# adelacvg/detail_tts

Hardware: AMD Instinct MI355X
Metric: generated audio seconds/sec (24 kHz), 10 s prompt, batch 8 per GPU (higher is better)
Workload: dtype f32; 1 GPU; configs[2]: 1xMI355X batch-8, 10 s prompts (T_ref=936), 234 codes -> 9.984 s audio per utterance; GPT KV-cache decode + 50-step CFG diffusion + flow-VAE/HiFiGAN vocoder, seed-0 random-init weights; batch_per_gpu=8, codes=234, diffusion_steps=50, parallelism=replica x1

## Files before the change

detail_tts_amd/csrc/conv_gemm.h:

```cpp
#pragma once
#include "common.h"

namespace dtts {

struct ConvParams {
    const float* x = nullptr;
    long long x_bs = 0;
    int x_cs = 0;
    const int* len_in = nullptr;
    const int* x_bidx = nullptr;
    int Tin = 0;
    const float* pro_ab = nullptr;
    int pro_act = ACT_NONE;
    float pro_slope = 0.f;
    const float* w = nullptr;
    const float* bias = nullptr;
    int Cin = 0, CinP = 0, Cout = 0, CoutP = 0, KW = 1, stride = 1, dil = 1, pad = 0;
    const float* badd = nullptr;
    int badd_bs = 0;
    int gate = GATE_NONE;
    int epi_act = ACT_NONE;
    float epi_slope = 0.f;
    float out_scale = 1.f;
    const float* res = nullptr;
    long long res_bs = 0;
    int res_cs = 0;
    float res_scale = 1.f;
    int res_bmod = 0;
    int mask_out = 0;
    float* y = nullptr;
    long long y_bs = 0;
    int y_cs = 0;
    const int* len_out = nullptr;
    int Nout = 0;
    int phases = 1;
    int B = 0;
    const void* w3 = nullptr;
    const void* x3 = nullptr;
    int x3_tp = 0;
    int x3_halo = 1;
    void* qkv_planes = nullptr;
    int qkv_heads = 0, qkv_nt64 = 0, qkv_tq = 0;
    float qkv_qscale = 1.f;
    void* gn_out3 = nullptr;
    const float *gn_gamma = nullptr, *gn_beta = nullptr;
    const float* gn_ada = nullptr;
    int gn_ada_stride = 0;
    const int* gn_ada_idx = nullptr;
    int gn_act = ACT_NONE, gn_groups = 32;
    float gn_eps = 1e-5f;
    void* gn_xch = nullptr;
    unsigned gn_tag = 0;
    int* gn_err = nullptr;
    const int* cols = nullptr;
    int ncols = 0, cols_b0 = 0;
    void* next3 = nullptr;
    int next_c8 = 0, next_tp = 0, next_halo = 0, next_act = ACT_NONE;
    float next_slope = 0.f;
    int* next_sat = nullptr;
    int ksplit = 1;
    int ksplit_max = 0;
    int p1 = 0;
    int epi_vec = 0;
    float* kpart = nullptr;
    int* kcount = nullptr;
    int ablate = 0;
};

void launch_conv_gemm(const ConvParams& p, hipStream_t stream);

}
```

detail_tts_amd/csrc/conv_gemm.hip:

```cpp
#include <cstdlib>
#include "conv_gemm_kernel.h"

namespace dtts {

static int env_int(const char* name) {
    const char* v = getenv(name);
    return v ? atoi(v) : 0;
}

void launch_conv_gemm(const ConvParams& p_in, hipStream_t stream) {
    static const int ablate = env_int("DTTS_CONV_ABLATE");
    ConvParams p = p_in;
    p.ablate = ablate;
    DTTS_REQUIRE(p.B > 0 && p.Nout > 0 && p.Cout > 0 && p.Cin > 0, "empty conv");
    DTTS_REQUIRE(p.x && p.w && p.y, "null pointer");
    DTTS_REQUIRE(p.gate == GATE_NONE || p.phases == 1, "gate+phases unsupported");
    static const int force_bn = env_int("DTTS_CONV_BN"), force_bk = env_int("DTTS_CONV_BK");
    const int halo = (p.KW - 1) * p.dil;
    auto fits = [&](int bn) { return (bn - 1) * p.stride + halo + 1 <= XW_MAX; };
    const bool bk32 = (p.CinP % 32 == 0) && force_bk == 32 && p.KW * p.dil <= 3;
    static const int small_tiles = []() { const char* v = getenv("DTTS_CONV_SMALL_TILES"); return v ? atoi(v) : 384; }();
    if (small_tiles > 0 && p.CoutP % 64 == 0 && fits(64) && (long long)cdiv(p.CoutP, 128) * cdiv(p.Nout, 128) * p.B <= small_tiles) {
        static const int small_bk = []() { const char* v = getenv("DTTS_CONV_SMALL_BK"); return v ? atoi(v) : 32; }();
        if (small_bk == 32 && p.CinP % 32 == 0 && p.KW * p.dil <= 3) launch_conv_tile<64, 64, 2, 2, 32>(p, stream, "conv_gemm_kernel<64,64,k32>");
        else launch_conv_tile<64, 64, 2, 2, 16>(p, stream, "conv_gemm_kernel<64,64,k16>");
        return;
    }
    if (p.CoutP % 128 == 0) {
        const int pad128 = round_up(p.Nout, 128), pad64 = round_up(p.Nout, 64);
        bool wide = fits(128) && (pad128 - pad64) * 10 <= p.Nout;
        if (force_bn == 128 && fits(128)) wide = true;
        if (force_bn == 64) wide = false;
        if (wide) {
            if (bk32) launch_conv_tile<128, 128, 2, 2, 32>(p, stream, "conv_gemm_kernel<128,128,k32>");
            else launch_conv_tile<128, 128, 2, 2, 16>(p, stream, "conv_gemm_kernel<128,128,k16>");
        } else {
            DTTS_REQUIRE(fits(64), "conv halo too large");
            if (bk32) launch_conv_tile<128, 64, 2, 2, 32>(p, stream, "conv_gemm_kernel<128,64,k32>");
            else launch_conv_tile<128, 64, 2, 2, 16>(p, stream, "conv_gemm_kernel<128,64,k16>");
        }
    } else if (p.CoutP % 64 == 0) {
        if (fits(128) && p.Nout > 64) launch_conv_tile<64, 128, 2, 2, 16>(p, stream, "conv_gemm_kernel<64,128,k16>");
        else { DTTS_REQUIRE(fits(64), "conv halo too large"); launch_conv_tile<64, 64, 2, 2, 16>(p, stream, "conv_gemm_kernel<64,64,k16>"); }
    } else {
        DTTS_REQUIRE(p.CoutP % 32 == 0, "CoutP must be a multiple of 32");
        DTTS_REQUIRE(fits(128), "conv halo too large");
        launch_conv_tile<32, 128, 1, 4, 16>(p, stream, "conv_gemm_kernel<32,128,k16>");
    }
}

}
```

detail_tts_amd/csrc/conv_x3.h:

```cpp
#pragma once
#include "conv_gemm.h"

namespace dtts {

constexpr int X3_HALO = 1;
constexpr int X3_BN = 192;
static inline int x3_tp(int T) { return round_up(T, X3_BN) + 2 * X3_HALO; }
static inline size_t x3_bytes(int B, int C, int T) { return (size_t)B * (C / 8) * 2 * x3_tp(T) * 16; }

void launch_split_weights(const float* wp, int KW, int CinP, int CoutP, void* out, hipStream_t s);
void launch_split_planes(const float* x, long long x_bs, int x_cs, const float* ab, int act, const int* lens, int T, int B, int C,
                         void* out, hipStream_t s);
void launch_split_planes_taps(const float* x, long long x_bs, int x_cs, const int* lens, int T, int B, int C, int KW, int pad, void* out,
                              hipStream_t s, int* sat = nullptr);
void launch_gn_split_planes(const float* x, long long x_bs, int x_cs, const int* lens, int T, int B, int C, int groups,
                            const float* gamma, const float* beta, float eps, const float* ada, int ada_stride, int ada_bs, int act,
                            void* out, hipStream_t s, const int* ada_idx = nullptr);
void launch_conv_x3(const ConvParams& p, hipStream_t s);

constexpr size_t X3_SLAB_FLOATS = 96 * 256, X3_MAX_SLABS = 1024, X3_SPLIT_COUNTERS = 4096;
void x3_split_workspace(hipStream_t s, size_t nslabs, float** part, int** count);

constexpr int GN_FUSE_MAX_NT = 6;
size_t conv_x3_gn_xch_bytes(int B, int Cout, int T);
bool conv_x3_gn_fusable(int Cout, int CoutP, int Cin, int KW, int groups, int B, int T);

constexpr int X3D_HALO = 32;
static inline int x3d_tp(int T) { return round_up(T, X3_BN) + 64 + X3D_HALO; }
static inline size_t x3d_bytes(int B, int CP, int T) { return (size_t)B * (CP / 8) * 2 * x3d_tp(T) * 16; }
void launch_split_planes_ex(const float* x, long long x_bs, int x_cs, int act, float slope, const int* lens, int T, int B, int C, int CP,
                            int halo, int Tp, void* out, hipStream_t s, int* sat = nullptr);
void launch_conv_x3d(const ConvParams& p, hipStream_t s);
void launch_zero_plane_margins(const int* lens, int T, int B, int CP, int halo, int Tp, void* out, hipStream_t s);

}
```

detail_tts_amd/csrc/conv_x3.hip:

```cpp
#include <algorithm>
#include <cstdio>
#include <mutex>
#include <type_traits>
#include <utility>
#include <vector>

#include "conv_x3.h"
#include <cstdlib>
#include "prof.h"
#include "split3.h"

namespace dtts {

typedef float f32x16 __attribute__((ext_vector_type(16)));

namespace {
constexpr int NPL = XS_PLANES, NK = 2 * NPL;
constexpr int BM = 128, BN = X3_BN;
constexpr int WTILE = NK * BM * 16;
constexpr int XMAIN = NK * BN * 16;
constexpr int XBUF = XMAIN + NK * 2 * 16;
typedef unsigned gn_u4 __attribute__((ext_vector_type(4)));
constexpr int GN_AUX_SC1 = 16;
constexpr int GN_MAXW = 8;
constexpr int GN_SPIN_LIMIT = 1 << 22;
static_assert(7 * 32 <= 256 && 3 * GN_FUSE_MAX_NT <= 32 && (4 * 16 * 104 + 4 * GN_MAXW + 16 + 2 * BM) * 4 <= 2 * (WTILE + XBUF), "fused GroupNorm epilogue: LDS / lanes");

__global__ __launch_bounds__(256) void split_weights_kernel(const float* __restrict__ wp, int C8, int CoutP, uint4* __restrict__ out) {
    const int m = blockIdx.x * 256 + threadIdx.x, c8 = blockIdx.y, tap = blockIdx.z;
    if (m >= CoutP) return;
    float v[8];
#pragma unroll
    for (int e = 0; e < 8; ++e) v[e] = wp[((long long)tap * C8 * 8 + c8 * 8 + e) * CoutP + m] * XS_SCALE_W;
    uint4 q0, q1;
    split8(v, q0, q1);
    uint4* o = out + ((long long)(tap * C8 + c8) * NPL) * CoutP + m;
    o[0] = q0;
    o[CoutP] = q1;
}

template <int ACT, bool AB>
__global__ __launch_bounds__(256) void split_planes_kernel(const float* __restrict__ x, long long x_bs, int x_cs,
                                                          const float* __restrict__ ab, const int* __restrict__ lens, int T, int C8,
                                                          int Tp, uint4* __restrict__ out) {
    const int tp = blockIdx.x * 256 + threadIdx.x, c8 = blockIdx.y, b = blockIdx.z;
    if (tp >= Tp) return;
    const int t = tp - X3_HALO, len = lens ? lens[b] : T;
    uint4 q0 = make_uint4(0, 0, 0, 0), q1 = q0;
    if (t >= 0 && t < len) {
        const float* xr = x + (long long)b * x_bs + (long long)(c8 * 8) * x_cs + t;
        float v[8];
#pragma unroll
        for (int e = 0; e < 8; ++e) v[e] = xr[(long long)e * x_cs];
        if (AB) {
            const float* abr = ab + ((long long)b * C8 + c8) * 16;
#pragma unroll
            for (int e = 0; e < 8; ++e) v[e] = abr[2 * e] * v[e] + abr[2 * e + 1];
        }
        if (ACT == ACT_SILU) {
#pragma unroll
            for (int e = 0; e < 8; ++e) v[e] = v[e] * __frcp_rn(1.f + __expf(-v[e]));
        }
#pragma unroll
        for (int e = 0; e < 8; ++e) v[e] *= XS_SCALE_X;
        split8(v, q0, q1);
    }
    uint4* o = out + ((long long)(b * C8 + c8) * NPL) * Tp + tp;
    o[0] = q0;
    o[Tp] = q1;
}

template <int ACT>
__global__ __launch_bounds__(1024) void gn_split_planes_kernel(const float* __restrict__ x, long long x_bs, int x_cs,
                                                              const int* __restrict__ lens, int T, int C, int groups,
                                                              const float* __restrict__ gamma, const float* __restrict__ beta, float eps,
                                                              const float* __restrict__ ada, int ada_stride, int ada_bs, int Tp,
                                                              uint4* __restrict__ out, const int* __restrict__ ada_idx) {
    __shared__ float red[2][16];
    __shared__ float sa[64], sd[64];
    const int g = blockIdx.x, b = blockIdx.y, tid = threadIdx.x, lane = tid & 63, wave = tid >> 6, nthr = blockDim.x;
    const int len = lens ? lens[b] : T;
    const int cpg = C / groups;
    const float* xg = x + (long long)b * x_bs + (long long)(g * cpg) * x_cs;
    const float k = xg[0];
    float s1 = 0.f, s2 = 0.f;
    const bool vec = ((x_cs & 3) == 0) && ((reinterpret_cast<unsigned long long>(xg) & 15ull) == 0);
    if (vec) {
        const int len4 = len >> 2, n4 = cpg * len4;
        for (int i0 = tid; i0 < n4; i0 += 4 * nthr) {
            float4 v[4];
#pragma unroll
            for (int u = 0; u < 4; ++u) {
                const int i = i0 + u * nthr, ic = i < n4 ? i : 0;
                const int row = ic / len4, t4 = ic - row * len4;
                v[u] = reinterpret_cast<const float4*>(xg + (long long)row * x_cs)[t4];
            }
#pragma unroll
            for (int u = 0; u < 4; ++u) {
                if (i0 + u * nthr >= n4) continue;
                const float d0 = v[u].x - k, d1 = v[u].y - k, d2 = v[u].z - k, d3 = v[u].w - k;
                s1 += (d0 + d1) + (d2 + d3);
                s2 += (d0 * d0 + d1 * d1) + (d2 * d2 + d3 * d3);
            }
        }
        const int rem = len - (len4 << 2);
        for (int i = tid; i < cpg * rem; i += nthr) {
            const int row = i / rem, t = (len4 << 2) + (i - row * rem);
            const float d = xg[(long long)row * x_cs + t] - k;
            s1 += d;
            s2 += d * d;
        }
    } else {
        for (int i = tid; i < cpg * len; i += nthr) {
            const int row = i / len, t = i - row * len;
            const float d = xg[(long long)row * x_cs + t] - k;
            s1 += d;
            s2 += d * d;
        }
    }
#pragma unroll
    for (int o = 32; o > 0; o >>= 1) {
        s1 += __shfl_xor(s1, o);
        s2 += __shfl_xor(s2, o);
    }
    if (lane == 0) { red[0][wave] = s1; red[1][wave] = s2; }
    __syncthreads();
    float S1 = 0.f, S2 = 0.f;
    for (int i = 0; i < (nthr >> 6); ++i) { S1 += red[0][i]; S2 += red[1][i]; }
    const float n = (float)(cpg * len);
    S1 /= n;
    S2 /= n;
    const float mean = k + S1, var = fmaxf(S2 - S1 * S1, 0.f), rstd = rsqrtf(var + eps);
    if (tid < cpg) {
        const int c = g * cpg + tid;
        float a = rstd * gamma[c];
        float d = beta[c] - mean * a;
        if (ada) {
            const float* ad = ada + (ada_idx ? (long long)ada_idx[b] : (long long)b * ada_bs);
            const float sc = 1.f + ad[(long long)c * ada_stride], sh = ad[(long long)(C + c) * ada_stride];
            a *= sc;
            d = d * sc + sh;
        }
        sa[tid] = a;
        sd[tid] = d;
    }
    __syncthreads();
    const int c8n = cpg >> 3, C8 = C >> 3;
    for (int item = blockIdx.z * nthr + tid; item < c8n * Tp; item += nthr * gridDim.z) {
        const int c8l = item / Tp, tp = item - c8l * Tp, t = tp - X3_HALO;
        uint4 q0 = make_uint4(0, 0, 0, 0), q1 = q0;
        if (t >= 0 && t < len) {
            const float* xr = xg + (long long)(c8l * 8) * x_cs + t;
            float v[8];
#pragma unroll
            for (int e = 0; e < 8; ++e) v[e] = xr[(long long)e * x_cs];
#pragma unroll
            for (int e = 0; e < 8; ++e) {
                v[e] = sa[c8l * 8 + e] * v[e] + sd[c8l * 8 + e];
                if (ACT == ACT_SILU) v[e] = v[e] * __frcp_rn(1.f + __expf(-v[e]));
                v[e] *= XS_SCALE_X;
            }
            split8(v, q0, q1);
        }
        uint4* o = out + ((long long)(b * C8 + g * c8n + c8l) * NPL) * Tp + tp;
        o[0] = q0;
        o[Tp] = q1;
    }
}

template <int ACT, int NI>
__global__ __launch_bounds__(1024) void gn_split_planes_reg_kernel(const float* __restrict__ x, long long x_bs, int x_cs,
                                                                  const int* __restrict__ lens, int T, int C, int groups,
                                                                  const float* __restrict__ gamma, const float* __restrict__ beta, float eps,
                                                                  const float* __restrict__ ada, int ada_stride, int ada_bs, int Tp,
                                                                  uint4* __restrict__ out, const int* __restrict__ ada_idx) {
    __shared__ float red[2][16];
    __shared__ float sa[64], sd[64];
    const int g = blockIdx.x, b = blockIdx.y, tid = threadIdx.x, lane = tid & 63, wave = tid >> 6;
    const int len = lens ? lens[b] : T;
    const int cpg = C / groups, c8n = cpg >> 3, C8 = C >> 3, nitems = c8n * Tp;
    const float* xg = x + (long long)b * x_bs + (long long)(g * cpg) * x_cs;
    const float k = xg[0];
    float v[NI][8];
    float s1 = 0.f, s2 = 0.f;
#pragma unroll
    for (int q = 0; q < NI; ++q) {
        const int item = tid + q * 1024, c8l = item / Tp, t = item - c8l * Tp - X3_HALO;
        const bool ok = item < nitems && t >= 0 && t < len;
        const float* xr = xg + (long long)(ok ? c8l * 8 : 0) * x_cs + (ok ? t : 0);
#pragma unroll
        for (int e = 0; e < 8; ++e) v[q][e] = xr[(long long)e * x_cs];
        if (ok) {
            float d[8];
#pragma unroll
            for (int e = 0; e < 8; ++e) d[e] = v[q][e] - k;
            s1 += ((d[0] + d[1]) + (d[2] + d[3])) + ((d[4] + d[5]) + (d[6] + d[7]));
            s2 += ((d[0] * d[0] + d[1] * d[1]) + (d[2] * d[2] + d[3] * d[3])) + ((d[4] * d[4] + d[5] * d[5]) + (d[6] * d[6] + d[7] * d[7]));
        }
    }
#pragma unroll
    for (int o = 32; o > 0; o >>= 1) {
        s1 += __shfl_xor(s1, o);
        s2 += __shfl_xor(s2, o);
    }
    if (lane == 0) { red[0][wave] = s1; red[1][wave] = s2; }
    __syncthreads();
    float S1 = 0.f, S2 = 0.f;
#pragma unroll
    for (int i = 0; i < 16; ++i) { S1 += red[0][i]; S2 += red[1][i]; }
    const float n = (float)(cpg * len);
    S1 /= n;
    S2 /= n;
    const float mean = k + S1, var = fmaxf(S2 - S1 * S1, 0.f), rstd = rsqrtf(var + eps);
    if (tid < cpg) {
        const int c = g * cpg + tid;
        float a = rstd * gamma[c];
        float d = beta[c] - mean * a;
        if (ada) {
            const float* ad = ada + (ada_idx ? (long long)ada_idx[b] : (long long)b * ada_bs);
            const float sc = 1.f + ad[(long long)c * ada_stride], sh = ad[(long long)(C + c) * ada_stride];
            a *= sc;
            d = d * sc + sh;
        }
        sa[tid] = a;
        sd[tid] = d;
    }
    __syncthreads();
#pragma unroll
    for (int q = 0; q < NI; ++q) {
        const int item = tid + q * 1024;
        if (item >= nitems) continue;
        const int c8l = item / Tp, tp = item - c8l * Tp, t = tp - X3_HALO;
        uint4 q0 = make_uint4(0, 0, 0, 0), q1 = q0;
        if (t >= 0 && t < len) {
            float w[8];
#pragma unroll
            for (int e = 0; e < 8; ++e) {
                w[e] = sa[c8l * 8 + e] * v[q][e] + sd[c8l * 8 + e];
                if (ACT == ACT_SILU) w[e] = w[e] * __frcp_rn(1.f + __expf(-w[e]));
                w[e] *= XS_SCALE_X;
            }
            split8(w, q0, q1);
        }
        uint4* o = out + ((long long)(b * C8 + g * c8n + c8l) * NPL) * Tp + tp;
        o[0] = q0;
        o[Tp] = q1;
    }
}

template <int EPI, bool KW3, int NSTG, bool P1 = false>
__global__ __launch_bounds__(256, (NSTG == 2 && EPI != 3) ? 3 : 2) void conv_x3_kernel(ConvParams p) {
    constexpr int KW = KW3 ? 3 : 1, D = NSTG - 1;
    constexpr int CB = P1 ? 4 : 2;
    constexpr int NT = P1 ? 2 : 3;
    auto chunk_of = [](int kind) { return P1 ? kind * NPL : (kind & 1) * NPL + (kind >> 1); };
    constexpr int XOFF = NSTG * WTILE;
    extern __shared__ __attribute__((aligned(16))) unsigned char smem[];
    const int tid = threadIdx.x, lane = tid & 63, wave = __builtin_amdgcn_readfirstlane(tid >> 6), l31 = lane & 31, lhi = lane >> 5;
    const int mtiles = p.CoutP / BM, ntiles = (p.Nout + BN - 1) / BN;
    const int Ls = xcd_remap(blockIdx.x, gridDim.x);
    const int S = p.ksplit, L = Ls / S, z = Ls - L * S;
    const bool mt_major = EPI == 3 && !(p.ablate & 16);
    int mt = mt_major ? (L / ntiles) % mtiles : L % mtiles;
    int b = mt_major ? L / (ntiles * mtiles) : (L / mtiles) / ntiles;
    int nti = mt_major ? L % ntiles : (L / mtiles) - b * ntiles;
    int bn = L / mtiles;
    if (EPI == 2 && mtiles > 6 && mtiles % 6 == 0 && !(p.ablate & 1024)) {
        const int nbn = p.cols ? p.ncols : ntiles * p.B, per_blk = 5 * mtiles, blk = L / per_blk, r = L - blk * per_blk;
        const int bn0 = blk * 5, nb = min(5, nbn - bn0), per_grp = nb * 6, mg = r / per_grp, r2 = r - mg * per_grp, bnl = r2 / 6;
        mt = mg * 6 + (r2 - bnl * 6);
        bn = bn0 + bnl;
        b = bn / ntiles;
        nti = bn - b * ntiles;
    }
    if (p.cols) {
        const int pk = __builtin_amdgcn_readfirstlane(p.cols[bn]);
        b = (pk >> 8) - p.cols_b0;
        nti = pk & 255;
    }
    const int m0 = mt * BM, n0 = nti * BN;
    const int nvalid = p.len_out ? p.len_out[b] : p.Nout;
    if (n0 >= nvalid) return;
    const int C8 = p.Cin >> 3, call = p.Cin >> (P1 ? 5 : 4), Tp = p.x3_tp;
    const int cbeg = (int)((long long)call * z / S), c16n = (int)((long long)call * (z + 1) / S) - cbeg, nks = KW * c16n;
    const int bin = p.x_bidx ? p.x_bidx[b] : b;
    const unsigned lane16 = (unsigned)lane * 16u;
    const unsigned char* wb8 = static_cast<const unsigned char*>(p.w3) + ((long long)m0 + (long long)(CB * cbeg) * NPL * p.CoutP) * 16;
    const unsigned char* xb8 = static_cast<const unsigned char*>(p.x3) +
                               ((long long)bin * C8 * NPL * Tp + n0 + (X3_HALO - p.pad) + (long long)(CB * cbeg) * NPL * Tp) * 16;
    const long long wtapB = (long long)C8 * NPL * p.CoutP * 16;
    const long long wblkB = (long long)CB * NPL * p.CoutP * 16;
    const long long xblkB = (long long)CB * NPL * Tp * 16;
    auto dma = [&](const unsigned char* g, int lds_off) {
        __builtin_amdgcn_global_load_lds((const __attribute__((address_space(1))) void*)(g + lane16),
                                         (__attribute__((address_space(3))) void*)(smem + lds_off), 16, 0, 0);
    };
    const int wkind = wave;
    const unsigned char* wq = wb8 + (long long)chunk_of(wkind) * p.CoutP * 16;
    const int wlds = wkind * (BM * 16);
    const unsigned char* xq = xb8 + (long long)chunk_of(wkind) * Tp * 16;
    const int xlds = XOFF + wkind * (BN * 16);
    long long x3o[3];
    int x3l[3];
#pragma unroll
    for (int t = 0; t < 3; ++t) {
        const int j = t * 4 + wave, kind = j / 3, cb = j - kind * 3;
        x3o[t] = ((long long)chunk_of(kind) * Tp + cb * 64) * 16;
        x3l[t] = XOFF + kind * (BN * 16) + cb * 1024;
    }
    const long long halo_lane = (lane < 2 * NK) ? (((long long)chunk_of(lane >> 1) * Tp + BN + (lane & 1)) * 16 - (long long)lane16) : 0;
    const unsigned char* xblk = xb8;
    auto issue_w = [&](int i, int stage) { dma(wq + i * 1024, stage * WTILE + wlds + i * 1024); };
    auto issue_x1 = [&](int i, int stage) { dma(xq + i * 1024, stage * XBUF + xlds + i * 1024); };
    auto issue_x3 = [&](int t, int stage) { dma(xblk + x3o[t], stage * XBUF + x3l[t]); };
    auto issue_halo = [&](int stage) {
        if (lane < 2 * NK)
            __builtin_amdgcn_global_load_lds((const __attribute__((address_space(1))) void*)(xblk + halo_lane + lane16),
                                             (__attribute__((address_space(3))) void*)(smem + XOFF + stage * XBUF + XMAIN), 16, 0, 0);
    };
    int itap = 0;
    auto next_w = [&]() {
        if (!KW3) wq += wblkB;
        else if (itap < 2) { wq += wtapB; ++itap; }
        else { wq += wblkB - 2 * wtapB; itap = 0; }
    };

    const int wm0 = (wave >> 1) * 64, wn0 = (wave & 1) * 96;
    f32x16 acc[2][3];
#pragma unroll
    for (int i = 0; i < 2; ++i)
#pragma unroll
        for (int j = 0; j < 3; ++j)
#pragma unroll
            for (int r = 0; r < 16; ++r) acc[i][j][r] = 0.f;

#pragma unroll
    for (int q = 0; q < D; ++q) {
        if (q < nks) {
            issue_w(0, q);
            issue_w(1, q);
        }
        next_w();
        if (!KW3) {
            if (q < nks) {
#pragma unroll
                for (int i = 0; i < 3; ++i) issue_x1(i, q);
            }
            xq += xblkB;
        } else {
            if (q < c16n) {
#pragma unroll
                for (int t = 0; t < 3; ++t) issue_x3(t, q);
                issue_halo(q);
            }
            xblk += xblkB;
        }
    }
    float* bias_s = reinterpret_cast<float*>(smem + XOFF + NSTG * XBUF);
    if (tid < BM) bias_s[tid] = (p.bias && m0 + tid < p.Cout) ? p.bias[m0 + tid] : 0.f;
    float* ga_s = bias_s + BM + 4;
    float* gb_s = ga_s + BM;
    if (EPI == 3 && tid < BM) {
        const int c = m0 + tid;
        float ga = p.gn_gamma[c], gb = p.gn_beta[c];
        if (p.gn_ada) {
            const float* ad = p.gn_ada + (p.gn_ada_idx ? (long long)p.gn_ada_idx[b] : 0);
            const float sc = 1.f + ad[(long long)c * p.gn_ada_stride], sh = ad[(long long)(p.Cout + c) * p.gn_ada_stride];
            ga *= sc;
            gb = gb * sc + sh;
        }
        ga_s[tid] = ga;
        gb_s[tid] = gb;
    }

    int c16 = 0, tap = 0;
    int sw = 0, sx = 0;
    auto read_frags = [&](hf8 (&fa)[2][NPL], hf8 (&fb)[3][NPL], int stw, int stx, int tp) {
        const unsigned char* As = smem + stw * WTILE + lhi * (BM * 16);
        const unsigned char* Xb = smem + XOFF + stx * XBUF;
#pragma unroll
        for (int j = 0; j < 3; ++j) {
            const int nn = wn0 + j * 32 + l31 + tp;
            const unsigned char* xr = nn < BN ? Xb + lhi * (BN * 16) + nn * 16 : Xb + XMAIN + lhi * 32 + (nn - BN) * 16;
            const int xps = nn < BN ? 2 * BN * 16 : 64;
#pragma unroll
            for (int pl = 0; pl < NPL; ++pl) fb[j][pl] = *reinterpret_cast<const hf8*>(xr + pl * xps);
        }
#pragma unroll
        for (int i = 0; i < 2; ++i)
#pragma unroll
            for (int pl = 0; pl < NPL; ++pl) fa[i][pl] = *reinterpret_cast<const hf8*>(As + pl * (2 * BM * 16) + (wm0 + i * 32 + l31) * 16);
    };
    auto issue_slot = [&](int slot, int swi, int sxi, bool wlive, bool xlive) {
        __builtin_amdgcn_sched_barrier(0);
        if (slot < 2) { if (wlive) issue_w(slot, swi); }
        else if (!KW3) { if (xlive) issue_x1(slot - 2, sxi); }
        else if (slot == 2) { if (xlive) issue_x3(tap, sxi); }
        else if (slot == 3 && tap == 2) { if (xlive) issue_halo(sxi); }
        __builtin_amdgcn_sched_barrier(0);
    };
    auto advance = [&]() {
        next_w();
        if (!KW3) xq += xblkB;
        sw = sw + 1 == NSTG ? 0 : sw + 1;
        if (++tap == KW) {
            tap = 0;
            ++c16;
            sx = sx + 1 == NSTG ? 0 : sx + 1;
            if (KW3) xblk += xblkB;
        }
    };
    constexpr int TA[3] = {P1 ? 0 : 1, P1 ? 1 : 0, 0}, TB[3] = {0, 1, 0};
    {
    hf8 a[2][NPL], bb[3][NPL];
    int ks = 0;
    constexpr int PERIOD = KW * NSTG;
    auto ustep = [&](auto kc) {
        constexpr int k = decltype(kc)::value;
        constexpr int TAPc = k % KW, SWc = k % NSTG, SXc = (k / KW) % NSTG;
        constexpr int SWI = (SWc + D) % NSTG, SXI = (SXc + D) % NSTG;
        if (NSTG == 2) asm volatile("s_waitcnt vmcnt(0)" ::: "memory");
        else asm volatile("s_waitcnt vmcnt(%0)" ::"n"((NSTG - 2) * (KW3 ? 3 : 5)) : "memory");
        __builtin_amdgcn_s_barrier();
        constexpr bool ASM_READS = NSTG >= 3;
        if (!ASM_READS) read_frags(a, bb, SWc, SXc, TAPc);
        else {
            const unsigned as_addr = (unsigned)(SWc * WTILE) + lhi * (BM * 16) + (wm0 + l31) * 16;
            const unsigned xb_addr = (unsigned)(XOFF + SXc * XBUF);
            auto rd = [&](hf8& dst, unsigned addr) { asm volatile("ds_read_b128 %0, %1" : "=v"(dst) : "v"(addr)); };
            auto a_addr = [&](int i, int pl) { return as_addr + pl * (2 * BM * 16) + i * 32 * 16; };
            auto x_addr = [&](int j, int pl) {
                const int nn = wn0 + j * 32 + l31 + TAPc;
                return nn < BN ? xb_addr + lhi * (BN * 16) + nn * 16 + pl * (2 * BN * 16) : xb_addr + XMAIN + lhi * 32 + (nn - BN) * 16 + pl * 64;
            };
            constexpr int PA0 = TA[0], PA1 = TA[1];
            rd(a[0][PA0], a_addr(0, PA0)); rd(bb[0][0], x_addr(0, 0)); rd(bb[1][0], x_addr(1, 0)); rd(bb[2][0], x_addr(2, 0));
            rd(a[1][PA0], a_addr(1, PA0));
            rd(a[0][PA1], a_addr(0, PA1)); rd(bb[0][1], x_addr(0, 1)); rd(bb[1][1], x_addr(1, 1)); rd(bb[2][1], x_addr(2, 1));
            rd(a[1][PA1], a_addr(1, PA1));
        }
        auto uslot = [&](int slot) {
            __builtin_amdgcn_sched_barrier(0);
            if (slot < 2) issue_w(slot, SWI);
            else if (!KW3) issue_x1(slot - 2, SXI);
            else if (slot == 2) issue_x3(TAPc, SXI);
            else if (slot == 3 && TAPc == 2) issue_halo(SXI);
            __builtin_amdgcn_sched_barrier(0);
        };
        int slot = 0;
#pragma unroll
        for (int t = 0; t < NT; ++t)
#pragma unroll
            for (int i = 0; i < 2; ++i) {
                if (ASM_READS && t == 0 && i == 0) asm volatile("s_waitcnt lgkmcnt(6)" : "+v"(a[0][TA[0]]), "+v"(bb[0][0]), "+v"(bb[1][0]), "+v"(bb[2][0]));
                if (ASM_READS && t == 0 && i == 1) asm volatile("s_waitcnt lgkmcnt(5)" : "+v"(a[1][TA[0]]));
                if (ASM_READS && t == 1 && i == 0) asm volatile("s_waitcnt lgkmcnt(1)" : "+v"(a[0][TA[1]]), "+v"(bb[0][1]), "+v"(bb[1][1]), "+v"(bb[2][1]));
                if (ASM_READS && t == 1 && i == 1) asm volatile("s_waitcnt lgkmcnt(0)" : "+v"(a[1][TA[1]]));
#pragma unroll
                for (int j = 0; j < 3; ++j) acc[i][j] = __builtin_amdgcn_mfma_f32_32x32x16_f16(a[i][TA[t]], bb[j][TB[t]], acc[i][j], 0, 0, 0);
                if (slot < 5) uslot(slot);
                ++slot;
            }
#pragma unroll
        for (; slot < 5; ++slot) uslot(slot);
        if (!KW3) {
            wq += wblkB;
            xq += xblkB;
        } else {
            if ((TAPc + D) % KW < 2) wq += wtapB;
            else wq += wblkB - 2 * wtapB;
            if (TAPc == KW - 1) xblk += xblkB;
        }
    };
    auto uperiod = [&](auto... kc) { (ustep(kc), ...); };
    constexpr bool UNROLL = KW3 || EPI == 2;
    if (UNROLL && !(p.ablate & 512)) {
        const int nper = KW3 ? (c16n - D) / NSTG : (nks - D) / PERIOD;
        for (int q = 0; q < nper; ++q) {
            if constexpr (PERIOD == 2) uperiod(std::integral_constant<int, 0>{}, std::integral_constant<int, 1>{});
            else if constexpr (PERIOD == 3) uperiod(std::integral_constant<int, 0>{}, std::integral_constant<int, 1>{}, std::integral_constant<int, 2>{});
            else if constexpr (PERIOD == 4) uperiod(std::integral_constant<int, 0>{}, std::integral_constant<int, 1>{}, std::integral_constant<int, 2>{}, std::integral_constant<int, 3>{});
            else if constexpr (PERIOD == 6) uperiod(std::integral_constant<int, 0>{}, std::integral_constant<int, 1>{}, std::integral_constant<int, 2>{}, std::integral_constant<int, 3>{}, std::integral_constant<int, 4>{}, std::integral_constant<int, 5>{});
            else if constexpr (PERIOD == 9) uperiod(std::integral_constant<int, 0>{}, std::integral_constant<int, 1>{}, std::integral_constant<int, 2>{}, std::integral_constant<int, 3>{}, std::integral_constant<int, 4>{}, std::integral_constant<int, 5>{}, std::integral_constant<int, 6>{}, std::integral_constant<int, 7>{}, std::integral_constant<int, 8>{});
            else uperiod(std::integral_constant<int, 0>{}, std::integral_constant<int, 1>{}, std::integral_constant<int, 2>{}, std::integral_constant<int, 3>{}, std::integral_constant<int, 4>{}, std::integral_constant<int, 5>{}, std::integral_constant<int, 6>{}, std::integral_constant<int, 7>{}, std::integral_constant<int, 8>{}, std::integral_constant<int, 9>{}, std::integral_constant<int, 10>{}, std::integral_constant<int, 11>{});
        }
        ks = nper * PERIOD;
        c16 = ks / KW;
        itap = D % KW;
    }
    for (; ks < nks; ++ks) {
        if (NSTG == 2 || ks + D > nks || (KW3 && c16 + D >= c16n)) asm volatile("s_waitcnt vmcnt(0)" ::: "memory");
        else asm volatile("s_waitcnt vmcnt(%0)" ::"n"((NSTG - 2) * (KW3 ? 3 : 5)) : "memory");
        __builtin_amdgcn_s_barrier();
        read_frags(a, bb, sw, sx, tap);
        const int swi = sw + D >= NSTG ? sw + D - NSTG : sw + D, sxi = sx + D >= NSTG ? sx + D - NSTG : sx + D;
        const bool wlive = ks + D < nks, xlive = KW3 ? c16 + D < c16n : ks + D < nks;
        int slot = 0;
#pragma unroll
        for (int t = 0; t < NT; ++t)
#pragma unroll
            for (int i = 0; i < 2; ++i) {
#pragma unroll
                for (int j = 0; j < 3; ++j) acc[i][j] = __builtin_amdgcn_mfma_f32_32x32x16_f16(a[i][TA[t]], bb[j][TB[t]], acc[i][j], 0, 0, 0);
                if (slot < 5) issue_slot(slot, swi, sxi, wlive, xlive);
                ++slot;
            }
#pragma unroll
        for (; slot < 5; ++slot) issue_slot(slot, swi, sxi, wlive, xlive);
        advance();
    }
    }
    asm volatile("s_waitcnt vmcnt(0)" ::: "memory");

    if (S > 1) {
        float* slab = p.kpart + ((size_t)L * S) * (96 * 256);
        float* mine = slab + (size_t)z * (96 * 256) + tid;
#pragma unroll
        for (int i = 0; i < 2; ++i)
#pragma unroll
            for (int j = 0; j < 3; ++j)
#pragma unroll
                for (int r = 0; r < 16; ++r) __hip_atomic_store(mine + ((i * 3 + j) * 16 + r) * 256, acc[i][j][r], __ATOMIC_RELAXED, __HIP_MEMORY_SCOPE_AGENT);
        asm volatile("s_waitcnt vmcnt(0)" ::: "memory");
        __syncthreads();
        int* s_last = reinterpret_cast<int*>(bias_s + BM);
        if (tid == 0) *s_last = __hip_atomic_fetch_add(p.kcount + L, 1, __ATOMIC_RELAXED, __HIP_MEMORY_SCOPE_AGENT) == S - 1 ? 1 : 0;
        __syncthreads();
        if (!*s_last) return;
        if (tid == 0) __hip_atomic_store(p.kcount + L, 0, __ATOMIC_RELAXED, __HIP_MEMORY_SCOPE_AGENT);
#pragma unroll
        for (int i = 0; i < 2; ++i)
#pragma unroll
            for (int j = 0; j < 3; ++j)
#pragma unroll
                for (int r = 0; r < 16; ++r) acc[i][j][r] = 0.f;
        for (int zz = 0; zz < S; ++zz) {
            const float* src = slab + (size_t)zz * (96 * 256) + tid;
#pragma unroll
            for (int i = 0; i < 2; ++i)
#pragma unroll
                for (int j = 0; j < 3; ++j)
#pragma unroll
                    for (int r = 0; r < 16; ++r)
                        acc[i][j][r] += __hip_atomic_load(src + ((i * 3 + j) * 16 + r) * 256, __ATOMIC_RELAXED, __HIP_MEMORY_SCOPE_AGENT);
        }
    }

    if (EPI == 3) {
        constexpr int EP_LD = 104;
        if (p.ablate & 64) return;
        __syncthreads();
        float* st = reinterpret_cast<float*>(smem) + wave * (16 * EP_LD);
        float* prt = reinterpret_cast<float*>(smem) + 4 * 16 * EP_LD;
        float* gst = prt + 4 * GN_MAXW;
        float* sa = gst + 16;
        float* sd = sa + BM;
        const int ncol0 = n0 + wn0;
        const float* rb = p.res ? p.res + (long long)(p.res_bmod ? b % p.res_bmod : b) * p.res_bs : nullptr;
        float4 rv[4][6];
        if (rb) {
#pragma unroll
            for (int q = 0; q < 4; ++q)
#pragma unroll
                for (int k = 0; k < 6; ++k) {
                    const int idx = lane + 64 * k, rl = idx / 24, c4 = idx - rl * 24, row = m0 + wm0 + (q >> 1) * 32 + (q & 1) * 16 + rl, n = ncol0 + c4 * 4;
                    const float* src = rb + (long long)row * p.res_cs + n;
                    rv[q][k] = make_float4(0.f, 0.f, 0.f, 0.f);
                    if (n + 3 < nvalid) rv[q][k] = *reinterpret_cast<const float4*>(src);
                    else if (n < nvalid) {
                        rv[q][k].x = src[0];
                        if (n + 1 < nvalid) rv[q][k].y = src[1];
                        if (n + 2 < nvalid) rv[q][k].z = src[2];
                    }
                }
        }
#pragma unroll
        for (int q = 0; q < 4; ++q) {
            const int i = q >> 1, rowt0 = wm0 + i * 32 + (q & 1) * 16;
            if (rb) {
#pragma unroll
                for (int k = 0; k < 6; ++k) {
                    const int idx = lane + 64 * k, rl = idx / 24, c4 = idx - rl * 24;
                    *reinterpret_cast<float4*>(st + rl * EP_LD + c4 * 4) = rv[q][k];
                }
                asm volatile("s_waitcnt lgkmcnt(0)" ::: "memory");
                __builtin_amdgcn_wave_barrier();
            }
#pragma unroll
            for (int j = 0; j < 3; ++j)
#pragma unroll
                for (int rr = 0; rr < 8; ++rr) {
                    const int r = (q & 1) * 8 + rr, rl = (rr & 3) + 8 * (rr >> 2) + 4 * lhi;
                    float v = acc[i][j][r] * XS_ACC_SCALE + bias_s[rowt0 + rl];
                    if (rb) v += p.res_scale * st[rl * EP_LD + j * 32 + l31];
                    acc[i][j][r] = v;
                }
            if (rb) {
                asm volatile("s_waitcnt lgkmcnt(0)" ::: "memory");
                __builtin_amdgcn_wave_barrier();
            }
        }
        bool okj[3];
#pragma unroll
        for (int j = 0; j < 3; ++j) okj[j] = ncol0 + j * 32 + l31 < nvalid;
        const int nvh = min(max(nvalid - ncol0, 0), 96);
        const float cnt = 8.f * (float)nvh, rcnt = nvh > 0 ? 1.f / cnt : 0.f;
        float s8[8];
#pragma unroll
        for (int ck = 0; ck < 8; ++ck) {
            float a = 0.f;
#pragma unroll
            for (int j = 0; j < 3; ++j)
#pragma unroll
                for (int e = 0; e < 4; ++e) a += okj[j] ? acc[ck >> 2][j][4 * (ck & 3) + e] : 0.f;
            s8[ck] = a;
        }
        const float tot = wave_sum8(s8, lane);
#pragma unroll
        for (int ck = 0; ck < 8; ++ck) {
            const float mu = __builtin_bit_cast(float, __builtin_amdgcn_readlane(__builtin_bit_cast(int, tot), 8 * ck)) * rcnt;
            float a = 0.f;
#pragma unroll
            for (int j = 0; j < 3; ++j)
#pragma unroll
                for (int e = 0; e < 4; ++e) {
                    const float dv = acc[ck >> 2][j][4 * (ck & 3) + e] - mu;
                    a += okj[j] ? dv * dv : 0.f;
                }
            s8[ck] = a;
        }
        const float m2 = wave_sum8(s8, lane);
        const int C8o = p.Cout >> 3, NTs = ntiles;
        const __amdgpu_buffer_rsrc_t xrs = __builtin_amdgcn_make_buffer_rsrc(p.gn_xch, (short)0, (int)((size_t)p.B * C8o * NTs * 2 * 16), 0x00020000);
        if ((lane & 7) == 0) {
            const int chunk = ((m0 + wm0) >> 3) + (lane >> 3);
            const gn_u4 wv = {__float_as_uint(tot * rcnt), __float_as_uint(m2), __float_as_uint(cnt), p.gn_tag};
            __builtin_amdgcn_raw_buffer_store_b128(wv, xrs, (((b * C8o + chunk) * NTs + nti) * 2 + (wave & 1)) * 16, 0, GN_AUX_SC1);
        }
        if (p.y) {
            float* yb = p.y + (long long)b * p.y_bs;
#pragma unroll
            for (int q = 0; q < 4; ++q) {
                const int i = q >> 1, rowt0 = wm0 + i * 32 + (q & 1) * 16;
#pragma unroll
                for (int j = 0; j < 3; ++j)
#pragma unroll
                    for (int rr = 0; rr < 8; ++rr) {
                        const int r = (q & 1) * 8 + rr, rl = (rr & 3) + 8 * (rr >> 2) + 4 * lhi;
                        st[rl * EP_LD + j * 32 + l31] = acc[i][j][r];
                    }
                asm volatile("s_waitcnt lgkmcnt(0)" ::: "memory");
                __builtin_amdgcn_wave_barrier();
#pragma unroll
                for (int k = 0; k < 6; ++k) {
                    const int idx = lane + 64 * k, rl = idx / 24, c4 = idx - rl * 24, row = m0 + rowt0 + rl, n = ncol0 + c4 * 4;
                    const float4 a4 = *reinterpret_cast<const float4*>(st + rl * EP_LD + c4 * 4);
                    if (n < nvalid) {
                        float* dst = yb + (long long)row * p.y_cs + n;
                        if (n + 3 < nvalid) *reinterpret_cast<float4*>(dst) = a4;
                        else {
                            dst[0] = a4.x;
                            if (n + 1 < nvalid) dst[1] = a4.y;
                            if (n + 2 < nvalid) dst[2] = a4.z;
                        }
                    }
                }
                asm volatile("s_waitcnt lgkmcnt(0)" ::: "memory");
                __builtin_amdgcn_wave_barrier();
            }
        }
        if (p.ablate & 128) return;
        const int cpg8 = (p.Cout / p.gn_groups) >> 3;
        const int ct0 = m0 >> 3, g_lo = ct0 / cpg8, g_hi = (ct0 + BM / 8 - 1) / cpg8;
        const int nvt = (nvalid + BN - 1) / BN, ppg = cpg8 * nvt;
        const int SL = ppg <= 16 ? 16 : 32;
        {
            const int gs = tid / SL, k = tid - gs * SL;
            const bool active = gs <= g_hi - g_lo && k < ppg;
            float pn = 0.f, pm = 0.f, pq = 0.f;
            if (active) {
                const int ch = k / nvt, nt = k - ch * nvt;
                const int off = (((b * C8o + (g_lo + gs) * cpg8 + ch) * NTs + nt) * 2) * 16;
                gn_u4 v0, v1;
                int spins = 0;
                for (;;) {
                    v0 = __builtin_amdgcn_raw_buffer_load_b128(xrs, off, 0, GN_AUX_SC1);
                    v1 = __builtin_amdgcn_raw_buffer_load_b128(xrs, off + 16, 0, GN_AUX_SC1);
                    if ((v0.w == p.gn_tag && v1.w == p.gn_tag) || (p.ablate & 8)) break;
                    if (++spins > GN_SPIN_LIMIT) {
                        __hip_atomic_store(p.gn_err, 1, __ATOMIC_RELAXED, __HIP_MEMORY_SCOPE_SYSTEM);
                        break;
                    }
                    __builtin_amdgcn_s_sleep(1);
                }
                const float m0v = __uint_as_float(v0.x), q0v = __uint_as_float(v0.y), n0v = __uint_as_float(v0.z);
                const float m1v = __uint_as_float(v1.x), q1v = __uint_as_float(v1.y), n1v = __uint_as_float(v1.z);
                pn = n0v + n1v;
                const float rn = pn > 0.f ? 1.f / pn : 0.f, dm = m0v - m1v;
                pm = (n0v * m0v + n1v * m1v) * rn;
                pq = q0v + q1v + n0v * n1v * rn * dm * dm;
            }
            float N = pn, S = pn * pm;
            for (int o = 1; o < SL; o <<= 1) {
                N += __shfl_xor(N, o);
                S += __shfl_xor(S, o);
            }
            const float mu = N > 0.f ? S / N : 0.f, dmu = pm - mu;
            float M2 = pq + pn * dmu * dmu;
            for (int o = 1; o < SL; o <<= 1) M2 += __shfl_xor(M2, o);
            if (active && k == 0) {
                gst[2 * gs] = mu;
                gst[2 * gs + 1] = rsqrtf((N > 0.f ? M2 / N : 0.f) + p.gn_eps);
            }
        }
        __syncthreads();
        if (tid < BM) {
            const int g = (m0 + tid) / (p.Cout / p.gn_groups) - g_lo;
            const float a = gst[2 * g + 1] * ga_s[tid];
            sa[tid] = a;
            sd[tid] = gb_s[tid] - gst[2 * g] * a;
        }
        __syncthreads();
        if (p.ablate & 256) return;
        const int Tp = p.x3_tp;
        unsigned char* ob = static_cast<unsigned char*>(p.gn_out3) + (size_t)b * C8o * NPL * Tp * 16;
        const bool silu = p.gn_act == ACT_SILU;
#pragma unroll
        for (int i = 0; i < 2; ++i)
#pragma unroll
            for (int j = 0; j < 3; ++j) {
                const int n = ncol0 + j * 32 + l31;
                const bool ok = n < nvalid;
#pragma unroll
                for (int k2 = 0; k2 < 2; ++k2) {
                    const int r16 = wm0 + i * 32 + 16 * k2;
                    float ve[4], vo[4];
#pragma unroll
                    for (int e = 0; e < 4; ++e) {
                        const int ra = r16 + e + 4 * lhi, rb2 = ra + 8;
                        float x0 = acc[i][j][8 * k2 + e] * sa[ra] + sd[ra], x1 = acc[i][j][8 * k2 + 4 + e] * sa[rb2] + sd[rb2];
                        if (silu) {
                            x0 = x0 * __frcp_rn(1.f + __expf(-x0));
                            x1 = x1 * __frcp_rn(1.f + __expf(-x1));
                        }
                        ve[e] = ok ? x0 * XS_SCALE_X : 0.f;
                        vo[e] = ok ? x1 * XS_SCALE_X : 0.f;
                    }
                    unsigned we0[2], we1[2], wo0[2], wo1[2];
                    split_pair(ve[0], ve[1], we0[0], we1[0]);
                    split_pair(ve[2], ve[3], we0[1], we1[1]);
                    split_pair(vo[0], vo[1], wo0[0], wo1[0]);
                    split_pair(vo[2], vo[3], wo0[1], wo1[1]);
                    const auto s00 = __builtin_amdgcn_permlane32_swap(we0[0], wo0[0], false, false);
                    const auto s01 = __builtin_amdgcn_permlane32_swap(we0[1], wo0[1], false, false);
                    const auto s10 = __builtin_amdgcn_permlane32_swap(we1[0], wo1[0], false, false);
                    const auto s11 = __builtin_amdgcn_permlane32_swap(we1[1], wo1[1], false, false);
                    const int c8 = ((m0 + r16) >> 3) + lhi;
                    unsigned char* o = ob + ((size_t)c8 * NPL * Tp + n + X3_HALO) * 16;
                    if (p.ablate & 32) continue;
                    *reinterpret_cast<uint4*>(o) = make_uint4(s00[0], s01[0], s00[1], s01[1]);
                    *reinterpret_cast<uint4*>(o + (size_t)Tp * 16) = make_uint4(s10[0], s11[0], s10[1], s11[1]);
                }
            }
        if (tid < 64) {
            const int side = tid >> 5, c8 = (m0 >> 3) + ((tid & 31) >> 1), pl = tid & 1;
            const int tp = side == 0 ? 0 : n0 + BN + X3_HALO;
            if (side == 0 ? n0 == 0 : (n0 + BN >= nvalid && tp < Tp))
                *reinterpret_cast<uint4*>(ob + ((size_t)(c8 * NPL + pl) * Tp + tp) * 16) = make_uint4(0, 0, 0, 0);
        }
        return;
    }

    if (EPI != 2 && p.epi_vec) {
        constexpr int EP_LD = 104;
        float* yb = p.y + (long long)b * p.y_bs;
        const float* rb = p.res ? p.res + (long long)(p.res_bmod ? b % p.res_bmod : b) * p.res_bs : nullptr;
        const int ncol0 = n0 + wn0;
        constexpr bool RES_AHEAD = NSTG >= 3;
        float4 rva[RES_AHEAD ? 4 : 1][6];
        auto load_res = [&](int q, float4 (&dst)[6]) {
#pragma unroll
            for (int k = 0; k < 6; ++k) {
                const int idx = lane + 64 * k, rl = idx / 24, c4 = idx - rl * 24, row = m0 + wm0 + (q >> 1) * 32 + (q & 1) * 16 + rl, n = ncol0 + c4 * 4;
                dst[k] = (row < p.Cout && n < nvalid) ? *reinterpret_cast<const float4*>(rb + (long long)row * p.res_cs + n)
                                                      : make_float4(0.f, 0.f, 0.f, 0.f);
            }
        };
        if (RES_AHEAD && rb) {
#pragma unroll
            for (int q = 0; q < 4; ++q) load_res(q, rva[q]);
        }
        __syncthreads();
        float* st = reinterpret_cast<float*>(smem) + wave * (16 * EP_LD);
#pragma unroll
        for (int q = 0; q < 4; ++q) {
            const int i = q >> 1, rowt0 = wm0 + i * 32 + (q & 1) * 16;
            float4 (&rv)[6] = rva[RES_AHEAD ? q : 0];
            if (!RES_AHEAD && rb) load_res(q, rv);
#pragma unroll
            for (int j = 0; j < 3; ++j)
#pragma unroll
                for (int rr = 0; rr < 8; ++rr) {
                    const int r = (q & 1) * 8 + rr, rl = (rr & 3) + 8 * (rr >> 2) + 4 * lhi;
                    st[rl * EP_LD + j * 32 + l31] = acc[i][j][r];
                }
            asm volatile("s_waitcnt lgkmcnt(0)" ::: "memory");
            __builtin_amdgcn_wave_barrier();
            if (EPI == 4) {
                const float* bad = p.badd ? p.badd + (long long)b * p.badd_bs : nullptr;
#pragma unroll
                for (int k = 0; k < 3; ++k) {
                    const int idx = lane + 64 * k, pr = idx / 24, c4 = idx - pr * 24, rt = rowt0 + 2 * pr, row = m0 + rt, n = ncol0 + c4 * 4;
                    const float4 a4 = *reinterpret_cast<const float4*>(st + (2 * pr) * EP_LD + c4 * 4);
                    const float4 b4 = *reinterpret_cast<const float4*>(st + (2 * pr + 1) * EP_LD + c4 * 4);
                    if (row + 1 < p.Cout && n < nvalid) {
                        float ba = bias_s[rt], bb = bias_s[rt + 1];
                        if (bad) { ba += bad[row]; bb += bad[row + 1]; }
                        const float av[4] = {a4.x, a4.y, a4.z, a4.w}, gv[4] = {b4.x, b4.y, b4.z, b4.w};
                        float o[4];
#pragma unroll
                        for (int e = 0; e < 4; ++e) {
                            const float ta = av[e] * XS_ACC_SCALE + ba, tb = gv[e] * XS_ACC_SCALE + bb;
                            o[e] = tanhf(ta) * sigmoidf_(tb);
                        }
                        float* dst = yb + (long long)(row >> 1) * p.y_cs + n;
                        if (n + 3 < nvalid) *reinterpret_cast<float4*>(dst) = make_float4(o[0], o[1], o[2], o[3]);
                        else
                            for (int e = 0; e < 4 && n + e < nvalid; ++e) dst[e] = o[e];
                    }
                }
                asm volatile("s_waitcnt lgkmcnt(0)" ::: "memory");
                __builtin_amdgcn_wave_barrier();
                continue;
            }
#pragma unroll
            for (int k = 0; k < 6; ++k) {
                const int idx = lane + 64 * k, rl = idx / 24, c4 = idx - rl * 24, row = m0 + rowt0 + rl, n = ncol0 + c4 * 4;
                const float4 a4 = *reinterpret_cast<const float4*>(st + rl * EP_LD + c4 * 4);
                const float bz = bias_s[rowt0 + rl];
                float o[4] = {a4.x * XS_ACC_SCALE + bz, a4.y * XS_ACC_SCALE + bz, a4.z * XS_ACC_SCALE + bz, a4.w * XS_ACC_SCALE + bz};
                if (EPI == 1) {
#pragma unroll
                    for (int e = 0; e < 4; ++e) o[e] = act_apply(o[e], p.epi_act, p.epi_slope) * p.out_scale;
                }
                if (rb) {
                    o[0] += p.res_scale * rv[k].x; o[1] += p.res_scale * rv[k].y; o[2] += p.res_scale * rv[k].z; o[3] += p.res_scale * rv[k].w;
                }
                if (row < p.Cout && n < nvalid) {
                    float* dst = yb + (long long)row * p.y_cs + n;
                    if (n + 3 < nvalid) *reinterpret_cast<float4*>(dst) = make_float4(o[0], o[1], o[2], o[3]);
                    else
                        for (int e = 0; e < 4 && n + e < nvalid; ++e) dst[e] = o[e];
                }
            }
            asm volatile("s_waitcnt lgkmcnt(0)" ::: "memory");
            __builtin_amdgcn_wave_barrier();
        }
        return;
    }
    if (EPI == 4) return;
    float bv[2][16];
#pragma unroll
    for (int i = 0; i < 2; ++i)
#pragma unroll
        for (int r = 0; r < 16; ++r) bv[i][r] = bias_s[wm0 + i * 32 + (r & 3) + 8 * (r >> 2) + 4 * lhi];
    if (EPI == 2) {
        constexpr int D = 48, KT = 64;
        const int H = p.qkv_heads, Tq = p.qkv_tq;
        const size_t qb = (size_t)2 * 6 * Tq * 16, hb = qb + (size_t)p.qkv_nt64 * (2 * (6 * KT + 384) * 16);
        unsigned char* pb = static_cast<unsigned char*>(p.qkv_planes) + (size_t)b * H * hb;
        const int q4 = lane & 3;
#pragma unroll
        for (int i = 0; i < 2; ++i)
#pragma unroll
            for (int j = 0; j < 3; ++j) {
                const int n = n0 + wn0 + j * 32 + l31;
                if (((n0 + wn0 + j * 32) & ~63) >= nvalid) continue;
                const bool ok = n < nvalid;
#pragma unroll
                for (int k2 = 0; k2 < 2; ++k2) {
                    const int r16 = m0 + wm0 + i * 32 + 16 * k2;
                    if (r16 >= p.Cout) continue;
                    const int h = r16 / (3 * D), rem = r16 - h * 3 * D, sec = rem / D, c16 = rem - sec * D;
                    if (sec == 2) continue;
                    unsigned char* hp = pb + (size_t)h * hb;
                    const float sc = sec == 0 ? p.qkv_qscale * 16.f : 16.f;
                    unsigned we0[2], we1[2], wo0[2], wo1[2];
                    {
                        float ve[4], vo[4];
#pragma unroll
                        for (int e = 0; e < 4; ++e) {
                            ve[e] = (acc[i][j][8 * k2 + e] * XS_ACC_SCALE + bv[i][8 * k2 + e]) * sc;
                            vo[e] = (acc[i][j][8 * k2 + 4 + e] * XS_ACC_SCALE + bv[i][8 * k2 + 4 + e]) * sc;
                            if (sec == 1 && !ok) ve[e] = vo[e] = 0.f;
                        }
                        split_pair(ve[0], ve[1], we0[0], we1[0]);
                        split_pair(ve[2], ve[3], we0[1], we1[1]);
                        split_pair(vo[0], vo[1], wo0[0], wo1[0]);
                        split_pair(vo[2], vo[3], wo0[1], wo1[1]);
                    }
                    uint4 q0, q1;
                    {
                        const auto s00 = __builtin_amdgcn_permlane32_swap(we0[0], wo0[0], false, false);
                        const auto s01 = __builtin_amdgcn_permlane32_swap(we0[1], wo0[1], false, false);
                        const auto s10 = __builtin_amdgcn_permlane32_swap(we1[0], wo1[0], false, false);
                        const auto s11 = __builtin_amdgcn_permlane32_swap(we1[1], wo1[1], false, false);
                        q0 = make_uint4(s00[0], s01[0], s00[1], s01[1]);
                        q1 = make_uint4(s10[0], s11[0], s10[1], s11[1]);
                    }
                    const int c8 = (c16 >> 3) + lhi;
                    if (sec == 0) {
                        if (ok) {
                            unsigned char* o = hp + ((size_t)c8 * Tq + n) * 16;
                            *reinterpret_cast<uint4*>(o) = q0;
                            *reinterpret_cast<uint4*>(o + (size_t)6 * Tq * 16) = q1;
                        }
                    } else {
                        unsigned char* o = hp + qb + (size_t)(n >> 6) * (2 * (6 * KT + 384) * 16) + ((size_t)c8 * KT + (n & 63)) * 16;
                        *reinterpret_cast<uint4*>(o) = q0;
                        *reinterpret_cast<uint4*>(o + 6 * KT * 16) = q1;
                    }
                }
#pragma unroll
                for (int rg = 0; rg < 4; ++rg) {
                    const int row0 = m0 + wm0 + i * 32 + 8 * rg + 4 * lhi;
                    if (row0 >= p.Cout) continue;
                    const int h = row0 / (3 * D), rem = row0 - h * 3 * D, sec = rem / D, c = rem - sec * D;
                    if (sec != 2) continue;
                    float v[4];
#pragma unroll
                    for (int e = 0; e < 4; ++e) v[e] = acc[i][j][4 * rg + e] * XS_ACC_SCALE + bv[i][4 * rg + e];
                    unsigned char* hp = pb + (size_t)h * hb;
                    {
                        float t[4];
#pragma unroll
                        for (int e = 0; e < 4; ++e) t[e] = ok ? v[e] * 16.f : 0.f;
                        {
                            const bool odd = q4 & 1;
                            const float a = odd ? t[0] : t[1], bq = odd ? t[2] : t[3];
                            const float ra = __builtin_bit_cast(float, __builtin_amdgcn_mov_dpp(__builtin_bit_cast(int, a), 0xB1, 0xF, 0xF, true));
                            const float rb = __builtin_bit_cast(float, __builtin_amdgcn_mov_dpp(__builtin_bit_cast(int, bq), 0xB1, 0xF, 0xF, true));
                            if (odd) { t[0] = ra; t[2] = rb; } else { t[1] = ra; t[3] = rb; }
                        }
                        {
                            const bool hi2 = q4 & 2;
                            const float a = hi2 ? t[0] : t[2], bq = hi2 ? t[1] : t[3];
                            const float ra = __builtin_bit_cast(float, __builtin_amdgcn_mov_dpp(__builtin_bit_cast(int, a), 0x4E, 0xF, 0xF, true));
                            const float rb = __builtin_bit_cast(float, __builtin_amdgcn_mov_dpp(__builtin_bit_cast(int, bq), 0x4E, 0xF, 0xF, true));
                            if (hi2) { t[0] = ra; t[1] = rb; } else { t[2] = ra; t[3] = rb; }
                        }
                        unsigned w0[2], w1[2];
                        split_pair(t[0], t[1], w0[0], w1[0]);
                        split_pair(t[2], t[3], w0[1], w1[1]);
                        const int ch = c + q4, kb = n - q4, k64 = kb & 63, u = k64 >> 5, j16 = (k64 >> 4) & 1, grp = (k64 & 15) >> 2;
                        const int chunk = ((u * 2 + j16) * 2 + (grp & 1)) * D + ch;
                        unsigned char* o = hp + qb + (size_t)(kb >> 6) * (2 * (6 * KT + 384) * 16) + (size_t)2 * 6 * KT * 16 + (size_t)chunk * 16 + (grp >> 1) * 8;
                        *reinterpret_cast<uint2*>(o) = make_uint2(w0[0], w0[1]);
                        *reinterpret_cast<uint2*>(o + 384 * 16) = make_uint2(w1[0], w1[1]);
                    }
                }
            }
        return;
    }
    float* yb = p.y + (long long)b * p.y_bs;
    const float* rb = p.res ? p.res + (long long)(p.res_bmod ? b % p.res_bmod : b) * p.res_bs : nullptr;
#pragma unroll
    for (int i = 0; i < 2; ++i)
#pragma unroll
        for (int j = 0; j < 3; ++j) {
            const int n = n0 + wn0 + j * 32 + l31;
            if (n >= nvalid) continue;
            float rv[16];
#pragma unroll
            for (int r = 0; r < 16; ++r) {
                const int row = m0 + wm0 + i * 32 + (r & 3) + 8 * (r >> 2) + 4 * lhi;
                rv[r] = rb ? rb[(long long)(row < p.Cout ? row : p.Cout - 1) * p.res_cs + n] : 0.f;
            }
#pragma unroll
            for (int r = 0; r < 16; ++r) {
                const int row = m0 + wm0 + i * 32 + (r & 3) + 8 * (r >> 2) + 4 * lhi;
                if (row >= p.Cout) continue;
                float v = acc[i][j][r] * XS_ACC_SCALE + bv[i][r];
                if (EPI == 1) v = act_apply(v, p.epi_act, p.epi_slope) * p.out_scale;
                v += p.res_scale * rv[r];
                yb[(long long)row * p.y_cs + n] = v;
            }
        }
}
}

void launch_split_weights(const float* wp, int KW, int CinP, int CoutP, void* out, hipStream_t s) {
    DTTS_REQUIRE(CinP % 16 == 0 && CoutP % 64 == 0, "split_weights: padding");
    hipLaunchKernelGGL(split_weights_kernel, dim3(cdiv(CoutP, 256), CinP / 8, KW), dim3(256), 0, s, wp, CinP / 8, CoutP,
                       static_cast<uint4*>(out));
    DTTS_CHECK_HIP(hipGetLastError());
}

template <int KW>
__global__ __launch_bounds__(256) void split_planes_taps_kernel(const float* __restrict__ x, long long x_bs, int x_cs, const int* __restrict__ lens,
                                                               int T, int C8, int pad, int Tp, uint4* __restrict__ out, int* __restrict__ sat) {
    const int tp = blockIdx.x * 256 + threadIdx.x, c8 = blockIdx.y, b = blockIdx.z;
    if (tp >= Tp) return;
    const int t = tp - X3_HALO, len = lens ? lens[b] : T;
    const bool live = t >= 0 && t < len;
    const float* xr = x + (long long)b * x_bs + (long long)(c8 * 8) * x_cs;
    bool over = false;
#pragma unroll
    for (int tap = 0; tap < KW; ++tap) {
        uint4 q0 = make_uint4(0, 0, 0, 0), q1 = q0;
        const int ts = t + tap - pad;
        if (live && ts >= 0 && ts < len) {
            float v[8];
#pragma unroll
            for (int e = 0; e < 8; ++e) {
                v[e] = xr[(long long)e * x_cs + ts] * XS_SCALE_X;
                over |= !(fabsf(v[e]) <= 65504.f);
            }
            split8(v, q0, q1);
        }
        uint4* o = out + ((long long)((b * KW + tap) * C8 + c8) * NPL) * Tp + tp;
        o[0] = q0;
        o[Tp] = q1;
    }
    if (sat && over) *sat = 1;
}

void launch_split_planes_taps(const float* x, long long x_bs, int x_cs, const int* lens, int T, int B, int C, int KW, int pad, void* out,
                              hipStream_t s, int* sat) {
    DTTS_REQUIRE(C % 16 == 0 && KW == 5 && pad >= 0 && pad < KW, "split_planes_taps: 5 taps, channels a multiple of 16");
    const int Tp = x3_tp(T);
    ProfScope ps("split_planes_taps_kernel", 0.0, (double)B * C * T * 4.0 * (1 + KW), s);
    hipLaunchKernelGGL((split_planes_taps_kernel<5>), dim3(cdiv(Tp, 256), C / 8, B), dim3(256), 0, s, x, x_bs, x_cs, lens, T, C / 8, pad, Tp,
                       static_cast<uint4*>(out), sat);
    DTTS_CHECK_HIP(hipGetLastError());
}

void launch_split_planes(const float* x, long long x_bs, int x_cs, const float* ab, int act, const int* lens, int T, int B, int C,
                         void* out, hipStream_t s) {
    DTTS_REQUIRE(C % 16 == 0, "split_planes: channels must be a multiple of 16");
    DTTS_REQUIRE(act == ACT_NONE || act == ACT_SILU, "split_planes: activation");
    const int Tp = x3_tp(T);
    const dim3 grid(cdiv(Tp, 256), C / 8, B);
    uint4* o = static_cast<uint4*>(out);
    const double n = (double)B * C * T;
    ProfScope ps("split_planes_kernel", 0.0, n * 8.0, s);
    if (ab) {
        if (act == ACT_SILU) hipLaunchKernelGGL((split_planes_kernel<ACT_SILU, true>), grid, dim3(256), 0, s, x, x_bs, x_cs, ab, lens, T, C / 8, Tp, o);
        else hipLaunchKernelGGL((split_planes_kernel<ACT_NONE, true>), grid, dim3(256), 0, s, x, x_bs, x_cs, ab, lens, T, C / 8, Tp, o);
    } else {
        if (act == ACT_SILU) hipLaunchKernelGGL((split_planes_kernel<ACT_SILU, false>), grid, dim3(256), 0, s, x, x_bs, x_cs, ab, lens, T, C / 8, Tp, o);
        else hipLaunchKernelGGL((split_planes_kernel<ACT_NONE, false>), grid, dim3(256), 0, s, x, x_bs, x_cs, ab, lens, T, C / 8, Tp, o);
    }
    DTTS_CHECK_HIP(hipGetLastError());
}

void launch_gn_split_planes(const float* x, long long x_bs, int x_cs, const int* lens, int T, int B, int C, int groups,
                            const float* gamma, const float* beta, float eps, const float* ada, int ada_stride, int ada_bs, int act,
                            void* out, hipStream_t s, const int* ada_idx) {
    DTTS_REQUIRE(C % groups == 0 && (C / groups) % 8 == 0 && C / groups <= 64, "gn_split_planes: group size");
    DTTS_REQUIRE(act == ACT_NONE || act == ACT_SILU, "gn_split_planes: activation");
    const int Tp = x3_tp(T);
    uint4* o = static_cast<uint4*>(out);
    ProfScope ps("gn_split_planes_kernel", 0.0, (double)B * C * T * 8.0, s);
    static const int ns = []() { const char* v = getenv("DTTS_GN_SPLIT_NS"); return v ? atoi(v) : 1; }();
    static const int nt = []() { const char* v = getenv("DTTS_GN_SPLIT_NT"); return v ? atoi(v) : 1024; }();
    static const bool reg_ok = []() { const char* v = getenv("DTTS_GN_SPLIT_REG"); return !(v && v[0] == '0'); }();
    constexpr int NI = 3;
    if (reg_ok && ns == 1 && (C / groups / 8) * Tp <= NI * 1024) {
        if (act == ACT_SILU)
            hipLaunchKernelGGL((gn_split_planes_reg_kernel<ACT_SILU, NI>), dim3(groups, B), dim3(1024), 0, s, x, x_bs, x_cs, lens, T, C, groups,
                               gamma, beta, eps, ada, ada_stride, ada_bs, Tp, o, ada_idx);
        else
            hipLaunchKernelGGL((gn_split_planes_reg_kernel<ACT_NONE, NI>), dim3(groups, B), dim3(1024), 0, s, x, x_bs, x_cs, lens, T, C, groups,
                               gamma, beta, eps, ada, ada_stride, ada_bs, Tp, o, ada_idx);
        DTTS_CHECK_HIP(hipGetLastError());
        return;
    }
    if (act == ACT_SILU)
        hipLaunchKernelGGL(gn_split_planes_kernel<ACT_SILU>, dim3(groups, B, ns), dim3(nt), 0, s, x, x_bs, x_cs, lens, T, C, groups, gamma,
                           beta, eps, ada, ada_stride, ada_bs, Tp, o, ada_idx);
    else
        hipLaunchKernelGGL(gn_split_planes_kernel<ACT_NONE>, dim3(groups, B, ns), dim3(nt), 0, s, x, x_bs, x_cs, lens, T, C, groups, gamma,
                           beta, eps, ada, ada_stride, ada_bs, Tp, o, ada_idx);
    DTTS_CHECK_HIP(hipGetLastError());
}

namespace {
struct KSplitWs {
    float* part;
    int* count;
};
KSplitWs ksplit_workspace(hipStream_t s, size_t nslabs) {
    constexpr int SLOTS = 8;
    constexpr size_t MAX_SLABS = X3_MAX_SLABS, MAX_TILES = X3_SPLIT_COUNTERS;
    static std::mutex mu;
    static hipStream_t owner[SLOTS];
    static int owner_dev[SLOTS];
    static float* part[SLOTS];
    static int* count[SLOTS];
    static int used = 0, victim = 0;
    DTTS_REQUIRE(nslabs <= MAX_SLABS, "conv_x3 split-K: launch too large");
    int dev = 0;
    DTTS_CHECK_HIP(hipGetDevice(&dev));
    std::lock_guard<std::mutex> lk(mu);
    int k = 0;
    while (k < used && !(owner[k] == s && owner_dev[k] == dev)) ++k;
    if (k == used) {
        if (used == SLOTS) {
            DTTS_CHECK_HIP(hipDeviceSynchronize());
            for (int t = 0; t < SLOTS; ++t, victim = (victim + 1) % SLOTS)
                if (owner_dev[victim] == dev) break;
            DTTS_REQUIRE(owner_dev[victim] == dev, "conv_x3 split-K: no scratch slot on this device");
            k = victim;
            victim = (victim + 1) % SLOTS;
            owner[k] = s;
            return {part[k], count[k]};
        }
        DTTS_CHECK_HIP(hipMalloc(reinterpret_cast<void**>(&part[k]), MAX_SLABS * 96 * 256 * sizeof(float)));
        DTTS_CHECK_HIP(hipMalloc(reinterpret_cast<void**>(&count[k]), MAX_TILES * sizeof(int)));
        DTTS_CHECK_HIP(hipMemsetAsync(count[k], 0, MAX_TILES * sizeof(int), s));
        owner[k] = s;
        owner_dev[k] = dev;
        ++used;
    }
    return {part[k], count[k]};
}
}

void x3_split_workspace(hipStream_t s, size_t nslabs, float** part, int** count) {
    const KSplitWs w = ksplit_workspace(s, nslabs);
    *part = w.part;
    *count = w.count;
}

size_t conv_x3_gn_xch_bytes(int B, int Cout, int T) { return (size_t)B * (Cout / 8) * cdiv(T, BN) * 2 * 16; }

static long long split_tiles_max() {
    static const long long v = []() { const char* e = getenv("DTTS_CONV_KSPLIT_MAXTILE"); return e ? atoll(e) : 128LL; }();
    return v;
}

bool conv_x3_gn_fusable(int Cout, int CoutP, int Cin, int KW, int groups, int B, int T) {
    if (Cout != CoutP || Cout % BM || groups <= 0 || Cout % groups || Cout / groups != 24 || Cin % 16 || (KW != 1 && KW != 3)) return false;
    const int nt = cdiv(T, BN);
    (void)B;
    return nt <= GN_FUSE_MAX_NT;
}

void launch_conv_x3(const ConvParams& p_in, hipStream_t s) {
    ConvParams p = p_in;
    DTTS_REQUIRE(p.w3 && p.x3 && (p.y || p.qkv_planes || p.gn_out3) && p.x3_tp > 0, "conv_x3: operands");
    const bool gn = p.gn_out3 != nullptr;
    static const int env_ablate = []() { const char* v = getenv("DTTS_CONV_ABLATE"); return v ? atoi(v) : 0; }();
    if (env_ablate) p.ablate = env_ablate;
    if (gn) {
        DTTS_REQUIRE(conv_x3_gn_fusable(p.Cout, p.CoutP, p.Cin, p.KW, p.gn_groups, p.B, p.Nout), "conv_x3: this launch cannot carry a fused GroupNorm");
        DTTS_REQUIRE(p.gn_gamma && p.gn_beta && p.gn_xch && p.gn_tag && p.gn_err && !p.qkv_planes && p.epi_act == ACT_NONE && p.out_scale == 1.f &&
                         (p.gn_act == ACT_NONE || p.gn_act == ACT_SILU), "conv_x3 fused GroupNorm: parameters");
        auto a16 = [](const void* q, long long bs, int cs) { return (reinterpret_cast<unsigned long long>(q) & 15ull) == 0 && (bs & 3) == 0 && (cs & 3) == 0; };
        DTTS_REQUIRE((!p.y || a16(p.y, p.y_bs, p.y_cs)) && (!p.res || a16(p.res, p.res_bs, p.res_cs)), "conv_x3 fused GroupNorm: 16-byte aligned rows");
    }
    DTTS_REQUIRE(p.B > 0 && p.Nout > 0 && p.Cout > 0, "empty conv");
    DTTS_REQUIRE(p.Cin % 16 == 0 && p.CoutP % BM == 0, "conv_x3: channel padding");
    const bool p1 = p.p1 != 0;
    DTTS_REQUIRE(!p1 || (p.Cin % 32 == 0 && p.gate == GATE_NONE), "conv_x3 one-product mode: input channels a multiple of 32, no gate");
    const bool gated = p.gate == GATE_TANH_SIGMOID;
    DTTS_REQUIRE(p.stride == 1 && p.dil == 1 && p.phases == 1 && (p.gate == GATE_NONE ? !p.badd : gated), "conv_x3: unsupported conv form");
    DTTS_REQUIRE(!gated || (p.KW == 1 && !gn && !p.qkv_planes && !p.res && p.epi_act == ACT_NONE && p.out_scale == 1.f && p.Cout % 2 == 0),
                 "conv_x3 gated epilogue: 1x1 conv, no residual / activation");
    DTTS_REQUIRE((p.KW == 1 && p.pad == 0) || (p.KW == 3 && p.pad == 1), "conv_x3: k = 1 or k = 3 (same padding) only");
    DTTS_REQUIRE(round_up(p.Nout, BN) + 2 * X3_HALO <= p.x3_tp, "conv_x3: time padding");
    static const int force_stg = []() { const char* v = getenv("DTTS_CONV_STAGES"); const int n = v ? atoi(v) : 0; return n >= 2 && n <= 4 ? n : 0; }();
    static const long long max3 = []() { const char* v = getenv("DTTS_CONV_STAGES3_MAXWG"); return v ? atoll(v) : 600LL; }();
    static const long long max4 = []() { const char* v = getenv("DTTS_CONV_STAGES4_MAXWG"); return v ? atoll(v) : 128LL; }();
    if (gn) p.cols = nullptr;
    DTTS_REQUIRE(!p.cols || (p.ncols > 0 && p.ncols <= cdiv(p.Nout, BN) * p.B && cdiv(p.Nout, BN) < 256), "conv_x3: column table");
    const long long ntile = (long long)(p.CoutP / BM) * (p.cols ? p.ncols : cdiv(p.Nout, BN) * p.B);
    static const int max_split = []() { const char* v = getenv("DTTS_CONV_KSPLIT"); const int n = v ? atoi(v) : 4; return n < 1 ? 1 : (n > 8 ? 8 : n); }();
    int S = 1;
    const long long split_tiles = split_tiles_max();
    static const long long split_wgs = []() { const char* v = getenv("DTTS_CONV_KSPLIT_WGS"); return v ? atoll(v) : 256LL; }();
    const long long ntile_pad = (long long)(p.CoutP / BM) * cdiv(p.Nout, BN) * p.B;
    static const int max_split_k1 = []() { const char* v = getenv("DTTS_CONV_KSPLIT_K1"); return v ? atoi(v) : 2; }();
    if (ntile_pad <= split_tiles) S = (int)std::min<long long>(std::min<long long>(p.KW == 3 ? max_split : std::min(max_split, max_split_k1), split_wgs / ntile_pad), (p.Cin >> 4) / 8);
    if (p.ksplit_max > 0) S = std::min(S, p.ksplit_max);
    if (S < 1) S = 1;
    p.ksplit = S;
    static const bool epi_vec_on = []() { const char* v = getenv("DTTS_X3_EPI_VEC"); return !(v && v[0] == '0'); }();
    auto al16 = [](const void* q, long long bs, int cs) { return (reinterpret_cast<unsigned long long>(q) & 15ull) == 0 && (bs & 3) == 0 && (cs & 3) == 0; };
    p.epi_vec = (epi_vec_on && p.y && al16(p.y, p.y_bs, p.y_cs) && (!p.res || al16(p.res, p.res_bs, p.res_cs))) ? 1 : 0;
    if (S > 1) {
        const KSplitWs w = ksplit_workspace(s, (size_t)ntile * S);
        p.kpart = w.part;
        p.kcount = w.count;
    }
    const long long nwg = ntile * S;
    static const long long max4k3 = []() { const char* v = getenv("DTTS_CONV_STAGES4_MAXWG_K3"); return v ? atoll(v) : 128LL; }();
    const int nstg = force_stg ? force_stg : (nwg <= (p.KW == 3 ? max4k3 : max4) ? 4 : (nwg <= max3 ? 3 : 2));
    const size_t lds = (size_t)nstg * (WTILE + XBUF) + BM * sizeof(float) + 16 + (gn ? 2 * BM * sizeof(float) : 0);
    const int l4 = 4 * (WTILE + XBUF) + 3 * BM * (int)sizeof(float) + 16;
    const dim3 grid((unsigned)nwg);
    const double cols = (double)p.B * p.Nout;
    const double flops = 2.0 * p.Cout * p.Cin * p.KW * cols;
    const double bytes = 4.0 * cols * p.Cin + 4.0 * cols * p.Cout * (p.res ? 2.0 : 1.0) + 4.0 * (double)p.Cout * p.Cin * p.KW;
    {
        static const bool by_shape = []() { const char* v = getenv("DTTS_PROF_SHAPES"); return v && v[0] == '1'; }();
        const char* tag = p1 ? "conv_x3_kernel<128,192,fp16>" : "conv_x3_kernel<128,192>";
        if (by_shape && p1) tag = p.KW == 3 ? "conv_x3 fp16 k3" : (p.Cout > 1024 ? "conv_x3 fp16 k1 M=2304" : (p.res ? "conv_x3 fp16 k1 +res" : "conv_x3 fp16 k1"));
        else if (by_shape) tag = p.KW == 3 ? "conv_x3 k3" : (p.Cout > 1024 ? "conv_x3 k1 M=2304" : (p.res ? "conv_x3 k1 +res" : "conv_x3 k1"));
        ProfScope ps(tag, flops, bytes, s);
        const bool epi = p.epi_act != ACT_NONE || p.out_scale != 1.f;
#define DTTS_LAUNCH_X3P1(E, K3)                                                                                        \
    do {                                                                                                               \
        if (nstg == 4) { lds_optin(reinterpret_cast<const void*>(conv_x3_kernel<E, K3, 4, true>), l4); hipLaunchKernelGGL((conv_x3_kernel<E, K3, 4, true>), grid, dim3(256), lds, s, p); } \
        else if (nstg == 3) { lds_optin(reinterpret_cast<const void*>(conv_x3_kernel<E, K3, 3, true>), l4); hipLaunchKernelGGL((conv_x3_kernel<E, K3, 3, true>), grid, dim3(256), lds, s, p); } \
        else { lds_optin(reinterpret_cast<const void*>(conv_x3_kernel<E, K3, 2, true>), l4); hipLaunchKernelGGL((conv_x3_kernel<E, K3, 2, true>), grid, dim3(256), lds, s, p); } \
    } while (0)
#define DTTS_LAUNCH_X3(E, K3)                                                                                          \
    do {                                                                                                               \
        if (p1) DTTS_LAUNCH_X3P1(E, K3);                                                                               \
        else DTTS_LAUNCH_X3N(E, K3);                                                                                   \
    } while (0)
#define DTTS_LAUNCH_X3N(E, K3)                                                                                         \
    do {                                                                                                               \
        if (nstg == 4) { lds_optin(reinterpret_cast<const void*>(conv_x3_kernel<E, K3, 4>), l4); hipLaunchKernelGGL((conv_x3_kernel<E, K3, 4>), grid, dim3(256), lds, s, p); } \
        else if (nstg == 3) { lds_optin(reinterpret_cast<const void*>(conv_x3_kernel<E, K3, 3>), l4); hipLaunchKernelGGL((conv_x3_kernel<E, K3, 3>), grid, dim3(256), lds, s, p); } \
        else { lds_optin(reinterpret_cast<const void*>(conv_x3_kernel<E, K3, 2>), l4); hipLaunchKernelGGL((conv_x3_kernel<E, K3, 2>), grid, dim3(256), lds, s, p); } \
    } while (0)
        if (gn) {
            if (p.KW == 3) DTTS_LAUNCH_X3(3, true);
            else DTTS_LAUNCH_X3(3, false);
        } else if (gated) {
            DTTS_REQUIRE(p.epi_vec, "conv_x3 gated epilogue: rows of y must be 16-byte aligned");
            DTTS_LAUNCH_X3N(4, false);
        } else if (p.qkv_planes) {
            DTTS_REQUIRE(p.KW == 1 && !epi && !p.res && p.Cout % 144 == 0 && p.qkv_heads * 144 == p.Cout, "qkv planes epilogue: 48-channel heads, 1x1 conv");
            DTTS_LAUNCH_X3(2, false);
        } else if (p.KW == 3) {
            if (epi) DTTS_LAUNCH_X3(1, true);
            else DTTS_LAUNCH_X3(0, true);
        } else {
            if (epi) DTTS_LAUNCH_X3(1, false);
            else DTTS_LAUNCH_X3(0, false);
        }
#undef DTTS_LAUNCH_X3
#undef DTTS_LAUNCH_X3N
#undef DTTS_LAUNCH_X3P1
    }
    DTTS_CHECK_HIP(hipGetLastError());
}

}
```

detail_tts_amd/csrc/model.h:

```cpp
#pragma once
#include <map>
#include <memory>
#include <atomic>
#include <thread>
#include <cstring>
#include <memory>
#include <mutex>
#include <string>
#include <unordered_map>
#include <vector>

#include "attention.h"
#include "common.h"
#include "conv_gemm.h"
#include "gpt_kernels.h"
#include "ops.h"
#include "../../include/detail_hip.h"

namespace dtts {

struct PackedConv {
    const float* w = nullptr;
    const float* b = nullptr;
    int Cin = 0, CinP = 0, Cout = 0, CoutP = 0, KW = 1;
    const void* w3 = nullptr;
};

static inline int packed_cout(int cout) { return cout > 64 ? round_up(cout, 128) : (cout > 32 ? 64 : 32); }

struct AttnBlockW {
    const float *gn_g = nullptr, *gn_b = nullptr, *bias_tab = nullptr;
    PackedConv qkv, proj;
    int C = 0, H = 0;
};

struct ResBlockW {
    const float *gn1_g = nullptr, *gn1_b = nullptr, *gn2_g = nullptr, *gn2_b = nullptr;
    PackedConv c1, c2, emb;
    int index = 0;
};

struct DiffLayerW {
    ResBlockW rb;
    AttnBlockW at;
};

struct MelStyleW {
    PackedConv sp0, sp1, t0, t1, qkv, afc, fc;
    int n_mel = 0, hidden = 0, out = 0;
};

struct EncLayerW {
    PackedConv qkv, o, f1, f2;
    const float *ek = nullptr, *ev = nullptr, *g1 = nullptr, *b1 = nullptr, *g2 = nullptr, *b2 = nullptr;
};

struct CouplingW {
    PackedConv pre, post, cond;
    PackedConv in[4], res[3], skip[4];
};

struct GptLayerW {
    const float *ln1_g = nullptr, *ln1_b = nullptr, *ln2_g = nullptr, *ln2_b = nullptr;
    PackedConv attn, proj, fc, fc2;
    const float *attn_c = nullptr, *attn_d = nullptr, *fc_c = nullptr, *fc_d = nullptr;
};

struct GptSession {
    int B = 0, cap = 0, G = 0, steps = 0;
    bool active = false;
    long long kv_bs = 0, kv_layer = 0;
    float *kv = nullptr, *x = nullptr, *y = nullptr, *ab = nullptr, *lat = nullptr, *xa = nullptr, *part = nullptr, *part2 = nullptr,
          *st1 = nullptr, *st2 = nullptr;
    unsigned char* seen = nullptr;
    int *finished = nullptr, *codes = nullptr, *forced = nullptr;
    GptCtl* ctl = nullptr;
    unsigned long long* xch = nullptr;
    float* logits = nullptr;
    int* tok_err = nullptr;
    unsigned* tok_epoch = nullptr;
    int tok_wgs = 128;
};

struct ResBlock1W {
    PackedConv c1[3], c2[3];
    int k = 3;
};

struct GenStageW {
    PackedConv up;
    int rate = 1, up_pad = 0, cout = 0;
    ResBlock1W rb[3];
};

class Arena {
public:
    ~Arena();
    void ensure(size_t bytes);
    void reset() { off_ = 0; }
    size_t mark() const { return off_; }
    void rewind(size_t m) { off_ = m; }
    float* f32(size_t n) { return static_cast<float*>(raw(n * sizeof(float))); }
    int* i32(size_t n) { return static_cast<int*>(raw(n * sizeof(int))); }
    void* raw(size_t bytes);
    size_t capacity() const { return cap_; }
    void swap(Arena& o) { std::swap(base_, o.base_); std::swap(cap_, o.cap_); std::swap(off_, o.off_); }

private:
    char* base_ = nullptr;
    size_t cap_ = 0, off_ = 0;
};

class ArenaUse {
public:
    explicit ArenaUse(Arena& a);
    ~ArenaUse();
    ArenaUse(const ArenaUse&) = delete;
    ArenaUse& operator=(const ArenaUse&) = delete;

private:
    Arena* prev_;
};
Arena* arena_override();

struct Schedule {
    int id = 0;
    int kind = 0;
    std::vector<int> tmap;
    std::vector<float> ftimes;
    std::vector<DiffStepCoefs> p;
    std::vector<float> ac, ac_prev;
    std::vector<DpmStepCoefs> dpm;
    float cfk_k = 0.f;
    const float* ss_table = nullptr;
    int n = 0;
    void* mem = nullptr;
    hipEvent_t used = nullptr;
    ~Schedule();
    DdimStepCoefs ddim(int i, float eta) const;
    bool same_key(const Schedule& o) const { return kind == o.kind && tmap == o.tmap && ftimes == o.ftimes; }
};

void dpm_schedule_table(int n, float cfk, std::vector<float>& times, std::vector<float>& model_times, std::vector<DpmStepCoefs>& steps,
                        std::vector<float>* lambda_s = nullptr);

class Model {
public:
    Model(const dtts_config& cfg, int device);
    ~Model();

    void bind_weights(const void* blob, size_t nbytes, const char* const* names, const unsigned long long* offsets,
                      const unsigned long long* numels, int n, hipStream_t stream);

    void diff_conditioning(const float* refer, const int* lens_host, int B, int Tmax, float* cond_out, hipStream_t s);
    void diff_timestep_independent(const float* latent_cm, const int* lens_n_host, int B, int nmax, const float* cond,
                                   float* code_emb, hipStream_t s);
    void diff_forward(const float* x, const float* code_emb, const int* lens_host, int B, int T, int step, int cond_free,
                      float* out, hipStream_t s);
    void diff_sample(const float* code_emb, const int* lens_host, int B, int T, unsigned long long seed, const int* sample_ids_host,
                     int n_steps, const float* x_init, const float* step_noise, float* mel_out, int denorm, hipStream_t s);
    void diff_sample_ex(int sched_id, int sampler, float eta, const float* code_emb, const int* lens_host, int B, int T,
                        unsigned long long seed, const int* sample_ids_host, int n_steps, const float* x_init, const float* step_noise,
                        float* mel_out, int denorm, hipStream_t s);
    void diff_step(int sched_id, int sampler, float eta, float* x, const float* code_emb, const int* lens_host, int B, int T, int step,
                   unsigned long long seed, const int* sample_ids_host, const float* noise, float* x0_out, hipStream_t s);
    void diff_forward_t(const float* x, const float* code_emb, const int* lens_host, int B, int T, int timestep, int cond_free,
                        float* out, hipStream_t s);
    int diff_schedule(const int* timesteps, int n, hipStream_t s);
    int diff_schedule_info(int sched_id, int* tmap, float* coefs, int cap);
    int diff_schedule_dpm(int n, hipStream_t s);
    void diff_step_dpm(int sched_id, float* x, float* x0_hist, const float* code_emb, const int* lens_host, int B, int T, int step,
                       float* x0_out, hipStream_t s);
    void diff_forward_tf(const float* x, const float* code_emb, const int* lens_host, int B, int T, float timestep, int cond_free,
                         float* out, hipStream_t s);
    void diff_p_sample(float* x, const float* code_emb, const int* lens_host, int B, int T, int step, unsigned long long seed,
                       const int* sample_ids_host, const float* noise, float* x0_out, hipStream_t s);
    void gpt_generate(const float* refer, const int* refer_lens_host, int Tr, const int* text_host, const int* text_lens_host,
                      int Lt_max, int B, const dtts_gpt_options& o, int* codes_host, int* ncodes_host, float* latents_cm,
                      int lat_stride, hipStream_t s);
    void gpt_prefill(const float* refer, const int* refer_lens_host, int Tr, const int* text_host, const int* text_lens_host, int Lt_max,
                     int B, const dtts_gpt_options& o, float* latents_cm, int lat_stride, hipStream_t s);
    void gpt_decode_step(hipStream_t s);
    int gpt_decode(int n_steps, hipStream_t s);
    int gpt_all_finished(hipStream_t s);
    void gpt_finish(int* codes_host, int* ncodes_host, hipStream_t s);
    int gpt_steps() const { return gs_.active ? gs_.steps : 0; }
    void op_sample_logits(const float* logits, int R, int V, const int* history_host, int hist_len, const float* uniforms, int top_k,
                          float top_p, float temperature, float repetition_penalty, float typical_mass, int suppress_eos, int* tokens_host,
                          hipStream_t s);
    void gpt_latents(const float* refer, const int* refer_lens_host, int Tr, const int* text_host, const int* text_lens_host,
                     int Lt_max, const int* codes_host, const int* ncodes_host, int n_max, int B, float* latents_cm, int lat_stride,
                     hipStream_t s);
    void mel_style(const MelStyleW& w, const float* mel, const int* lens_dev, const int* lens_host, int B, int T, float* g_out,
                   hipStream_t s);
    void op_mel_style(const char* which, const float* mel, const int* lens_host, int B, int T, float* g_out, hipStream_t s);
    void vocoder(const float* mel, const int* lens_host, int B, int T, unsigned long long seed, const int* sample_ids_host,
                 float noise_scale, const float* noise_override, float* wav, float* trace_z, hipStream_t s, int gen_chunk = 0);
    void generator(const float* z, const float* g, const int* lens_host, int B, int T, float* wav, hipStream_t s, long long z_bs = 0,
                   int z_cs = 0);
    void op_generator(const float* z, const float* g, const int* lens_host, int B, int T, float* wav, hipStream_t s);
    bool rb_fused_ok(const GenStageW& st, int ch) const;
    void rb_fused(const GenStageW& st, const float* x, float* y, int ch, const int* lens, int B, int T, int branch_mask, float scale, hipStream_t s);
    void op_resblock1(int stage, int branch, const float* x, const int* lens_host, int B, int T, float* y, hipStream_t s);
    void op_wn(int flow, const float* h, const float* g, const int* lens_host, int B, int T, float* out, hipStream_t s);
    void op_enc_p(const float* mel, const int* lens_host, int B, int T, float* m_p, float* logs_p, hipStream_t s);
    void enc_p_fwd(const float* mel, const int* dl, int B, int T, float* x, float* y, float* qkv, float* att, float* ffn, float* relk, float* ml,
                   float* stats, hipStream_t s);
    void vq_decode(const int* codes_host, const int* ncodes_host, int nmax, const float* refer, const int* refer_lens_host, int Tr,
                   int B, float* mel_out, hipStream_t s);
    void resample(const float* x, int B, int L, const float* kernel, int orig, int neu, int width, float* y, int Lout, hipStream_t s);
    void mel_spectrogram(const float* wav, const int* lens_host, int B, int L, int n_fft, int hop, float* mel_out, int Tmax, hipStream_t s,
                         float* spec_out = nullptr);
    void vq_encode(const float* mel, const int* lens_host, int B, int T, int* codes_out, float* xvq_out, hipStream_t s);
    void op_attention_block(const char* prefix, const float* x, const int* lens_host, int B, int C, int T, float* y, hipStream_t s);
    void op_resblock(const char* prefix, const float* x, const int* lens_host, int B, int T, int step, float* y, hipStream_t s);
    void op_conv1d(const char* name, const float* x, const int* lens_in_host, int B, int Cin, int Tin, int Cout, int KW, int stride,
                   int dil, int pad, int pro_act, int epi_act, int gate, int phases, const float* res, float* y, int Tout_alloc,
                   hipStream_t s);
    void op_philox_normal(float* out, int n, int B, unsigned long long seed, const int* sample_ids_host, int stage, int step,
                          hipStream_t s);

    void set_option(const std::string& key, int value) {
        if (key == "two_streams") opt_two_streams_ = value != 0;
        else if (key == "conv_x3") {
            DTTS_REQUIRE(value != 0 || !opt_trunk_fp16_, "conv_x3 = 0 (exact fp32 kernels) has no trunk_fp16 mode: set trunk_fp16 = 0 first");
            opt_conv_x3_ = value != 0;
        }
        else if (key == "trunk_fp16") {
            DTTS_REQUIRE(value == 0 || value == 1, "trunk_fp16: 0 or 1");
            DTTS_REQUIRE(value == 0 || use_x3(), "trunk_fp16 = 1 needs the split-precision kernels (conv_x3 = 1): the exact fp32 kernels have no one-product mode");
            opt_trunk_fp16_ = value != 0;
        }
        else if (key == "gpt_graph") opt_gpt_graph_ = value != 0;
        else if (key == "x3_range_check") opt_range_check_ = value != 0;
        else if (key == "gpt_token_kernel") { opt_gpt_token_ = value != 0; if (value != 0) tok_failed_ = false; gpt_drop_graphs(); }
        else if (key == "gpt_token_exclusive_cu") { opt_tok_exclusive_ = value != 0; gpt_drop_graphs(); }
        else if (key == "gpt_token_min_rows") { DTTS_REQUIRE(value == 1 || value == 4 || value == 8, "gpt_token_min_rows: 1, 4 or 8"); opt_tok_min_rows_ = value; gpt_drop_graphs(); }
        else if (key == "gpt_token_wgs") { DTTS_REQUIRE(value == 128 || value == 64 || value == 32, "gpt_token_wgs: 128, 64 or 32"); opt_tok_wgs_ = value; gpt_drop_graphs(); }
        else if (key == "gpt_token_fault") opt_tok_fault_ = value;
        else if (key == "gpt_token_fault_eos") opt_tok_fault_eos_ = value;
        else if (key == "cfg_streams") opt_cfg_streams_ = value < 0 ? 0 : value;
        else if (key == "gn_fuse") opt_gn_fuse_ = value != 0;
        else if (key == "conv_cols") opt_conv_cols_ = value != 0;
        else if (key == "voc_chain_planes") opt_voc_chain_ = value != 0;
        else if (key == "voc_x3") opt_voc_x3_ = value != 0;
        else if (key == "x3_fault") opt_x3_fault_ = value;
        else if (key == "attn_ksplit_cus") set_attn_ksplit_cus(value);
        else if (key == "attn_ksplit") set_attn_ksplit(value);
        else if (key == "ln_reg") set_ln_channels_reg(value != 0);
        else if (key == "integ_pipeline") opt_integ_pipeline_ = value;
        else throw Error(-1, "unknown option '" + key + "'");
    }
    int get_option(const std::string& key) const {
        if (key == "conv_x3") return use_x3() ? 1 : 0;
        if (key == "trunk_fp16") return opt_trunk_fp16_ ? 1 : 0;
        throw Error(-1, "option '" + key + "' cannot be read back");
    }
    std::string last_error;
    dtts_config cfg;
    int device;

private:
    friend struct Stage;
    const float* W(const std::string& name, size_t numel) const;
    const float* Wopt(const std::string& name, size_t numel) const;
    PackedConv conv(const std::string& name, int Cin, int Cout, int KW, bool bias = true, int cout_p = 0) const;
    AttnBlockW attn_block(const std::string& prefix, int C, int H) const;
    ResBlockW res_block(const std::string& prefix, int C, int index) const;
    void resblock1_fwd(const ResBlock1W& rb, const float* x, float* tmp, float* out, int ch, const int* lens, int B, int T, hipStream_t s,
                       void* xs = nullptr);
    bool vocoder_x3() const;
    void wn_fwd(const CouplingW& c, float* h, const float* g, int gin, float* Gc, float* acts, float* h2, float* skip, const int* dl, int B,
                int T, hipStream_t s);
    void build_diffusion(hipStream_t s);
    void build_vocoder(hipStream_t s);
    void build_gpt(hipStream_t s);
    void gpt_head_and_sample(hipStream_t s);
    void gpt_step_launches(hipStream_t s);
    hipGraphExec_t gpt_capture(int n);
    void gpt_drop_graphs();
    void build_vq();
    void build_frontend();
    void gpt_prefill_layers(float* x, const int* lens, int B, int L, float* kv_cache, long long kv_layer_stride, long long kv_bs,
                            int kv_cs, hipStream_t s);
    MelStyleW mel_style_w(const std::string& prefix, int n_mel, int hidden, int out) const;
    ConvParams cp(const float* x, int cin, float* y, int cout, int B, int T, int Ta, const int* lens) const;

    const int* upload_ints(const int* host, int n, hipStream_t s);
    void register_cols(const int* lens_dev, const int* lens_host, int nb, int T, hipStream_t s);

    void run_conv(const PackedConv& pc, ConvParams p, hipStream_t s) const;
    struct GnNext {
        const float *gamma = nullptr, *beta = nullptr;
        int act = ACT_NONE;
    };
    struct GnFuse {
        void* xs_alt = nullptr;
        int slot = 0;
        bool in_ready = false;
    };
    void attention_block(const AttnBlockW& w, const float* x, float* y, float* qkv, float* att, float* ab, const int* lens, int B,
                         int T, int Ta, hipStream_t s, void* xs = nullptr, GnFuse* f = nullptr, const GnNext* next = nullptr);
    void res_block_fwd(const Schedule& sc, const ResBlockW& w, const float* x, float* h1, float* y, float* ab, const int* lens, int B, int T, int Ta,
                       int step, hipStream_t s, void* xs = nullptr, const int* step_idx = nullptr, GnFuse* f = nullptr,
                       const GnNext* next = nullptr);
    struct GnXch {
        void* buf = nullptr;
        size_t bytes = 0;
        unsigned tag = 0;
    };
    static constexpr int GN_SLOTS = 8;
    GnXch gn_xch_[GN_SLOTS];
    int* gn_err_host_ = nullptr;
    int* gn_err_dev_ = nullptr;
    bool opt_gn_fuse_ = false;
    void gn_fill(ConvParams& p, int slot, size_t bytes, const GnNext& n, void* out3, int groups, hipStream_t s);
    void gn_check();
    bool use_x3() const;
    void diff_forward_pair(const Schedule& sc, const float* x, const float* cbuf0, const int* lens2, const int* lens_i, const int* umap, int B, int Nu,
                           int T, int step, float* out2, hipStream_t s, const float* integ = nullptr);
    void precompute_integrator(const Schedule& sc, const float* cbuf0, const int* lens_i_host, int B, int Nu, int T, const std::vector<int>& steps,
                               float* integ_all, hipStream_t s, std::vector<std::pair<int, hipEvent_t>>* ready = nullptr);
    struct PairPlan { const int *lens2, *lens_i, *umap; int Nu; std::vector<int> ulen; };
    PairPlan plan_pair(const int* lens_host, int B, int T, hipStream_t s);

    std::unordered_map<std::string, std::pair<const float*, size_t>> weights_;
    bool bound_ = false;

    std::vector<DiffLayerW> integ_, layers_;
    std::vector<ResBlockW> tail_;
    std::vector<AttnBlockW> latcond_, ctx_;
    PackedConv inp_block_, integ1_, integ2_, out_conv_, latcond0_, ctx0_, ctx1_, te0_, te2_;
    const float *out_gn_g_ = nullptr, *out_gn_b_ = nullptr, *code_gn_g_ = nullptr, *code_gn_b_ = nullptr, *uncond_ = nullptr;
    int n_resblocks_ = 0;
    Schedule sched0_;
    static constexpr size_t MAX_SCHEDULES = 8;
    std::vector<std::unique_ptr<Schedule>> sched_cache_;
    int sched_next_id_ = 1;
    std::mutex sched_mu_;
    Schedule& schedule(int id);
    void diff_forward_s(Schedule& sc, const float* x, const float* code_emb, const int* lens_host, int B, int T, int step, int cond_free,
                        float* out, hipStream_t s);
    void build_ss_table(const Schedule& sc, float* ss_table, float* scratch, void* ts_dev, hipStream_t s);
    int cache_schedule(std::unique_ptr<Schedule> key, hipStream_t s);

    MelStyleW ref_enc_, gpt_cond_;
    bool has_vocoder_ = false, has_gpt_ = false;
    PackedConv in_proj_, enc_out_, enc_proj_, dec_pre_, dec_cond_, dec_post_;
    std::vector<EncLayerW> enc_layers_;
    std::vector<CouplingW> flows_;
    std::vector<GenStageW> gen_;

    std::vector<GptLayerW> gpt_layers_;
    PackedConv mel_head_;
    const float *lnf_g_ = nullptr, *lnf_b_ = nullptr, *fin_g_ = nullptr, *fin_b_ = nullptr;
    const float *text_emb_ = nullptr, *mel_emb_ = nullptr, *text_pos_ = nullptr, *mel_pos_ = nullptr;

    Arena gpt_persist_;
    Arena gpt_tokw_;
    std::vector<GptTokenLayer> tok_layers_;
    GptTokenParams tokp_;
    bool tok_ok_ = false;
    bool opt_gpt_token_ = true;
    bool opt_tok_exclusive_ = false;
    int opt_tok_min_rows_ = 1;
    int opt_tok_wgs_ = 128;
    bool tok_failed_ = false;
    int opt_tok_fault_ = 0;
    int opt_tok_fault_eos_ = 0;
    struct GptReplay {
        bool valid = false;
        int Tr = 0, Lt_max = 0, B = 0, lat_stride = 0;
        bool has_refer_lens = false, has_text_lens = false;
        std::vector<int> refer_lens, text, text_lens, sample_ids, forced_codes;
        std::vector<unsigned long long> row_seeds;
        dtts_gpt_options o;
        float* latents_cm = nullptr;
    } replay_;
    Arena gpt_replay_;
    bool replaying_ = false;
    bool gpt_use_token_kernel() const;
    Arena gpt_state_;
    GptSession gs_;
    GptCtl ctl_host_;
    hipGraphExec_t gpt_graph_[2] = {nullptr, nullptr};
    hipStream_t sg_ = nullptr;
    hipEvent_t ev_g0_ = nullptr, ev_g1_ = nullptr;
    bool opt_gpt_graph_ = false;

    bool opt_two_streams_ = true;
    int prof_rot_ = 0;
    bool opt_voc_x3_ = true;
    int opt_x3_fault_ = 0;
    bool opt_voc_chain_ = true;
    bool opt_conv_cols_ = true;
    bool opt_range_check_ = false;
    static constexpr int X3_SAT_SLOTS = 8;
    int* x3_sat_ = nullptr;
    int* x3_sat_ring_dev_ = nullptr;
    int* x3_sat_dev_ = nullptr;
    long long x3_ticket_ = 0;
    int* x3_sat_flag(hipStream_t s);
    void x3_sat_check(hipStream_t s);
public:
    long long vocoder_ticket() const { return x3_ticket_; }
    bool vocoder_check_active() const { return x3_sat_dev_ != nullptr && vocoder_x3(); }
    int x3_sat_depth_ = 0;
    struct SatScope {
        Model* m;
        hipStream_t s;
        SatScope(Model* m_, hipStream_t s_) : m(m_), s(s_) { if (m->x3_sat_depth_++ == 0) m->x3_sat_flag(s); }
        ~SatScope() { --m->x3_sat_depth_; }
        void check() { if (m->x3_sat_depth_ == 1) m->x3_sat_check(s); }
        SatScope(const SatScope&) = delete;
        SatScope& operator=(const SatScope&) = delete;
    };
    void vocoder_check(long long ticket);
private:
    int opt_cfg_streams_ = 0;
    bool opt_conv_x3_ = true;
    bool opt_trunk_fp16_ = false;
    Arena w3_;
    Arena w3_voc_;
    static constexpr int MAX_CFG_STREAMS = 4;
    hipStream_t sx_[MAX_CFG_STREAMS - 1] = {nullptr, nullptr, nullptr};
    hipEvent_t ev_fork_ = nullptr, ev_joinx_[MAX_CFG_STREAMS - 1] = {nullptr, nullptr, nullptr};
    int opt_integ_pipeline_ = 0;
    hipStream_t si_ = nullptr;
    std::vector<hipEvent_t> ev_integ_;

    bool has_frontend_ = false;
    PackedConv fe_dft_, fe_mel_;
    int fe_nfft_ = 0;

    bool has_vq_ = false;
    MelStyleW vq_ref_enc_;
    PackedConv vq_up1_, vq_up2_, vq_out_;
    const float *vq_table_ = nullptr, *vq_ln_g_ = nullptr, *vq_ln_b_ = nullptr;
    bool has_vq_enc_ = false;
    PackedConv vqe_c1_, vqe_c2_, vqe_c3_, vq_proj_in_;
    const float *vqe_ln_g_ = nullptr, *vqe_ln_b_ = nullptr, *vq_embed_ = nullptr, *vq_embed_sq_ = nullptr;

    Arena ws_main_;
    Arena& ws() { Arena* o = arena_override(); return o ? *o : ws_main_; }
    Arena ws_voc_;
    Arena ws_gpt_;
    Arena persist_;
    struct IntRing {
        static constexpr int SEGS = 16;
        int* dev = nullptr;
        int* pinned = nullptr;
        size_t off = 0;
        int seg = 0;
        std::vector<hipStream_t> users[SEGS];
        hipEvent_t ev = nullptr;
        unsigned long long last_use = 0;
        std::shared_ptr<std::atomic<int>> owner_alive;
    };
    static constexpr size_t MAX_INT_RINGS = 16;
    unsigned long long ring_clock_ = 0;
    std::map<std::thread::id, std::unique_ptr<IntRing>> int_rings_;
    std::mutex ints_mu_;
    IntRing& int_ring();
};

}
```

detail_tts_amd/csrc/model.hip:

```cpp
#include "model.h"
#include <algorithm>
#include <cstring>
#include "conv_x3.h"
#include "prof.h"

#include <cmath>
#include <cstdlib>

namespace dtts {
static void make_side_stream(hipStream_t* st) {
    static const int reserve = []() { const char* v = getenv("DTTS_B_CU_RESERVE"); return v ? atoi(v) : 0; }();
    if (reserve > 0 && reserve < 256) {
        uint32_t mask[8];
        for (int i = 0; i < 8; ++i) mask[i] = 0xffffffffu;
        for (int b = 256 - reserve; b < 256; ++b) mask[b >> 5] &= ~(1u << (b & 31));
        DTTS_CHECK_HIP(hipExtStreamCreateWithCUMask(st, 8, mask));
        return;
    }
    DTTS_CHECK_HIP(hipStreamCreateWithFlags(st, hipStreamNonBlocking));
}


static thread_local Arena* t_arena_override = nullptr;
Arena* arena_override() { return t_arena_override; }
// ... 472 lines not shown
        if (e->id == id) return *e;
    throw Error(-1, "diffusion schedule " + std::to_string(id) + " is not cached (evicted or never built): call dtts_diff_schedule again");
}

int Model::cache_schedule(std::unique_ptr<Schedule> sc, hipStream_t s) {
    std::lock_guard<std::mutex> lk(sched_mu_);
    for (size_t k = 0; k < sched_cache_.size(); ++k)
        if (sched_cache_[k]->same_key(*sc)) {
            std::rotate(sched_cache_.begin(), sched_cache_.begin() + k, sched_cache_.begin() + k + 1);
            return sched_cache_[0]->id;
        }
    while (sched_cache_.size() >= MAX_SCHEDULES) sched_cache_.pop_back();
    const int C = cfg.diff_channels, NS = sc->n;
    const size_t fl = (size_t)n_resblocks_ * 2 * C * NS;
    DTTS_CHECK_HIP(hipMalloc(&sc->mem, sizeof(float) * (fl + 3 * (size_t)C * NS) + sizeof(int) * NS));
    float* base = static_cast<float*>(sc->mem);
    sc->ss_table = base;
    build_ss_table(*sc, base, base + fl, base + fl + 3 * (size_t)C * NS, s);
    DTTS_CHECK_HIP(hipEventCreateWithFlags(&sc->used, hipEventDisableTiming));
    DTTS_CHECK_HIP(hipEventRecord(sc->used, s));
    sc->id = sched_next_id_++;
    sched_cache_.insert(sched_cache_.begin(), std::move(sc));
    return sched_cache_[0]->id;
}

int Model::diff_schedule(const int* timesteps, int n, hipStream_t s) {
    DTTS_REQUIRE(bound_ && sched0_.n > 0, "diffusion weights not bound");
    DTTS_REQUIRE(timesteps && n >= 1, "diff_schedule: empty timestep list");
    const int trained = cfg.diff_trained_steps;
    std::vector<int> tmap(timesteps, timesteps + n);
    for (int t : tmap) DTTS_REQUIRE(t >= 0 && t < trained, "diff_schedule: timestep out of [0, diff_trained_steps)");
    std::sort(tmap.begin(), tmap.end());
    tmap.erase(std::unique(tmap.begin(), tmap.end()), tmap.end());
    if (tmap == sched0_.tmap) return 0;
    auto sc = std::make_unique<Schedule>();
    make_schedule(trained, tmap, cfg.cond_free_k, *sc);
    return cache_schedule(std::move(sc), s);
}

int Model::diff_schedule_dpm(int n, hipStream_t s) {
    DTTS_REQUIRE(bound_ && sched0_.n > 0, "diffusion weights not bound");
    DTTS_REQUIRE(n >= 2 && n <= cfg.diff_trained_steps, "diff_schedule_dpm: n out of [2, diff_trained_steps]");
    auto sc = std::make_unique<Schedule>();
    std::vector<float> times, mt;
    std::vector<DpmStepCoefs> steps;
    dpm_schedule_table(n, cfg.cond_free_k, times, mt, steps);
    sc->kind = 1;
    sc->n = n;
    sc->cfk_k = cfg.cond_free_k;
    sc->ftimes.resize(n);
    sc->dpm.resize(n);
    for (int i = 0; i < n; ++i) {
        sc->ftimes[i] = mt[n - 1 - i];
        sc->dpm[i] = steps[n - 1 - i];
    }
    return cache_schedule(std::move(sc), s);
}

int Model::diff_schedule_info(int sched_id, int* tmap, float* coefs, int cap) {
    const Schedule& sc = schedule(sched_id);
    DTTS_REQUIRE(sc.kind == 0, "diff_schedule_coefs: not an integer-timestep schedule (DPM tables: dtts_dpm_schedule_table)");
    for (int i = 0; i < sc.n && i < cap; ++i) {
        if (tmap) tmap[i] = sc.tmap[i];
        if (coefs) {
            const DiffStepCoefs& k = sc.p[i];
            const float v[9] = {k.sqrt_recip_ac, k.sqrt_recipm1_ac, k.coef1, k.coef2, k.min_log, k.max_log, k.cfk, sc.ac[i], sc.ac_prev[i]};
            std::memcpy(coefs + (size_t)9 * i, v, sizeof(v));
        }
    }
    return sc.n;
}

void Model::build_diffusion(hipStream_t s) {
    const int C = cfg.diff_channels, H = cfg.diff_heads, NL = cfg.diff_layers;
    {
        std::lock_guard<std::mutex> lk(sched_mu_);
        sched_cache_.clear();
    }
    const std::string d = "diffusion.";
    integ_.clear();
    layers_.clear();
    tail_.clear();
    latcond_.clear();
    ctx_.clear();
    int rbi = 0;
    for (int i = 0; i < 3; ++i) {
        const std::string p = d + "conditioning_timestep_integrator." + std::to_string(i);
        integ_.push_back({res_block(p + ".resblk", C, rbi++), attn_block(p + ".attn", C, H)});
    }
    for (int i = 0; i < NL; ++i) {
        const std::string p = d + "layers." + std::to_string(i);
        layers_.push_back({res_block(p + ".resblk", C, rbi++), attn_block(p + ".attn", C, H)});
    }
    for (int i = NL; i < NL + 3; ++i) tail_.push_back(res_block(d + "layers." + std::to_string(i), C, rbi++));
    inp_block_ = conv(d + "inp_block", cfg.mel_channels, C, 3);
    integ1_ = conv(d + "integrating_conv.a", C, C, 1);
    integ2_ = conv(d + "integrating_conv.b", C, C, 1, false);
    out_gn_g_ = W(d + "out.0.weight", C);
    out_gn_b_ = W(d + "out.0.bias", C);
    out_conv_ = conv(d + "out.2", C, cfg.diff_out_channels, 3);
    code_gn_g_ = W(d + "code_norm.weight", C);
    code_gn_b_ = W(d + "code_norm.bias", C);
    uncond_ = W(d + "unconditioned_embedding", C);
    latcond0_ = conv(d + "latent_conditioner.0", C, C, 3);
    for (int i = 1; i < 5; ++i) latcond_.push_back(attn_block(d + "latent_conditioner." + std::to_string(i), C, H));
    ctx0_ = conv(d + "contextual_embedder.0", cfg.mel_channels, C, 3);
    ctx1_ = conv(d + "contextual_embedder.1", C, 2 * C, 3);
    for (int i = 2; i < 7; ++i) ctx_.push_back(attn_block(d + "contextual_embedder." + std::to_string(i), 2 * C, H));
    te0_ = conv(d + "time_embed.0", C, C, 1);
    te2_ = conv(d + "time_embed.2", C, C, 1);

    make_schedule(cfg.diff_trained_steps, space_steps(cfg.diff_trained_steps, cfg.diff_steps), cfg.cond_free_k, sched0_);
    sched0_.id = 0;
    n_resblocks_ = rbi;

    const int NS = sched0_.n, NRB = rbi;
    persist_.ensure(sizeof(float) * ((size_t)NRB * 2 * C * NS + 3 * (size_t)C * NS) + sizeof(int) * NS + 4096);
    float* ss_table = persist_.f32((size_t)NRB * 2 * C * NS);
    float* scratch = persist_.f32(3 * (size_t)C * NS);
    int* ts_dev = persist_.i32(NS);
    sched0_.ss_table = ss_table;
    build_ss_table(sched0_, ss_table, scratch, ts_dev, s);

    std::vector<PackedConv*> hot = {&inp_block_, &integ1_, &integ2_, &out_conv_};
    auto add_layer = [&](DiffLayerW& l) {
        hot.push_back(&l.rb.c1);
        hot.push_back(&l.rb.c2);
        hot.push_back(&l.at.qkv);
        hot.push_back(&l.at.proj);
    };
    for (auto& l : integ_) add_layer(l);
    for (auto& l : layers_) add_layer(l);
    for (auto& r : tail_) { hot.push_back(&r.c1); hot.push_back(&r.c2); }
    for (auto& b : ctx_) { hot.push_back(&b.qkv); hot.push_back(&b.proj); }
    for (auto& b : latcond_) { hot.push_back(&b.qkv); hot.push_back(&b.proj); }
    size_t total = 0;
    for (PackedConv* pc : hot) {
        DTTS_REQUIRE(pc->Cin == pc->CinP && pc->CoutP % 128 == 0, "trunk conv not eligible for the split-precision path");
        total += (size_t)pc->KW * pc->CinP * pc->CoutP * 4 + 256;
    }
    w3_.ensure(total + 4096);
    for (PackedConv* pc : hot) {
        void* dst = w3_.raw((size_t)pc->KW * pc->CinP * pc->CoutP * 4);
        launch_split_weights(pc->w, pc->KW, pc->CinP, pc->CoutP, dst, s);
        pc->w3 = dst;
    }
}

static size_t qkv_floats(int B, int C, int T) {
    const size_t rows = (size_t)3 * B * C * T, planes = (AttnPlanes::bytes(B, C / AttnPlanes::D, T) + 3) / 4;
    return std::max(rows, planes) + 64;
}

static bool attn_x3_enabled() {
    static const bool on = []() { const char* v = getenv("DTTS_ATTN_X3"); return !(v && v[0] == '0'); }();
    return on;
}

bool Model::use_x3() const {
    static const bool env_on = []() { const char* v = getenv("DTTS_CONV_X3"); return !(v && v[0] == '0'); }();
    return env_on && opt_conv_x3_;
}

void Model::gn_fill(ConvParams& p, int slot, size_t bytes, const GnNext& n, void* out3, int groups, hipStream_t s) {
    DTTS_REQUIRE(slot >= 0 && slot < GN_SLOTS, "fused GroupNorm: exchange slot");
    GnXch& g = gn_xch_[slot];
    if (!gn_err_host_) {
        DTTS_CHECK_HIP(hipHostMalloc(reinterpret_cast<void**>(&gn_err_host_), sizeof(int), hipHostMallocMapped));
        *gn_err_host_ = 0;
        DTTS_CHECK_HIP(hipHostGetDevicePointer(reinterpret_cast<void**>(&gn_err_dev_), gn_err_host_, 0));
    }
    if (bytes > g.bytes) {
        DTTS_CHECK_HIP(hipDeviceSynchronize());
        if (g.buf) DTTS_CHECK_HIP(hipFree(g.buf));
        g.buf = nullptr;
        g.bytes = 0;
        const size_t want = bytes + bytes / 4 + 4096;
        DTTS_CHECK_HIP(hipMalloc(&g.buf, want));
        DTTS_CHECK_HIP(hipMemsetAsync(g.buf, 0, want, s));
        g.bytes = want;
        g.tag = 0;
    }
    if (++g.tag == 0) {
        DTTS_CHECK_HIP(hipMemsetAsync(g.buf, 0, g.bytes, s));
        g.tag = 1;
    }
    p.gn_out3 = out3;
    p.gn_gamma = n.gamma;
    p.gn_beta = n.beta;
    p.gn_act = n.act;
    p.gn_groups = groups;
    p.gn_eps = 1e-5f;
    p.gn_xch = g.buf;
    p.gn_tag = g.tag;
    p.gn_err = gn_err_dev_;
}

void Model::gn_check() {
    if (gn_err_host_ && *gn_err_host_) {
        *gn_err_host_ = 0;
        throw Error(-4, "fused GroupNorm: a statistics exchange timed out (the result of the previous diffusion call is invalid); "
                        "dtts_set_option(\"gn_fuse\", 0) selects the separate pass");
    }
}

void Model::attention_block(const AttnBlockW& w, const float* x, float* y, float* qkv, float* att, float* ab, const int* lens,
                            int B, int T, int Ta, hipStream_t s, void* xs, GnFuse* f, const GnNext* next) {
    const int C = w.C, D = C / w.H;
    const long long bs = (long long)C * Ta;
    int groups = 32;
    while (C % groups) groups /= 2;
    const bool x3 = xs && w.qkv.w3 && w.proj.w3;
    DTTS_REQUIRE(!f || x3, "fused GroupNorm needs the split-precision path");
    const bool in_ready = f && f->in_ready;
    if (f) f->in_ready = false;
    if (in_ready) {}
    else if (x3) launch_gn_split_planes(x, bs, Ta, lens, T, B, C, groups, w.gn_g, w.gn_b, 1e-5f, nullptr, 0, 0, ACT_NONE, xs, s);
    else launch_gn_coeffs(x, bs, Ta, lens, T, B, C, groups, w.gn_g, w.gn_b, 1e-5f, nullptr, 0, 0, ab, s);
    ConvParams p;
    p.B = B;
    p.Tin = T;
    p.Nout = T;
    p.len_in = lens;
    p.len_out = lens;
    p.x = x;
    p.x_bs = bs;
    p.x_cs = Ta;
    p.pro_ab = ab;
    p.y = qkv;
    p.y_bs = 3 * bs;
    p.y_cs = Ta;
    static const bool env_planes = []() { const char* v = getenv("DTTS_ATTN_PLANES"); return !(v && v[0] == '0'); }();
    const bool planes = x3 && attn_x3_enabled() && env_planes && D == AttnPlanes::D;
    DTTS_REQUIRE(!t_layer_p1 || planes, "trunk_fp16: the attention has its one-product mode only on the qkv conv's operand images (split-precision path, head dim 48)");
    if (x3) {
        p.x3 = xs;
        p.x3_tp = x3_tp(T);
    }
    if (planes) {
        p.qkv_planes = qkv;
        p.qkv_heads = w.H;
        p.qkv_nt64 = AttnPlanes::nt64(T);
        p.qkv_tq = AttnPlanes::tq(T);
        p.qkv_qscale = (1.f / std::sqrt((float)D)) * 1.4426950408889634f;
    }
    run_conv(w.qkv, p, s);
    AttnParams a;
    a.qkv = qkv;
    a.bs = 3 * bs;
    a.cs = Ta;
    a.q_off = 0;
    a.k_off = D;
    a.v_off = 2 * D;
    a.head_stride = 3 * D;
    a.out = att;
    a.o_bs = bs;
    a.o_cs = Ta;
    a.lens = lens;
    a.T = T;
    a.B = B;
    a.H = w.H;
    a.D = D;
    a.scale = 1.f / std::sqrt((float)D);
    a.bias_tab = w.bias_tab;
    a.x3 = x3 && attn_x3_enabled();
    if (planes) a.planes = qkv;
    a.p1 = t_layer_p1 ? 1 : 0;
    const bool att_planes = a.x3 && D == 48 && w.bias_tab && T + 1 < x3_tp(T);
    DTTS_REQUIRE(!f || att_planes, "fused GroupNorm: the attention must write the proj conv's planes");
    void* xs_att = f ? f->xs_alt : xs;
    if (att_planes) {
        a.out_x3 = xs_att;
        a.x3_tp = x3_tp(T);
    }
    launch_flash_attention(a, s);
    ConvParams q;
    q.B = B;
    q.Tin = T;
    q.Nout = T;
    q.len_in = lens;
    q.len_out = lens;
    q.x = att;
    q.x_bs = bs;
    q.x_cs = Ta;
    q.y = y;
    q.y_bs = bs;
    q.y_cs = Ta;
    q.res = x;
    q.res_bs = bs;
    q.res_cs = Ta;
    if (x3) {
        if (!att_planes) launch_split_planes(att, bs, Ta, nullptr, ACT_NONE, lens, T, B, C, xs, s);
        q.x3 = xs_att;
        q.x3_tp = x3_tp(T);
    }
    if (f && next) {
        gn_fill(q, f->slot, conv_x3_gn_xch_bytes(B, C, T), *next, xs, groups, s);
        f->in_ready = true;
    }
    run_conv(w.proj, q, s);
}

void Model::res_block_fwd(const Schedule& sc, const ResBlockW& w, const float* x, float* h1, float* y, float* ab, const int* lens, int B, int T,
                          int Ta, int step, hipStream_t s, void* xs, const int* step_idx, GnFuse* f, const GnNext* next) {
    const int C = cfg.diff_channels;
    const long long bs = (long long)C * Ta;
    int groups = 32;
    while (C % groups) groups /= 2;
    const bool x3 = xs && w.c1.w3 && w.c2.w3;
    DTTS_REQUIRE(!f || x3, "fused GroupNorm needs the split-precision path");
    const bool in_ready = f && f->in_ready;
    if (f) f->in_ready = false;
    if (in_ready) {}
    else if (x3) launch_gn_split_planes(x, bs, Ta, lens, T, B, C, groups, w.gn1_g, w.gn1_b, 1e-5f, nullptr, 0, 0, ACT_SILU, xs, s);
    else launch_gn_coeffs(x, bs, Ta, lens, T, B, C, groups, w.gn1_g, w.gn1_b, 1e-5f, nullptr, 0, 0, ab, s);
    ConvParams p;
    p.B = B;
    p.Tin = T;
    p.Nout = T;
    p.len_in = lens;
    p.len_out = lens;
    p.x = x;
    p.x_bs = bs;
    p.x_cs = Ta;
    p.pro_ab = ab;
    p.pro_act = ACT_SILU;
    p.y = h1;
    p.y_bs = bs;
    p.y_cs = Ta;
    if (x3) {
        p.x3 = xs;
        p.x3_tp = x3_tp(T);
    }
    const float* ada = sc.ss_table + (size_t)w.index * 2 * C * sc.n + (step_idx ? 0 : step);
    if (f) {
        GnNext n2;
        n2.gamma = w.gn2_g;
        n2.beta = w.gn2_b;
        n2.act = ACT_SILU;
        ConvParams p1 = p;
        p1.y = nullptr;
        gn_fill(p1, f->slot, conv_x3_gn_xch_bytes(B, C, T), n2, f->xs_alt, groups, s);
        p1.gn_ada = ada;
        p1.gn_ada_stride = sc.n;
        p1.gn_ada_idx = step_idx;
        run_conv(w.c1, p1, s);
    } else {
        run_conv(w.c1, p, s);
        if (x3) launch_gn_split_planes(h1, bs, Ta, lens, T, B, C, groups, w.gn2_g, w.gn2_b, 1e-5f, ada, sc.n, 0, ACT_SILU, xs, s, step_idx);
        else launch_gn_coeffs(h1, bs, Ta, lens, T, B, C, groups, w.gn2_g, w.gn2_b, 1e-5f, ada, sc.n, 0, ab, s, step_idx);
    }
    ConvParams q = p;
    q.x = h1;
    q.pad = 1;
    q.y = y;
    q.res = x;
    q.res_bs = bs;
    q.res_cs = Ta;
    if (f) {
        q.x3 = f->xs_alt;
        if (next) {
            gn_fill(q, f->slot, conv_x3_gn_xch_bytes(B, C, T), *next, xs, groups, s);
            f->in_ready = true;
        }
    }
    run_conv(w.c2, q, s);
}

Model::PairPlan Model::plan_pair(const int* lens_host, int B, int T, hipStream_t s) {
    std::vector<int> l2(2 * B), li, um(2 * B), ul;
    for (int b = 0; b < B; ++b) {
        const int len = lens_host ? lens_host[b] : T;
        l2[b] = l2[B + b] = len;
        li.push_back(len);
        um[b] = b;
        int gidx = -1;
        for (size_t k = 0; k < ul.size(); ++k)
            if (ul[k] == len) gidx = (int)k;
        if (gidx < 0) { gidx = (int)ul.size(); ul.push_back(len); }
        um[B + b] = B + gidx;
    }
    for (int v : ul) li.push_back(v);
    PairPlan pl;
    pl.Nu = (int)ul.size();
    pl.ulen = ul;
    pl.lens2 = upload_ints(l2.data(), 2 * B, s);
    pl.lens_i = upload_ints(li.data(), (int)li.size(), s);
    pl.umap = upload_ints(um.data(), 2 * B, s);
    register_cols(pl.lens2, l2.data(), 2 * B, T, s);
    register_cols(pl.lens_i, li.data(), (int)li.size(), T, s);
    return pl;
}

void Model::diff_forward_pair(const Schedule& sc, const float* x, const float* cbuf0, const int* lens2, const int* lens_i, const int* umap, int B, int Nu,
                              int T, int step, float* out2, hipStream_t s, const float* integ) {
    const int C = cfg.diff_channels, Ta = T, OC = cfg.diff_out_channels;
    const long long bs = (long long)C * Ta;
    static const bool env_two = []() { const char* v = getenv("DTTS_TWO_STREAMS"); return !(v && v[0] == '0'); }();
    const bool two_streams = env_two && opt_two_streams_;
    int groups = 32;
    while (C % groups) groups /= 2;
    const bool x3 = use_x3();
    DTTS_REQUIRE(!opt_trunk_fp16_ || x3, "trunk_fp16 = 1 needs the split-precision kernels (conv_x3 = 1)");

    float* xin = ws().f32((size_t)B * C * Ta);
    float* xpath = ws().f32((size_t)B * C * Ta);
    {
        ConvParams p = cp(x, cfg.mel_channels, xin, C, B, T, Ta, lens2);
        p.x_bs = (long long)cfg.mel_channels * T;
        p.x_cs = T;
        p.pad = 1;
        ConvParams q = cp(xin, C, xpath, C, B, T, Ta, lens2);
        if (x3) {
            void* xs0 = ws().raw(x3_bytes(B, C, T));
            launch_split_planes(x, p.x_bs, T, nullptr, ACT_NONE, lens2, T, B, cfg.mel_channels, xs0, s);
            p.x3 = xs0;
            p.x3_tp = x3_tp(T);
            run_conv(inp_block_, p, s);
            launch_split_planes(xin, bs, Ta, nullptr, ACT_NONE, lens2, T, B, C, xs0, s);
            q.x3 = xs0;
            q.x3_tp = x3_tp(T);
            run_conv(integ1_, q, s);
        } else {
            run_conv(inp_block_, p, s);
            run_conv(integ1_, q, s);
        }
    }
    static const int env_ns = []() { const char* v = getenv("DTTS_CFG_STREAMS"); return v ? atoi(v) : 0; }();
    int NS = env_ns > 0 ? env_ns : (opt_cfg_streams_ > 0 ? opt_cfg_streams_ : (B <= 4 ? 1 : 2));
    if (!two_streams) NS = 1;
    if (NS > MAX_CFG_STREAMS) NS = MAX_CFG_STREAMS;
    while (NS > 1 && ((2 * B) % NS != 0 || (B % ((2 * B) / NS) != 0 && ((2 * B) / NS) % B != 0))) --NS;
    const int n = 2 * B / NS, Bi = B + Nu;
    for (int k = 1; k < NS; ++k)
        if (!sx_[k - 1]) make_side_stream(&sx_[k - 1]);
    if (NS > 1 && !ev_fork_) {
        DTTS_CHECK_HIP(hipEventCreateWithFlags(&ev_fork_, hipEventDisableTiming));
        for (auto& e : ev_joinx_) DTTS_CHECK_HIP(hipEventCreateWithFlags(&e, hipEventDisableTiming));
    }
    const float* code_path = integ;
    if (!integ) {
        float* bufI = ws().f32((size_t)Bi * C * Ta);
        const size_t mark = ws().mark();
        const size_t act = (size_t)Bi * C * Ta;
        float* tA = ws().f32(act);
        float* tB = ws().f32(act);
        float* qkv = ws().f32(qkv_floats(Bi, C, T));
        float* ab = ws().f32((size_t)Bi * C * 2);
        void* xs = x3 ? ws().raw(x3_bytes(Bi, C, T)) : nullptr;
        const float* in = cbuf0;
        for (int l = 0; l < 3; ++l) {
            res_block_fwd(sc, integ_[l].rb, in, tA, tB, ab, lens_i, Bi, T, Ta, step, s, xs);
            attention_block(integ_[l].at, tB, bufI, qkv, tA, ab, lens_i, Bi, T, Ta, s, xs);
            in = bufI;
        }
        ws().rewind(mark);
        code_path = bufI;
    }
    void* xs_code = nullptr;
    if (x3) {
        xs_code = ws().raw(x3_bytes(Bi, C, T));
        launch_split_planes(code_path, bs, Ta, nullptr, ACT_NONE, lens_i, T, Bi, C, xs_code, s);
    }
    if (NS > 1) {
        DTTS_CHECK_HIP(hipEventRecord(ev_fork_, s));
        for (int k = 1; k < NS; ++k) DTTS_CHECK_HIP(hipStreamWaitEvent(sx_[k - 1], ev_fork_, 0));
    }
    for (int k = 0; k < NS; ++k) {
        hipStream_t st = k ? sx_[k - 1] : s;
        const int b0 = k * n;
        const int* lens = lens2 + b0;
        const size_t act = (size_t)n * C * Ta;
        float* bufA = ws().f32(act);
        float* bufB = ws().f32(act);
        float* bufC = ws().f32(act);
        float* qkv = ws().f32(qkv_floats(n, C, T));
        float* ab = ws().f32((size_t)n * C * 2);
        void* xs = x3 ? ws().raw(x3_bytes(n, C, T)) : nullptr;
        static const int env_fuse = []() { const char* v = getenv("DTTS_GN_FUSE"); return v ? (v[0] == '0' ? 0 : 1) : -1; }();
        const bool fuse = x3 && (env_fuse >= 0 ? env_fuse != 0 : opt_gn_fuse_) && conv_x3_gn_fusable(C, C, C, 3, groups, n, T) && T + 1 < x3_tp(T);
        GnFuse fz;
        GnFuse* f = nullptr;
        if (fuse) {
            fz.xs_alt = ws().raw(x3_bytes(n, C, T));
            fz.slot = k;
            f = &fz;
        }
        auto norm_of = [](const float* g, const float* be, int act) {
            GnNext nn;
            nn.gamma = g;
            nn.beta = be;
            nn.act = act;
            return nn;
        };
        ConvParams r = cp(code_path, C, bufB, C, n, T, Ta, lens);
        r.res = xpath + (size_t)(b0 % B) * C * Ta;
        r.res_bs = bs;
        r.res_cs = Ta;
        r.res_bmod = n > B ? B : 0;
        r.x_bidx = umap + b0;
        if (x3) {
            r.x3 = xs_code;
            r.x3_tp = x3_tp(T);
        }
        const GnNext out_norm = norm_of(out_gn_g_, out_gn_b_, ACT_SILU);
        auto first_norm = [&](size_t li, size_t ti) {
            if (li < layers_.size()) return norm_of(layers_[li].rb.gn1_g, layers_[li].rb.gn1_b, ACT_SILU);
            if (ti < tail_.size()) return norm_of(tail_[ti].gn1_g, tail_[ti].gn1_b, ACT_SILU);
            return out_norm;
        };
        if (f) {
            const GnNext n0 = first_norm(0, 0);
            gn_fill(r, f->slot, conv_x3_gn_xch_bytes(n, C, T), n0, xs, groups, st);
            f->in_ready = true;
        }
        run_conv(integ2_, r, st);
        float* cur = bufB;
        float* t1 = bufA;
        float* t2 = bufC;
        for (size_t li = 0; li < layers_.size(); ++li) {
            const auto& l = layers_[li];
            LayerP1 mode(opt_trunk_fp16_ && li >= 1);
            const GnNext na = norm_of(l.at.gn_g, l.at.gn_b, ACT_NONE), nn = first_norm(li + 1, 0);
            res_block_fwd(sc, l.rb, cur, t1, t2, ab, lens, n, T, Ta, step, st, xs, nullptr, f, &na);
            attention_block(l.at, t2, cur, qkv, t1, ab, lens, n, T, Ta, st, xs, f, &nn);
        }
        for (size_t ti = 0; ti < tail_.size(); ++ti) {
            const GnNext nn = first_norm(layers_.size(), ti + 1);
            LayerP1 mode(opt_trunk_fp16_);
            res_block_fwd(sc, tail_[ti], cur, t1, t2, ab, lens, n, T, Ta, step, st, xs, nullptr, f, &nn);
            std::swap(cur, t2);
        }
        if (f && f->in_ready) {}
        else if (x3) launch_gn_split_planes(cur, bs, Ta, lens, T, n, C, groups, out_gn_g_, out_gn_b_, 1e-5f, nullptr, 0, 0, ACT_SILU, xs, st);
        else launch_gn_coeffs(cur, bs, Ta, lens, T, n, C, groups, out_gn_g_, out_gn_b_, 1e-5f, nullptr, 0, 0, ab, st);
        ConvParams o = cp(cur, C, out2 + (size_t)b0 * OC * T, OC, n, T, Ta, lens);
        o.pro_ab = ab;
        o.pro_act = ACT_SILU;
        o.pad = 1;
        o.y_bs = (long long)OC * T;
        o.y_cs = T;
        if (x3) {
            o.x3 = xs;
            o.x3_tp = x3_tp(T);
        }
        run_conv(out_conv_, o, st);
    }
    for (int k = 1; k < NS; ++k) {
        DTTS_CHECK_HIP(hipEventRecord(ev_joinx_[k - 1], sx_[k - 1]));
        DTTS_CHECK_HIP(hipStreamWaitEvent(s, ev_joinx_[k - 1], 0));
    }
}

static size_t integ_ws_bytes(int Bv, int C, int T) {
    const size_t act = (size_t)Bv * C * T;
    return sizeof(float) * (act + 2 * (3 * act + qkv_floats(Bv, C, T) + (size_t)2 * Bv * C)) + 2 * x3_bytes(Bv, C, T) + 32 * 256;
}
static int integ_chunk(int Bi) {
    static const int target = []() { const char* v = getenv("DTTS_INTEG_SAMPLES"); return v ? atoi(v) : 36; }();
    return std::max(1, target / Bi);
}

void Model::precompute_integrator(const Schedule& sc, const float* cbuf0, const int* lens_i_host, int B, int Nu, int T, const std::vector<int>& steps,
                                  float* integ_all, hipStream_t s, std::vector<std::pair<int, hipEvent_t>>* ready) {
    const int C = cfg.diff_channels, Bi = B + Nu, J = integ_chunk(Bi), NS = (int)steps.size();
    const size_t ct = (size_t)C * T, mark = ws().mark();
    const int Bv = J * Bi;
    const bool x3 = use_x3();
    static const bool env_two = []() { const char* v = getenv("DTTS_TWO_STREAMS"); return !(v && v[0] == '0'); }();
    const bool piped = ready != nullptr && NS > J;
    const bool two = (env_two && opt_two_streams_) || piped;
    if (piped) {
        if (!si_) {
            static const int cus = []() { const char* v = getenv("DTTS_INTEG_CUS"); return v ? atoi(v) : 0; }();
            if (cus > 0 && cus < 256) {
                uint32_t mask[8] = {0, 0, 0, 0, 0, 0, 0, 0};
                for (int b = 0; b < cus; ++b) mask[b >> 5] |= 1u << (b & 31);
                DTTS_CHECK_HIP(hipExtStreamCreateWithCUMask(&si_, 8, mask));
            } else {
                static const bool low = []() { const char* v = getenv("DTTS_INTEG_PRIO"); return v && v[0] == 'l'; }();
                int least = 0, greatest = 0;
                DTTS_CHECK_HIP(hipDeviceGetStreamPriorityRange(&least, &greatest));
                DTTS_CHECK_HIP(hipStreamCreateWithPriority(&si_, hipStreamNonBlocking, low ? least : 0));
            }
        }
        while ((int)ev_integ_.size() < cdiv(NS, J)) {
            hipEvent_t e;
            DTTS_CHECK_HIP(hipEventCreateWithFlags(&e, hipEventDisableTiming));
            ev_integ_.push_back(e);
        }
    }
    hipStream_t side = piped ? si_ : sx_[0];
    if (two && !piped && !sx_[0]) { make_side_stream(&sx_[0]); side = sx_[0]; }
    if (two && !ev_fork_) {
        DTTS_CHECK_HIP(hipEventCreateWithFlags(&ev_fork_, hipEventDisableTiming));
        for (auto& e : ev_joinx_) DTTS_CHECK_HIP(hipEventCreateWithFlags(&e, hipEventDisableTiming));
    }
    float* vin = ws().f32((size_t)Bv * ct);
    for (int j = 0; j < J; ++j)
        DTTS_CHECK_HIP(hipMemcpyAsync(vin + (size_t)j * Bi * ct, cbuf0, sizeof(float) * (size_t)Bi * ct, hipMemcpyDeviceToDevice, s));
    struct Lane { hipStream_t st; float *bufA, *bufB, *bufC, *qkv, *ab; void* xs; };
    Lane lanes[2];
    for (int q = 0; q < (two ? 2 : 1); ++q) {
        lanes[q].st = q ? side : s;
        lanes[q].bufB = ws().f32((size_t)Bv * ct);
        lanes[q].bufC = ws().f32((size_t)Bv * ct);
        lanes[q].bufA = ws().f32((size_t)Bv * ct);
        lanes[q].qkv = ws().f32(qkv_floats(Bv, C, T));
        lanes[q].ab = ws().f32((size_t)2 * Bv * C);
        lanes[q].xs = x3 ? ws().raw(x3_bytes(Bv, C, T)) : nullptr;
    }
    if (two) {
        DTTS_CHECK_HIP(hipEventRecord(ev_fork_, s));
        DTTS_CHECK_HIP(hipStreamWaitEvent(side, ev_fork_, 0));
    }
    std::vector<int> lv(Bv), sv(Bv);
    int ci = 0;
    const int prof_rot = prof_rot_++;
    for (int k0 = 0; k0 < NS; k0 += J, ++ci) {
        const Lane& L = lanes[piped ? (ci ? 1 : 0) : (two ? (ci & 1) : 0)];
        Profiler::gate() = ((ci / 2 + prof_rot) % Profiler::get().step_every) == 0;
        const int jn = std::min(J, NS - k0), nb = jn * Bi;
        for (int j = 0; j < jn; ++j)
            for (int b = 0; b < Bi; ++b) {
                lv[j * Bi + b] = lens_i_host[b];
                sv[j * Bi + b] = steps[k0 + j];
            }
        const int* dl = upload_ints(lv.data(), nb, L.st);
        const int* ds = upload_ints(sv.data(), nb, L.st);
        register_cols(dl, lv.data(), nb, T, L.st);
        float* outp = integ_all + (size_t)k0 * Bi * ct;
        auto dlayer = [&](const DiffLayerW& l, const float* in, float* o) {
            res_block_fwd(sc, l.rb, in, L.bufB, L.bufC, L.ab, dl, nb, T, T, 0, L.st, L.xs, ds);
            attention_block(l.at, L.bufC, o, L.qkv, L.bufB, L.ab, dl, nb, T, T, L.st, L.xs);
        };
        dlayer(integ_[0], vin, L.bufA);
        dlayer(integ_[1], L.bufA, L.bufA);
        dlayer(integ_[2], L.bufA, outp);
        register_cols(dl, nullptr, 0, T, L.st);
        if (piped && ci) {
            DTTS_CHECK_HIP(hipEventRecord(ev_integ_[ci], si_));
            ready->emplace_back(k0, ev_integ_[ci]);
        }
    }
    Profiler::gate() = true;
    if (piped) return;
    if (two) {
        DTTS_CHECK_HIP(hipEventRecord(ev_joinx_[0], sx_[0]));
        DTTS_CHECK_HIP(hipStreamWaitEvent(s, ev_joinx_[0], 0));
    }
    ws().rewind(mark);
}

static size_t pair_ws_bytes(int B, int C, int T) {
    const size_t act = (size_t)B * C * T;
    return sizeof(float) * (2 * act + 2 * (3 * act + qkv_floats(B, C, T) + (size_t)2 * B * C) + 2 * act + 2 * (2 * act + qkv_floats(B, C, T) + (size_t)2 * B * C)) +
           9 * x3_bytes(B, C, T) + 64 * 256;
}

void Model::diff_forward(const float* x, const float* code_emb, const int* lens_host, int B, int T, int step, int cond_free,
                         float* out, hipStream_t s) {
    gn_check();
    DTTS_REQUIRE(bound_, "weights not bound");
    DTTS_REQUIRE(step >= 0 && step < sched0_.n, "step out of range");
    diff_forward_s(sched0_, x, code_emb, lens_host, B, T, step, cond_free, out, s);
}

void Model::diff_forward_s(Schedule& sc, const float* x, const float* code_emb, const int* lens_host, int B, int T, int step, int cond_free,
                           float* out, hipStream_t s) {
    const int C = cfg.diff_channels, OC = cfg.diff_out_channels;
    ws().ensure(pair_ws_bytes(B, C, T) + sizeof(float) * ((size_t)2 * B * C * T + (size_t)2 * B * OC * T) + 4096);
    const PairPlan pl = plan_pair(lens_host, B, T, s);
    float* cbuf0 = ws().f32((size_t)2 * B * C * T);
    float* out2 = ws().f32((size_t)2 * B * OC * T);
    const size_t half = (size_t)B * C * T;
    if (code_emb)
        DTTS_CHECK_HIP(hipMemcpyAsync(cbuf0, code_emb, sizeof(float) * half, hipMemcpyDeviceToDevice, s));
    else
        launch_broadcast_channels(uncond_, B, C, T, cbuf0, (long long)C * T, T, s);
    launch_broadcast_channels(uncond_, pl.Nu, C, T, cbuf0 + half, (long long)C * T, T, s);
    diff_forward_pair(sc, x, cbuf0, pl.lens2, pl.lens_i, pl.umap, B, pl.Nu, T, step, out2, s);
    const float* src = out2 + (cond_free ? (size_t)B * OC * T : 0);
    DTTS_CHECK_HIP(hipMemcpyAsync(out, src, sizeof(float) * (size_t)B * OC * T, hipMemcpyDeviceToDevice, s));
}

void Model::diff_forward_t(const float* x, const float* code_emb, const int* lens_host, int B, int T, int timestep, int cond_free,
                           float* out, hipStream_t s) {
    gn_check();
    DTTS_REQUIRE(bound_, "weights not bound");
    DTTS_REQUIRE(timestep >= 0 && timestep < cfg.diff_trained_steps, "timestep out of [0, diff_trained_steps)");
    const auto it = std::lower_bound(sched0_.tmap.begin(), sched0_.tmap.end(), timestep);
    if (it != sched0_.tmap.end() && *it == timestep) {
        diff_forward_s(sched0_, x, code_emb, lens_host, B, T, (int)(it - sched0_.tmap.begin()), cond_free, out, s);
        return;
    }
    Schedule& sc = schedule(diff_schedule(&timestep, 1, s));
    diff_forward_s(sc, x, code_emb, lens_host, B, T, 0, cond_free, out, s);
    DTTS_CHECK_HIP(hipEventRecord(sc.used, s));
}

void Model::diff_forward_tf(const float* x, const float* code_emb, const int* lens_host, int B, int T, float timestep, int cond_free,
                            float* out, hipStream_t s) {
    gn_check();
    DTTS_REQUIRE(bound_, "weights not bound");
    DTTS_REQUIRE(std::isfinite(timestep) && timestep >= 0.f && timestep < (float)cfg.diff_trained_steps,
                 "timestep out of [0, diff_trained_steps)");
    if (timestep == std::floor(timestep)) {
        diff_forward_t(x, code_emb, lens_host, B, T, (int)timestep, cond_free, out, s);
        return;
    }
    auto key = std::make_unique<Schedule>();
    key->kind = 2;
    key->n = 1;
    key->ftimes = {timestep};
    Schedule& sc = schedule(cache_schedule(std::move(key), s));
    diff_forward_s(sc, x, code_emb, lens_host, B, T, 0, cond_free, out, s);
    DTTS_CHECK_HIP(hipEventRecord(sc.used, s));
}

void Model::diff_sample(const float* code_emb, const int* lens_host, int B, int T, unsigned long long seed,
                        const int* sample_ids_host, int n_steps, const float* x_init, const float* step_noise, float* mel_out,
                        int denorm, hipStream_t s) {
    diff_sample_ex(0, 0, 0.f, code_emb, lens_host, B, T, seed, sample_ids_host, n_steps, x_init, step_noise, mel_out, denorm, s);
}

void Model::diff_sample_ex(int sched_id, int sampler, float eta, const float* code_emb, const int* lens_host, int B, int T,
                           unsigned long long seed, const int* sample_ids_host, int n_steps, const float* x_init, const float* step_noise,
                           float* mel_out, int denorm, hipStream_t s) {
    gn_check();
    DTTS_REQUIRE(bound_, "weights not bound");
    DTTS_REQUIRE(sampler == 0 || sampler == 1 || sampler == 2, "sampler: 0 (p), 1 (ddim) or 2 (dpmsolver++)");
    DTTS_REQUIRE(eta >= 0.f, "eta must be >= 0");
    Schedule& sc = schedule(sched_id);
    const bool dpm = sampler == 2;
    DTTS_REQUIRE(dpm == (sc.kind == 1), dpm ? "sampler 2 (dpmsolver++) runs on a DPM schedule (dtts_diff_schedule_dpm)"
                                            : "samplers 0 / 1 run on an integer-timestep schedule (dtts_diff_schedule)");
    DTTS_REQUIRE(!dpm || (eta == 0.f && !step_noise), "dpmsolver++ draws no noise: eta must be 0 and step_noise NULL");
    const int C = cfg.diff_channels, OC = cfg.diff_out_channels, MC = cfg.mel_channels;
    if (n_steps <= 0 || n_steps > sc.n) n_steps = sc.n;
    const size_t per_call = pair_ws_bytes(B, C, T);
    static const bool env_pre_on = []() { const char* v = getenv("DTTS_INTEG_PRECOMPUTE"); return !(v && v[0] == '0'); }();
    static const double max_gb = []() { const char* v = getenv("DTTS_INTEG_MAX_GB"); return v ? atof(v) : 24.0; }();
    const size_t integ_table = sizeof(float) * (size_t)n_steps * 2 * B * C * T;
    const bool env_pre = env_pre_on && (double)integ_table <= max_gb * 1073741824.0;
    const size_t integ_bytes = env_pre ? integ_table + integ_ws_bytes(integ_chunk(B + 1) * 2 * B, C, T) : 0;
    const size_t hist_floats = dpm ? (size_t)B * MC * T : 0;
    ws().ensure(per_call + integ_bytes + sizeof(float) * ((size_t)2 * B * C * T + (size_t)2 * B * OC * T + hist_floats) + 8192);
    const PairPlan pl = plan_pair(lens_host, B, T, s);
    const int* lens2 = pl.lens2;
    const int* sids = upload_ints(sample_ids_host, B, s);
    float* cbuf0 = ws().f32((size_t)2 * B * C * T);
    float* out2 = ws().f32((size_t)2 * B * OC * T);
    float* x0_hist = dpm ? ws().f32(hist_floats) : nullptr;
    const size_t half = (size_t)B * C * T;
    DTTS_CHECK_HIP(hipMemcpyAsync(cbuf0, code_emb, sizeof(float) * half, hipMemcpyDeviceToDevice, s));
    launch_broadcast_channels(uncond_, pl.Nu, C, T, cbuf0 + half, (long long)C * T, T, s);
    float* x = mel_out;
    const long long xbs = (long long)MC * T;
    if (x_init) {
        DTTS_CHECK_HIP(hipMemcpyAsync(x, x_init, sizeof(float) * (size_t)B * MC * T, hipMemcpyDeviceToDevice, s));
    } else {
        DTTS_CHECK_HIP(hipMemsetAsync(x, 0, sizeof(float) * (size_t)B * MC * T, s));
        for (int b = 0; b < B; ++b) {
            const int len = lens_host ? lens_host[b] : T;
            if (len == T) {
                launch_philox_normal(x + (size_t)b * xbs, xbs, MC * T, 1, seed, sids + b, STAGE_DIFF_INIT, 0, 1.f, s);
            } else {
                float* tmp = out2;
                launch_philox_normal(tmp, 0, MC * len, 1, seed, sids + b, STAGE_DIFF_INIT, 0, 1.f, s);
                DTTS_CHECK_HIP(hipMemcpy2DAsync(x + (size_t)b * xbs, sizeof(float) * T, tmp, sizeof(float) * len,
                                                sizeof(float) * len, MC, hipMemcpyDeviceToDevice, s));
            }
        }
    }
    float* integ_all = nullptr;
    const int Bi = B + pl.Nu;
    static const int env_pipe = []() { const char* v = getenv("DTTS_INTEG_PIPELINE"); return v ? atoi(v) : -1; }();
    const int pipe_opt = env_pipe >= 0 ? env_pipe : opt_integ_pipeline_;
    const bool pipe = pipe_opt < 0 ? B <= 4 : pipe_opt != 0;
    std::vector<std::pair<int, hipEvent_t>> ready;
    if (env_pre) {
        std::vector<int> steps(n_steps), li(Bi);
        for (int k = 0; k < n_steps; ++k) steps[k] = sc.n - 1 - k;
        for (int b = 0; b < B; ++b) li[b] = lens_host ? lens_host[b] : T;
        for (int u = 0; u < pl.Nu; ++u) li[B + u] = pl.ulen[u];
        integ_all = ws().f32((size_t)n_steps * Bi * C * T);
        precompute_integrator(sc, cbuf0, li.data(), B, pl.Nu, T, steps, integ_all, s, pipe ? &ready : nullptr);
    }
    const size_t mark = ws().mark();
    size_t next_ready = 0;
    for (int k = 0; k < n_steps; ++k) {
        const int i = sc.n - 1 - k;
        Profiler::gate() = (k % Profiler::get().step_every) == 0;
        ws().rewind(mark);
        if (next_ready < ready.size() && ready[next_ready].first == k)
            DTTS_CHECK_HIP(hipStreamWaitEvent(s, ready[next_ready++].second, 0));
        diff_forward_pair(sc, x, cbuf0, lens2, pl.lens_i, pl.umap, B, pl.Nu, T, i, out2, s,
                          integ_all ? integ_all + (size_t)k * Bi * C * T : nullptr);
        const bool last = (k == n_steps - 1);
        const float* nz = step_noise ? step_noise + (size_t)k * B * MC * T : nullptr;
        if (dpm)
            launch_dpm_update(x, xbs, T, out2, (long long)OC * T, T, lens2, T, B, MC, sc.dpm[i], x0_hist, (denorm && last) ? 1 : 0, s);
        else if (sampler == 1)
            launch_ddim_update(x, xbs, T, out2, (long long)OC * T, T, lens2, T, B, MC, sc.ddim(i, eta), seed, sids, i, nz,
                               (denorm && last) ? 1 : 0, s);
        else
            launch_diff_update(x, xbs, T, out2, (long long)OC * T, T, lens2, T, B, MC, sc.p[i], seed, sids, i, nz, (denorm && last) ? 1 : 0, s);
    }
    Profiler::gate() = true;
    if (sc.used) DTTS_CHECK_HIP(hipEventRecord(sc.used, s));
}

void Model::diff_p_sample(float* x, const float* code_emb, const int* lens_host, int B, int T, int step, unsigned long long seed,
                          const int* sample_ids_host, const float* noise, float* x0_out, hipStream_t s) {
    diff_step(0, 0, 0.f, x, code_emb, lens_host, B, T, step, seed, sample_ids_host, noise, x0_out, s);
}

void Model::diff_step(int sched_id, int sampler, float eta, float* x, const float* code_emb, const int* lens_host, int B, int T, int step,
                      unsigned long long seed, const int* sample_ids_host, const float* noise, float* x0_out, hipStream_t s) {
    gn_check();
    DTTS_REQUIRE(bound_, "weights not bound");
    DTTS_REQUIRE(sampler == 0 || sampler == 1, "sampler: 0 (p) or 1 (ddim)");
    DTTS_REQUIRE(eta >= 0.f, "eta must be >= 0");
    Schedule& sc = schedule(sched_id);
    DTTS_REQUIRE(sc.kind == 0, "diff_step runs on an integer-timestep schedule (DPM-Solver++: diff_step_dpm)");
    DTTS_REQUIRE(step >= 0 && step < sc.n, "step out of range");
    DTTS_REQUIRE(sample_ids_host, "sample_ids");
    const int C = cfg.diff_channels, OC = cfg.diff_out_channels, MC = cfg.mel_channels;
    ws().ensure(pair_ws_bytes(B, C, T) + sizeof(float) * ((size_t)2 * B * C * T + (size_t)2 * B * OC * T) + 8192);
    const PairPlan pl = plan_pair(lens_host, B, T, s);
    const int* sids = upload_ints(sample_ids_host, B, s);
    float* cbuf0 = ws().f32((size_t)2 * B * C * T);
    float* out2 = ws().f32((size_t)2 * B * OC * T);
    const size_t half = (size_t)B * C * T;
    DTTS_CHECK_HIP(hipMemcpyAsync(cbuf0, code_emb, sizeof(float) * half, hipMemcpyDeviceToDevice, s));
    launch_broadcast_channels(uncond_, pl.Nu, C, T, cbuf0 + half, (long long)C * T, T, s);
    diff_forward_pair(sc, x, cbuf0, pl.lens2, pl.lens_i, pl.umap, B, pl.Nu, T, step, out2, s);
    if (sampler == 1)
        launch_ddim_update(x, (long long)MC * T, T, out2, (long long)OC * T, T, pl.lens2, T, B, MC, sc.ddim(step, eta), seed, sids, step, noise,
                           0, s, x0_out);
    else
        launch_diff_update(x, (long long)MC * T, T, out2, (long long)OC * T, T, pl.lens2, T, B, MC, sc.p[step], seed, sids, step, noise, 0, s,
                           x0_out);
    if (sc.used) DTTS_CHECK_HIP(hipEventRecord(sc.used, s));
}

void Model::diff_step_dpm(int sched_id, float* x, float* x0_hist, const float* code_emb, const int* lens_host, int B, int T, int step,
                          float* x0_out, hipStream_t s) {
    gn_check();
    DTTS_REQUIRE(bound_, "weights not bound");
    Schedule& sc = schedule(sched_id);
    DTTS_REQUIRE(sc.kind == 1, "diff_step_dpm runs on a DPM schedule (dtts_diff_schedule_dpm)");
    DTTS_REQUIRE(step >= 0 && step < sc.n, "step out of range");
    DTTS_REQUIRE(x && x0_hist && code_emb, "x, x0_hist, code_emb");
    const int C = cfg.diff_channels, OC = cfg.diff_out_channels, MC = cfg.mel_channels;
    ws().ensure(pair_ws_bytes(B, C, T) + sizeof(float) * ((size_t)2 * B * C * T + (size_t)2 * B * OC * T) + 8192);
    const PairPlan pl = plan_pair(lens_host, B, T, s);
    float* cbuf0 = ws().f32((size_t)2 * B * C * T);
    float* out2 = ws().f32((size_t)2 * B * OC * T);
    const size_t half = (size_t)B * C * T;
    DTTS_CHECK_HIP(hipMemcpyAsync(cbuf0, code_emb, sizeof(float) * half, hipMemcpyDeviceToDevice, s));
    launch_broadcast_channels(uncond_, pl.Nu, C, T, cbuf0 + half, (long long)C * T, T, s);
    diff_forward_pair(sc, x, cbuf0, pl.lens2, pl.lens_i, pl.umap, B, pl.Nu, T, step, out2, s);
    launch_dpm_update(x, (long long)MC * T, T, out2, (long long)OC * T, T, pl.lens2, T, B, MC, sc.dpm[step], x0_hist, 0, s, x0_out);
    DTTS_CHECK_HIP(hipEventRecord(sc.used, s));
}

void Model::diff_conditioning(const float* refer, const int* lens_host, int B, int Tmax, float* cond_out, hipStream_t s) {
    DTTS_REQUIRE(bound_, "weights not bound");
    const int C = cfg.diff_channels, C2 = 2 * C;
    const int T1 = (Tmax - 1) / 2 + 1, T2 = (T1 - 1) / 2 + 1;
    std::vector<int> l0(B), l1(B), l2(B);
    for (int b = 0; b < B; ++b) {
        l0[b] = lens_host ? lens_host[b] : Tmax;
        l1[b] = (l0[b] - 1) / 2 + 1;
        l2[b] = (l1[b] - 1) / 2 + 1;
    }
    const size_t act = (size_t)B * C2 * T2;
    const bool x3c = use_x3() && !ctx_.empty() && ctx_[0].qkv.w3;
    ws().ensure(sizeof(float) * ((size_t)B * C * T1 + 3 * act + qkv_floats(B, C2, T2) + (size_t)2 * B * C2) + (x3c ? x3_bytes(B, C2, T2) : 0) + 8192);
    const int* d0 = upload_ints(l0.data(), B, s);
    const int* d1 = upload_ints(l1.data(), B, s);
    const int* d2 = upload_ints(l2.data(), B, s);
    float* h1 = ws().f32((size_t)B * C * T1);
    float* a = ws().f32(act);
    float* bb = ws().f32(act);
    float* att = ws().f32(act);
    float* qkv = ws().f32(qkv_floats(B, C2, T2));
    float* ab = ws().f32((size_t)2 * B * C2);
    void* xsc = x3c ? ws().raw(x3_bytes(B, C2, T2)) : nullptr;
    ConvParams p;
    p.B = B;
    p.Tin = Tmax;
    p.Nout = T1;
    p.len_in = d0;
    p.len_out = d1;
    p.x = refer;
    p.x_bs = (long long)cfg.mel_channels * Tmax;
    p.x_cs = Tmax;
    p.stride = 2;
    p.pad = 1;
    p.y = h1;
    p.y_bs = (long long)C * T1;
    p.y_cs = T1;
    run_conv(ctx0_, p, s);
    ConvParams q;
    q.B = B;
    q.Tin = T1;
    q.Nout = T2;
    q.len_in = d1;
    q.len_out = d2;
    q.x = h1;
    q.x_bs = (long long)C * T1;
    q.x_cs = T1;
    q.stride = 2;
    q.pad = 1;
    q.y = a;
    q.y_bs = (long long)C2 * T2;
    q.y_cs = T2;
    run_conv(ctx1_, q, s);
    float* cur = a;
    float* nxt = bb;
    for (auto& blk : ctx_) {
        attention_block(blk, cur, nxt, qkv, att, ab, d2, B, T2, T2, s, xsc);
        std::swap(cur, nxt);
    }
    launch_mean_time(cur, (long long)C2 * T2, T2, d2, T2, B, C2, cond_out, s);
}

void Model::diff_timestep_independent(const float* latent_cm, const int* lens_n_host, int B, int nmax, const float* cond,
                                      float* code_emb, hipStream_t s) {
    DTTS_REQUIRE(bound_, "weights not bound");
    const int C = cfg.diff_channels;
    const size_t act = (size_t)B * C * nmax;
    const bool x3l = use_x3() && !latcond_.empty() && latcond_[0].qkv.w3;
    ws().ensure(sizeof(float) * (3 * act + qkv_floats(B, C, nmax) + (size_t)2 * B * C) + (x3l ? x3_bytes(B, C, nmax) : 0) + 8192);
    std::vector<int> ln(B);
    for (int b = 0; b < B; ++b) ln[b] = lens_n_host ? lens_n_host[b] : nmax;
    const int* dl = upload_ints(ln.data(), B, s);
    float* a = ws().f32(act);
    float* bb = ws().f32(act);
    float* att = ws().f32(act);
    float* qkv = ws().f32(qkv_floats(B, C, nmax));
    float* ab = ws().f32((size_t)2 * B * C);
    void* xsl = x3l ? ws().raw(x3_bytes(B, C, nmax)) : nullptr;
    const long long bs = (long long)C * nmax;
    ConvParams p;
    p.B = B;
    p.Tin = nmax;
    p.Nout = nmax;
    p.len_in = dl;
    p.len_out = dl;
    p.x = latent_cm;
    p.x_bs = bs;
    p.x_cs = nmax;
    p.pad = 1;
    p.y = a;
    p.y_bs = bs;
    p.y_cs = nmax;
    run_conv(latcond0_, p, s);
    float* cur = a;
    float* nxt = bb;
    for (auto& blk : latcond_) {
        attention_block(blk, cur, nxt, qkv, att, ab, dl, B, nmax, nmax, s, xsl);
        std::swap(cur, nxt);
    }
    int groups = 32;
    while (C % groups) groups /= 2;
    launch_gn_coeffs(cur, bs, nmax, dl, nmax, B, C, groups, code_gn_g_, code_gn_b_, 1e-5f, cond, 1, 2 * C, ab, s);
    launch_affine_apply(cur, bs, nmax, ab, dl, nmax, B, C, 4, ACT_NONE, code_emb, (long long)C * 4 * nmax, 4 * nmax, s);
}

void Model::op_attention_block(const char* prefix, const float* x, const int* lens_host, int B, int C, int T, float* y,
                               hipStream_t s) {
    DTTS_REQUIRE(bound_, "weights not bound");
    AttnBlockW w = attn_block(prefix, C, cfg.diff_heads);
    const size_t act = (size_t)B * C * T;
    ws().ensure(sizeof(float) * (act + qkv_floats(B, C, T) + (size_t)2 * B * C) + x3_bytes(B, C, T) + 8192);
    std::vector<int> l(B);
    for (int b = 0; b < B; ++b) l[b] = lens_host ? lens_host[b] : T;
    const int* dl = upload_ints(l.data(), B, s);
    float* qkv = ws().f32(qkv_floats(B, C, T));
    float* att = ws().f32(act);
    float* ab = ws().f32((size_t)2 * B * C);
    bool p1 = false;
    for (auto* grp : {&integ_, &layers_})
        for (size_t i = 0; i < grp->size(); ++i)
            if ((*grp)[i].at.qkv.w == w.qkv.w) {
                w = (*grp)[i].at;
                p1 = opt_trunk_fp16_ && grp == &layers_ && i >= 1;
            }
    LayerP1 mode(p1);
    void* xs = (use_x3() && w.qkv.w3) ? ws().raw(x3_bytes(B, C, T)) : nullptr;
    attention_block(w, x, y, qkv, att, ab, dl, B, T, T, s, xs);
}

void Model::op_resblock(const char* prefix, const float* x, const int* lens_host, int B, int T, int step, float* y,
                        hipStream_t s) {
    DTTS_REQUIRE(bound_, "weights not bound");
    DTTS_REQUIRE(step >= 0 && step < sched0_.n, "step out of range");
    const int C = cfg.diff_channels;
    const ResBlockW* found = nullptr;
    const std::string pf(prefix);
    bool p1 = false;
    auto check = [&](const ResBlockW& r, const std::string& name, bool covered) {
        if (name == pf) { found = &r; p1 = opt_trunk_fp16_ && covered; }
    };
    for (size_t i = 0; i < integ_.size(); ++i) check(integ_[i].rb, "diffusion.conditioning_timestep_integrator." + std::to_string(i) + ".resblk", false);
    for (size_t i = 0; i < layers_.size(); ++i) check(layers_[i].rb, "diffusion.layers." + std::to_string(i) + ".resblk", i >= 1);
    for (size_t i = 0; i < tail_.size(); ++i) check(tail_[i], "diffusion.layers." + std::to_string(layers_.size() + i), true);
    DTTS_REQUIRE(found, "unknown resblock prefix");
    const size_t act = (size_t)B * C * T;
    ws().ensure(sizeof(float) * (act + (size_t)2 * B * C) + x3_bytes(B, C, T) + 8192);
    std::vector<int> l(B);
    for (int b = 0; b < B; ++b) l[b] = lens_host ? lens_host[b] : T;
    const int* dl = upload_ints(l.data(), B, s);
    float* h1 = ws().f32(act);
    float* ab = ws().f32((size_t)2 * B * C);
    void* xs = use_x3() ? ws().raw(x3_bytes(B, C, T)) : nullptr;
    LayerP1 mode(p1);
    res_block_fwd(sched0_, *found, x, h1, y, ab, dl, B, T, T, step, s, xs);
}

void Model::op_conv1d(const char* name, const float* x, const int* lens_in_host, int B, int Cin, int Tin, int Cout, int KW,
                      int stride, int dil, int pad, int pro_act, int epi_act, int gate, int phases, const float* res, float* y,
                      int Tout_alloc, hipStream_t s) {
    DTTS_REQUIRE(!weights_.empty(), "weights not bound");
    const int rows = Cout * (phases > 1 ? phases : 1);
    PackedConv pc = conv(name, Cin, rows, KW, Wopt(std::string(name) + ".bp", (size_t)packed_cout(rows)) != nullptr);
    const int Nout = (Tin + 2 * pad - dil * (KW - 1) - 1) / stride + 1;
    std::vector<int> li(B), lo(B);
    for (int b = 0; b < B; ++b) {
        li[b] = lens_in_host ? lens_in_host[b] : Tin;
        lo[b] = (li[b] + 2 * pad - dil * (KW - 1) - 1) / stride + 1;
    }
    const int* dli = upload_ints(li.data(), B, s);
    const int* dlo = upload_ints(lo.data(), B, s);
    const int cout_real = gate ? Cout / 2 : Cout;
    ConvParams p;
    p.B = B;
    p.Tin = Tin;
    p.Nout = Nout;
    p.len_in = dli;
    p.len_out = dlo;
    p.x = x;
    p.x_bs = (long long)Cin * Tin;
    p.x_cs = Tin;
    p.stride = stride;
    p.dil = dil;
    p.pad = pad;
    p.pro_act = pro_act;
    p.pro_slope = 0.1f;
    p.epi_act = epi_act;
    p.epi_slope = 0.1f;
    p.gate = gate;
    p.phases = phases > 1 ? phases : 1;
    p.y = y;
    p.y_bs = (long long)cout_real * Tout_alloc;
    p.y_cs = Tout_alloc;
    if (res) {
        p.res = res;
        p.res_bs = p.y_bs;
        p.res_cs = Tout_alloc;
    }
    run_conv(pc, p, s);
}

void Model::op_philox_normal(float* out, int n, int B, unsigned long long seed, const int* sample_ids_host, int stage, int step,
                             hipStream_t s) {
    const int* sids = upload_ints(sample_ids_host, B, s);
    launch_philox_normal(out, n, n, B, seed, sids, stage, step, 1.f, s);
}

}
```

Before: 179.0 audio_s/s.

## Hoist step-invariant first-conv head and unconditional integrating conv out of diffusion loop

The integrator precompute no longer replicates the conditioning buffer J times. It computes the first res-block's GroupNorm+SiLU and 1x1 conv once, which does not depend on the step, and reuses that head across all step chunks. It also precomputes the unconditional branch's integrating_conv output per step into a table U. A new fused epilogue (EPI 5) writes a second output equal to the conv result plus a gathered addend, so the per-step CFG pair can skip recomputing those rows. The cost is extra workspace for the U table, a k-split planning override (plan_B) so the hoisted conv keeps the same reduction split and results stay consistent, and more complex code paths.

```diff
diff --git a/detail_tts_amd/csrc/conv_gemm.h b/detail_tts_amd/csrc/conv_gemm.h
--- a/detail_tts_amd/csrc/conv_gemm.h
+++ b/detail_tts_amd/csrc/conv_gemm.h
@@ -60,6 +60,10 @@
     int* next_sat = nullptr;
     int ksplit = 1;
     int ksplit_max = 0;
+    int plan_B = 0;
+    float* y2 = nullptr;
+    const float* add2 = nullptr;
+    const int* add2_idx = nullptr;
     int p1 = 0;
     int epi_vec = 0;
     float* kpart = nullptr;
diff --git a/detail_tts_amd/csrc/conv_gemm.hip b/detail_tts_amd/csrc/conv_gemm.hip
--- a/detail_tts_amd/csrc/conv_gemm.hip
+++ b/detail_tts_amd/csrc/conv_gemm.hip
@@ -14,6 +14,7 @@
     p.ablate = ablate;
     DTTS_REQUIRE(p.B > 0 && p.Nout > 0 && p.Cout > 0 && p.Cin > 0, "empty conv");
     DTTS_REQUIRE(p.x && p.w && p.y, "null pointer");
+    DTTS_REQUIRE(!p.y2, "second output: split-precision kernels only");
     DTTS_REQUIRE(p.gate == GATE_NONE || p.phases == 1, "gate+phases unsupported");
     static const int force_bn = env_int("DTTS_CONV_BN"), force_bk = env_int("DTTS_CONV_BK");
     const int halo = (p.KW - 1) * p.dil;
diff --git a/detail_tts_amd/csrc/conv_x3.h b/detail_tts_amd/csrc/conv_x3.h
--- a/detail_tts_amd/csrc/conv_x3.h
+++ b/detail_tts_amd/csrc/conv_x3.h
@@ -15,7 +15,8 @@
                               hipStream_t s, int* sat = nullptr);
 void launch_gn_split_planes(const float* x, long long x_bs, int x_cs, const int* lens, int T, int B, int C, int groups,
                             const float* gamma, const float* beta, float eps, const float* ada, int ada_stride, int ada_bs, int act,
-                            void* out, hipStream_t s, const int* ada_idx = nullptr);
+                            void* out, hipStream_t s, const int* ada_idx = nullptr, int x_bmod = 0);
+int conv_x3_ksplit(int Cin, int CoutP, int KW, int Nout, int B, int ksplit_max = 0);
 void launch_conv_x3(const ConvParams& p, hipStream_t s);
 
 constexpr size_t X3_SLAB_FLOATS = 96 * 256, X3_MAX_SLABS = 1024, X3_SPLIT_COUNTERS = 4096;
diff --git a/detail_tts_amd/csrc/conv_x3.hip b/detail_tts_amd/csrc/conv_x3.hip
--- a/detail_tts_amd/csrc/conv_x3.hip
+++ b/detail_tts_amd/csrc/conv_x3.hip
@@ -75,13 +75,13 @@
                                                               const int* __restrict__ lens, int T, int C, int groups,
                                                               const float* __restrict__ gamma, const float* __restrict__ beta, float eps,
                                                               const float* __restrict__ ada, int ada_stride, int ada_bs, int Tp,
-                                                              uint4* __restrict__ out, const int* __restrict__ ada_idx) {
+                                                              uint4* __restrict__ out, const int* __restrict__ ada_idx, int x_bmod) {
     __shared__ float red[2][16];
     __shared__ float sa[64], sd[64];
     const int g = blockIdx.x, b = blockIdx.y, tid = threadIdx.x, lane = tid & 63, wave = tid >> 6, nthr = blockDim.x;
     const int len = lens ? lens[b] : T;
     const int cpg = C / groups;
-    const float* xg = x + (long long)b * x_bs + (long long)(g * cpg) * x_cs;
+    const float* xg = x + (long long)(x_bmod ? b % x_bmod : b) * x_bs + (long long)(g * cpg) * x_cs;
     const float k = xg[0];
     float s1 = 0.f, s2 = 0.f;
     const bool vec = ((x_cs & 3) == 0) && ((reinterpret_cast<unsigned long long>(xg) & 15ull) == 0);
@@ -173,13 +173,13 @@
                                                                   const int* __restrict__ lens, int T, int C, int groups,
                                                                   const float* __restrict__ gamma, const float* __restrict__ beta, float eps,
                                                                   const float* __restrict__ ada, int ada_stride, int ada_bs, int Tp,
-                                                                  uint4* __restrict__ out, const int* __restrict__ ada_idx) {
+                                                                  uint4* __restrict__ out, const int* __restrict__ ada_idx, int x_bmod) {
     __shared__ float red[2][16];
     __shared__ float sa[64], sd[64];
     const int g = blockIdx.x, b = blockIdx.y, tid = threadIdx.x, lane = tid & 63, wave = tid >> 6;
     const int len = lens ? lens[b] : T;
     const int cpg = C / groups, c8n = cpg >> 3, C8 = C >> 3, nitems = c8n * Tp;
-    const float* xg = x + (long long)b * x_bs + (long long)(g * cpg) * x_cs;
+    const float* xg = x + (long long)(x_bmod ? b % x_bmod : b) * x_bs + (long long)(g * cpg) * x_cs;
     const float k = xg[0];
     float v[NI][8];
     float s1 = 0.f, s2 = 0.f;
@@ -775,6 +775,8 @@
         constexpr int EP_LD = 104;
         float* yb = p.y + (long long)b * p.y_bs;
         const float* rb = p.res ? p.res + (long long)(p.res_bmod ? b % p.res_bmod : b) * p.res_bs : nullptr;
+        float* y2b = EPI == 5 ? p.y2 + (long long)b * p.y_bs : nullptr;
+        const float* a2b = EPI == 5 ? p.add2 + (long long)p.add2_idx[b] * p.y_bs : nullptr;
         const int ncol0 = n0 + wn0;
         constexpr bool RES_AHEAD = NSTG >= 3;
         float4 rva[RES_AHEAD ? 4 : 1][6];
@@ -851,6 +853,14 @@
                     if (n + 3 < nvalid) *reinterpret_cast<float4*>(dst) = make_float4(o[0], o[1], o[2], o[3]);
                     else
                         for (int e = 0; e < 4 && n + e < nvalid; ++e) dst[e] = o[e];
+                    if (EPI == 5) {
+                        const long long off = (long long)row * p.y_cs + n;
+                        if (n + 3 < nvalid) {
+                            const float4 u = *reinterpret_cast<const float4*>(a2b + off);
+                            *reinterpret_cast<float4*>(y2b + off) = make_float4(o[0] + u.x, o[1] + u.y, o[2] + u.z, o[3] + u.w);
+                        } else
+                            for (int e = 0; e < 4 && n + e < nvalid; ++e) y2b[off + e] = o[e] + a2b[off + e];
+                    }
                 }
             }
             asm volatile("s_waitcnt lgkmcnt(0)" ::: "memory");
@@ -1056,8 +1066,9 @@
 
 void launch_gn_split_planes(const float* x, long long x_bs, int x_cs, const int* lens, int T, int B, int C, int groups,
                             const float* gamma, const float* beta, float eps, const float* ada, int ada_stride, int ada_bs, int act,
-                            void* out, hipStream_t s, const int* ada_idx) {
+                            void* out, hipStream_t s, const int* ada_idx, int x_bmod) {
     DTTS_REQUIRE(C % groups == 0 && (C / groups) % 8 == 0 && C / groups <= 64, "gn_split_planes: group size");
+    DTTS_REQUIRE(x_bmod >= 0, "gn_split_planes: input row modulo");
     DTTS_REQUIRE(act == ACT_NONE || act == ACT_SILU, "gn_split_planes: activation");
     const int Tp = x3_tp(T);
     uint4* o = static_cast<uint4*>(out);
@@ -1069,19 +1080,19 @@
     if (reg_ok && ns == 1 && (C / groups / 8) * Tp <= NI * 1024) {
         if (act == ACT_SILU)
             hipLaunchKernelGGL((gn_split_planes_reg_kernel<ACT_SILU, NI>), dim3(groups, B), dim3(1024), 0, s, x, x_bs, x_cs, lens, T, C, groups,
-                               gamma, beta, eps, ada, ada_stride, ada_bs, Tp, o, ada_idx);
+                               gamma, beta, eps, ada, ada_stride, ada_bs, Tp, o, ada_idx, x_bmod);
         else
             hipLaunchKernelGGL((gn_split_planes_reg_kernel<ACT_NONE, NI>), dim3(groups, B), dim3(1024), 0, s, x, x_bs, x_cs, lens, T, C, groups,
-                               gamma, beta, eps, ada, ada_stride, ada_bs, Tp, o, ada_idx);
+                               gamma, beta, eps, ada, ada_stride, ada_bs, Tp, o, ada_idx, x_bmod);
         DTTS_CHECK_HIP(hipGetLastError());
         return;
     }
     if (act == ACT_SILU)
         hipLaunchKernelGGL(gn_split_planes_kernel<ACT_SILU>, dim3(groups, B, ns), dim3(nt), 0, s, x, x_bs, x_cs, lens, T, C, groups, gamma,
-                           beta, eps, ada, ada_stride, ada_bs, Tp, o, ada_idx);
+                           beta, eps, ada, ada_stride, ada_bs, Tp, o, ada_idx, x_bmod);
     else
         hipLaunchKernelGGL(gn_split_planes_kernel<ACT_NONE>, dim3(groups, B, ns), dim3(nt), 0, s, x, x_bs, x_cs, lens, T, C, groups, gamma,
-                           beta, eps, ada, ada_stride, ada_bs, Tp, o, ada_idx);
+                           beta, eps, ada, ada_stride, ada_bs, Tp, o, ada_idx, x_bmod);
     DTTS_CHECK_HIP(hipGetLastError());
 }
 
@@ -1140,6 +1151,18 @@
     return v;
 }
 
+int conv_x3_ksplit(int Cin, int CoutP, int KW, int Nout, int B, int ksplit_max) {
+    static const int max_split = []() { const char* v = getenv("DTTS_CONV_KSPLIT"); const int n = v ? atoi(v) : 4; return n < 1 ? 1 : (n > 8 ? 8 : n); }();
+    static const long long split_wgs = []() { const char* v = getenv("DTTS_CONV_KSPLIT_WGS"); return v ? atoll(v) : 256LL; }();
+    static const int max_split_k1 = []() { const char* v = getenv("DTTS_CONV_KSPLIT_K1"); return v ? atoi(v) : 2; }();
+    const long long split_tiles = split_tiles_max();
+    const long long ntile_pad = (long long)(CoutP / BM) * cdiv(Nout, BN) * B;
+    int S = 1;
+    if (ntile_pad <= split_tiles) S = (int)std::min<long long>(std::min<long long>(KW == 3 ? max_split : std::min(max_split, max_split_k1), split_wgs / ntile_pad), (Cin >> 4) / 8);
+    if (ksplit_max > 0) S = std::min(S, ksplit_max);
+    return S < 1 ? 1 : S;
+}
+
 bool conv_x3_gn_fusable(int Cout, int CoutP, int Cin, int KW, int groups, int B, int T) {
     if (Cout != CoutP || Cout % BM || groups <= 0 || Cout % groups || Cout / groups != 24 || Cin % 16 || (KW != 1 && KW != 3)) return false;
     const int nt = cdiv(T, BN);
@@ -1176,15 +1199,9 @@
     if (gn) p.cols = nullptr;
     DTTS_REQUIRE(!p.cols || (p.ncols > 0 && p.ncols <= cdiv(p.Nout, BN) * p.B && cdiv(p.Nout, BN) < 256), "conv_x3: column table");
     const long long ntile = (long long)(p.CoutP / BM) * (p.cols ? p.ncols : cdiv(p.Nout, BN) * p.B);
-    static const int max_split = []() { const char* v = getenv("DTTS_CONV_KSPLIT"); const int n = v ? atoi(v) : 4; return n < 1 ? 1 : (n > 8 ? 8 : n); }();
-    int S = 1;
-    const long long split_tiles = split_tiles_max();
-    static const long long split_wgs = []() { const char* v = getenv("DTTS_CONV_KSPLIT_WGS"); return v ? atoll(v) : 256LL; }();
-    const long long ntile_pad = (long long)(p.CoutP / BM) * cdiv(p.Nout, BN) * p.B;
-    static const int max_split_k1 = []() { const char* v = getenv("DTTS_CONV_KSPLIT_K1"); return v ? atoi(v) : 2; }();
-    if (ntile_pad <= split_tiles) S = (int)std::min<long long>(std::min<long long>(p.KW == 3 ? max_split : std::min(max_split, max_split_k1), split_wgs / ntile_pad), (p.Cin >> 4) / 8);
-    if (p.ksplit_max > 0) S = std::min(S, p.ksplit_max);
-    if (S < 1) S = 1;
+    DTTS_REQUIRE(p.plan_B == 0 || (p.plan_B >= p.B && !gn), "conv_x3: plan_B names a larger launch of the same rows (no fused GroupNorm)");
+    const int plan_B = p.plan_B > 0 ? p.plan_B : p.B;
+    const int S = conv_x3_ksplit(p.Cin, p.CoutP, p.KW, p.Nout, plan_B, p.ksplit_max);
     p.ksplit = S;
     static const bool epi_vec_on = []() { const char* v = getenv("DTTS_X3_EPI_VEC"); return !(v && v[0] == '0'); }();
     auto al16 = [](const void* q, long long bs, int cs) { return (reinterpret_cast<unsigned long long>(q) & 15ull) == 0 && (bs & 3) == 0 && (cs & 3) == 0; };
@@ -1195,8 +1212,9 @@
         p.kcount = w.count;
     }
     const long long nwg = ntile * S;
+    const long long nwg_plan = nwg * plan_B / p.B;
     static const long long max4k3 = []() { const char* v = getenv("DTTS_CONV_STAGES4_MAXWG_K3"); return v ? atoll(v) : 128LL; }();
-    const int nstg = force_stg ? force_stg : (nwg <= (p.KW == 3 ? max4k3 : max4) ? 4 : (nwg <= max3 ? 3 : 2));
+    const int nstg = force_stg ? force_stg : (nwg_plan <= (p.KW == 3 ? max4k3 : max4) ? 4 : (nwg_plan <= max3 ? 3 : 2));
     const size_t lds = (size_t)nstg * (WTILE + XBUF) + BM * sizeof(float) + 16 + (gn ? 2 * BM * sizeof(float) : 0);
     const int l4 = 4 * (WTILE + XBUF) + 3 * BM * (int)sizeof(float) + 16;
     const dim3 grid((unsigned)nwg);
@@ -1236,6 +1254,10 @@
         } else if (p.qkv_planes) {
             DTTS_REQUIRE(p.KW == 1 && !epi && !p.res && p.Cout % 144 == 0 && p.qkv_heads * 144 == p.Cout, "qkv planes epilogue: 48-channel heads, 1x1 conv");
             DTTS_LAUNCH_X3(2, false);
+        } else if (p.y2) {
+            DTTS_REQUIRE(p.KW == 1 && !epi && !p1 && p.epi_vec && p.add2 && p.add2_idx && al16(p.y2, p.y_bs, p.y_cs) && al16(p.add2, p.y_bs, p.y_cs),
+                         "conv_x3 second output: 1x1 conv, plain epilogue, 16-byte aligned rows");
+            DTTS_LAUNCH_X3N(5, false);
         } else if (p.KW == 3) {
             if (epi) DTTS_LAUNCH_X3(1, true);
             else DTTS_LAUNCH_X3(0, true);
diff --git a/detail_tts_amd/csrc/model.h b/detail_tts_amd/csrc/model.h
--- a/detail_tts_amd/csrc/model.h
+++ b/detail_tts_amd/csrc/model.h
@@ -249,6 +249,7 @@
         else if (key == "attn_ksplit") set_attn_ksplit(value);
         else if (key == "ln_reg") set_ln_channels_reg(value != 0);
         else if (key == "integ_pipeline") opt_integ_pipeline_ = value;
+        else if (key == "integ_hoist") opt_integ_hoist_ = value != 0;
         else throw Error(-1, "unknown option '" + key + "'");
     }
     int get_option(const std::string& key) const {
@@ -303,7 +304,7 @@
                          int T, int Ta, hipStream_t s, void* xs = nullptr, GnFuse* f = nullptr, const GnNext* next = nullptr);
     void res_block_fwd(const Schedule& sc, const ResBlockW& w, const float* x, float* h1, float* y, float* ab, const int* lens, int B, int T, int Ta,
                        int step, hipStream_t s, void* xs = nullptr, const int* step_idx = nullptr, GnFuse* f = nullptr,
-                       const GnNext* next = nullptr);
+                       const GnNext* next = nullptr, const float* h1_pre = nullptr, int src_bmod = 0);
     struct GnXch {
         void* buf = nullptr;
         size_t bytes = 0;
@@ -318,10 +319,14 @@
     void gn_check();
     bool use_x3() const;
     void diff_forward_pair(const Schedule& sc, const float* x, const float* cbuf0, const int* lens2, const int* lens_i, const int* umap, int B, int Nu,
-                           int T, int step, float* out2, hipStream_t s, const float* integ = nullptr);
+                           int T, int step, float* out2, hipStream_t s, const float* integ = nullptr, const float* U = nullptr, const int* ug = nullptr);
+    struct PairCut { int NS = 1, n = 0; bool fuse = false, from_u = false; };
+    PairCut pair_cut(int B, int T) const;
+    bool integ_hoist_on() const;
     void precompute_integrator(const Schedule& sc, const float* cbuf0, const int* lens_i_host, int B, int Nu, int T, const std::vector<int>& steps,
-                               float* integ_all, hipStream_t s, std::vector<std::pair<int, hipEvent_t>>* ready = nullptr);
-    struct PairPlan { const int *lens2, *lens_i, *umap; int Nu; std::vector<int> ulen; };
+                               float* integ_all, hipStream_t s, std::vector<std::pair<int, hipEvent_t>>* ready = nullptr, float* U = nullptr,
+                               int u_plan = 0);
+    struct PairPlan { const int *lens2, *lens_i, *umap, *ug; int Nu; std::vector<int> ulen; };
     PairPlan plan_pair(const int* lens_host, int B, int T, hipStream_t s);
 
     std::unordered_map<std::string, std::pair<const float*, size_t>> weights_;
@@ -425,6 +430,7 @@
     static constexpr int MAX_CFG_STREAMS = 4;
     hipStream_t sx_[MAX_CFG_STREAMS - 1] = {nullptr, nullptr, nullptr};
     hipEvent_t ev_fork_ = nullptr, ev_joinx_[MAX_CFG_STREAMS - 1] = {nullptr, nullptr, nullptr};
+    bool opt_integ_hoist_ = true;
     int opt_integ_pipeline_ = 0;
     hipStream_t si_ = nullptr;
     std::vector<hipEvent_t> ev_integ_;
diff --git a/detail_tts_amd/csrc/model.hip b/detail_tts_amd/csrc/model.hip
--- a/detail_tts_amd/csrc/model.hip
+++ b/detail_tts_amd/csrc/model.hip
@@ -798,16 +798,19 @@
 }
 
 void Model::res_block_fwd(const Schedule& sc, const ResBlockW& w, const float* x, float* h1, float* y, float* ab, const int* lens, int B, int T,
-                          int Ta, int step, hipStream_t s, void* xs, const int* step_idx, GnFuse* f, const GnNext* next) {
+                          int Ta, int step, hipStream_t s, void* xs, const int* step_idx, GnFuse* f, const GnNext* next, const float* h1_pre,
+                          int src_bmod) {
     const int C = cfg.diff_channels;
     const long long bs = (long long)C * Ta;
     int groups = 32;
     while (C % groups) groups /= 2;
     const bool x3 = xs && w.c1.w3 && w.c2.w3;
     DTTS_REQUIRE(!f || x3, "fused GroupNorm needs the split-precision path");
+    const bool pre = h1_pre != nullptr;
+    DTTS_REQUIRE(!pre || (x3 && !f && src_bmod > 0), "res_block_fwd: a precomputed head needs the split-precision path without the fused GroupNorm");
     const bool in_ready = f && f->in_ready;
     if (f) f->in_ready = false;
-    if (in_ready) {}
+    if (in_ready || pre) {}
     else if (x3) launch_gn_split_planes(x, bs, Ta, lens, T, B, C, groups, w.gn1_g, w.gn1_b, 1e-5f, nullptr, 0, 0, ACT_SILU, xs, s);
     else launch_gn_coeffs(x, bs, Ta, lens, T, B, C, groups, w.gn1_g, w.gn1_b, 1e-5f, nullptr, 0, 0, ab, s);
     ConvParams p;
@@ -842,8 +845,9 @@
         p1.gn_ada_idx = step_idx;
         run_conv(w.c1, p1, s);
     } else {
-        run_conv(w.c1, p, s);
-        if (x3) launch_gn_split_planes(h1, bs, Ta, lens, T, B, C, groups, w.gn2_g, w.gn2_b, 1e-5f, ada, sc.n, 0, ACT_SILU, xs, s, step_idx);
+        if (!pre) run_conv(w.c1, p, s);
+        if (x3) launch_gn_split_planes(pre ? h1_pre : h1, bs, Ta, lens, T, B, C, groups, w.gn2_g, w.gn2_b, 1e-5f, ada, sc.n, 0, ACT_SILU, xs, s, step_idx,
+                                       pre ? src_bmod : 0);
         else launch_gn_coeffs(h1, bs, Ta, lens, T, B, C, groups, w.gn2_g, w.gn2_b, 1e-5f, ada, sc.n, 0, ab, s, step_idx);
     }
     ConvParams q = p;
@@ -853,6 +857,7 @@
     q.res = x;
     q.res_bs = bs;
     q.res_cs = Ta;
+    if (pre) q.res_bmod = src_bmod;
     if (f) {
         q.x3 = f->xs_alt;
         if (next) {
@@ -864,7 +869,7 @@
 }
 
 Model::PairPlan Model::plan_pair(const int* lens_host, int B, int T, hipStream_t s) {
-    std::vector<int> l2(2 * B), li, um(2 * B), ul;
+    std::vector<int> l2(2 * B), li, um(2 * B), ul, ug(B);
     for (int b = 0; b < B; ++b) {
         const int len = lens_host ? lens_host[b] : T;
         l2[b] = l2[B + b] = len;
@@ -875,6 +880,7 @@
             if (ul[k] == len) gidx = (int)k;
         if (gidx < 0) { gidx = (int)ul.size(); ul.push_back(len); }
         um[B + b] = B + gidx;
+        ug[b] = gidx;
     }
     for (int v : ul) li.push_back(v);
     PairPlan pl;
@@ -883,21 +889,44 @@
     pl.lens2 = upload_ints(l2.data(), 2 * B, s);
     pl.lens_i = upload_ints(li.data(), (int)li.size(), s);
     pl.umap = upload_ints(um.data(), 2 * B, s);
+    pl.ug = upload_ints(ug.data(), B, s);
     register_cols(pl.lens2, l2.data(), 2 * B, T, s);
     register_cols(pl.lens_i, li.data(), (int)li.size(), T, s);
     return pl;
 }
 
+Model::PairCut Model::pair_cut(int B, int T) const {
+    const int C = cfg.diff_channels;
+    static const bool env_two = []() { const char* v = getenv("DTTS_TWO_STREAMS"); return !(v && v[0] == '0'); }();
+    static const int env_ns = []() { const char* v = getenv("DTTS_CFG_STREAMS"); return v ? atoi(v) : 0; }();
+    int NS = env_ns > 0 ? env_ns : (opt_cfg_streams_ > 0 ? opt_cfg_streams_ : (B <= 4 ? 1 : 2));
+    if (!(env_two && opt_two_streams_)) NS = 1;
+    if (NS > MAX_CFG_STREAMS) NS = MAX_CFG_STREAMS;
+    while (NS > 1 && ((2 * B) % NS != 0 || (B % ((2 * B) / NS) != 0 && ((2 * B) / NS) % B != 0))) --NS;
+    PairCut c;
+    c.NS = NS;
+    c.n = 2 * B / NS;
+    int groups = 32;
+    while (C % groups) groups /= 2;
+    static const int env_fuse = []() { const char* v = getenv("DTTS_GN_FUSE"); return v ? (v[0] == '0' ? 0 : 1) : -1; }();
+    c.fuse = use_x3() && (env_fuse >= 0 ? env_fuse != 0 : opt_gn_fuse_) && conv_x3_gn_fusable(C, C, C, 3, groups, c.n, T) && T + 1 < x3_tp(T);
+    c.from_u = use_x3() && integ_hoist_on() && NS > 1 && c.n <= B && !c.fuse;
+    return c;
+}
+
 void Model::diff_forward_pair(const Schedule& sc, const float* x, const float* cbuf0, const int* lens2, const int* lens_i, const int* umap, int B, int Nu,
-                              int T, int step, float* out2, hipStream_t s, const float* integ) {
+                              int T, int step, float* out2, hipStream_t s, const float* integ, const float* U, const int* ug) {
     const int C = cfg.diff_channels, Ta = T, OC = cfg.diff_out_channels;
     const long long bs = (long long)C * Ta;
-    static const bool env_two = []() { const char* v = getenv("DTTS_TWO_STREAMS"); return !(v && v[0] == '0'); }();
-    const bool two_streams = env_two && opt_two_streams_;
     int groups = 32;
     while (C % groups) groups /= 2;
     const bool x3 = use_x3();
     DTTS_REQUIRE(!opt_trunk_fp16_ || x3, "trunk_fp16 = 1 needs the split-precision kernels (conv_x3 = 1)");
+
+    const PairCut cut = pair_cut(B, T);
+    const int NS = cut.NS, n = cut.n, Bi = B + Nu;
+    const bool from_u = U && ug && integ && cut.from_u;
+    float* ustart = from_u ? ws().f32((size_t)B * C * Ta) : nullptr;
 
     float* xin = ws().f32((size_t)B * C * Ta);
     float* xpath = ws().f32((size_t)B * C * Ta);
@@ -916,18 +945,17 @@
             launch_split_planes(xin, bs, Ta, nullptr, ACT_NONE, lens2, T, B, C, xs0, s);
             q.x3 = xs0;
             q.x3_tp = x3_tp(T);
+            if (from_u) {
+                q.y2 = ustart;
+                q.add2 = U;
+                q.add2_idx = ug;
+            }
             run_conv(integ1_, q, s);
         } else {
             run_conv(inp_block_, p, s);
             run_conv(integ1_, q, s);
         }
     }
-    static const int env_ns = []() { const char* v = getenv("DTTS_CFG_STREAMS"); return v ? atoi(v) : 0; }();
-    int NS = env_ns > 0 ? env_ns : (opt_cfg_streams_ > 0 ? opt_cfg_streams_ : (B <= 4 ? 1 : 2));
-    if (!two_streams) NS = 1;
-    if (NS > MAX_CFG_STREAMS) NS = MAX_CFG_STREAMS;
-    while (NS > 1 && ((2 * B) % NS != 0 || (B % ((2 * B) / NS) != 0 && ((2 * B) / NS) % B != 0))) --NS;
-    const int n = 2 * B / NS, Bi = B + Nu;
     for (int k = 1; k < NS; ++k)
         if (!sx_[k - 1]) make_side_stream(&sx_[k - 1]);
     if (NS > 1 && !ev_fork_) {
@@ -956,7 +984,7 @@
     void* xs_code = nullptr;
     if (x3) {
         xs_code = ws().raw(x3_bytes(Bi, C, T));
-        launch_split_planes(code_path, bs, Ta, nullptr, ACT_NONE, lens_i, T, Bi, C, xs_code, s);
+        launch_split_planes(code_path, bs, Ta, nullptr, ACT_NONE, lens_i, T, from_u ? B : Bi, C, xs_code, s);
     }
     if (NS > 1) {
         DTTS_CHECK_HIP(hipEventRecord(ev_fork_, s));
@@ -973,8 +1001,7 @@
         float* qkv = ws().f32(qkv_floats(n, C, T));
         float* ab = ws().f32((size_t)n * C * 2);
         void* xs = x3 ? ws().raw(x3_bytes(n, C, T)) : nullptr;
-        static const int env_fuse = []() { const char* v = getenv("DTTS_GN_FUSE"); return v ? (v[0] == '0' ? 0 : 1) : -1; }();
-        const bool fuse = x3 && (env_fuse >= 0 ? env_fuse != 0 : opt_gn_fuse_) && conv_x3_gn_fusable(C, C, C, 3, groups, n, T) && T + 1 < x3_tp(T);
+        const bool fuse = cut.fuse;
         GnFuse fz;
         GnFuse* f = nullptr;
         if (fuse) {
@@ -1010,8 +1037,9 @@
             gn_fill(r, f->slot, conv_x3_gn_xch_bytes(n, C, T), n0, xs, groups, st);
             f->in_ready = true;
         }
-        run_conv(integ2_, r, st);
-        float* cur = bufB;
+        const bool chunk_u = from_u && b0 >= B;
+        if (!chunk_u) run_conv(integ2_, r, st);
+        float* cur = chunk_u ? ustart + (size_t)(b0 - B) * C * Ta : bufB;
         float* t1 = bufA;
         float* t2 = bufC;
         for (size_t li = 0; li < layers_.size(); ++li) {
@@ -1048,6 +1076,11 @@
     }
 }
 
+bool Model::integ_hoist_on() const {
+    static const int env = []() { const char* v = getenv("DTTS_INTEG_HOIST"); return v ? (v[0] == '0' ? 0 : 1) : -1; }();
+    return env >= 0 ? env != 0 : opt_integ_hoist_;
+}
+
 static size_t integ_ws_bytes(int Bv, int C, int T) {
     const size_t act = (size_t)Bv * C * T;
     return sizeof(float) * (act + 2 * (3 * act + qkv_floats(Bv, C, T) + (size_t)2 * Bv * C)) + 2 * x3_bytes(Bv, C, T) + 32 * 256;
@@ -1058,11 +1091,13 @@
 }
 
 void Model::precompute_integrator(const Schedule& sc, const float* cbuf0, const int* lens_i_host, int B, int Nu, int T, const std::vector<int>& steps,
-                                  float* integ_all, hipStream_t s, std::vector<std::pair<int, hipEvent_t>>* ready) {
+                                  float* integ_all, hipStream_t s, std::vector<std::pair<int, hipEvent_t>>* ready, float* U, int u_plan) {
     const int C = cfg.diff_channels, Bi = B + Nu, J = integ_chunk(Bi), NS = (int)steps.size();
     const size_t ct = (size_t)C * T, mark = ws().mark();
     const int Bv = J * Bi;
     const bool x3 = use_x3();
+    const bool hoist = x3 && integ_hoist_on();
+    DTTS_REQUIRE(!U || (hoist && u_plan > 0), "precompute_integrator: the unconditional integrating_conv table belongs to integ_hoist");
     static const bool env_two = []() { const char* v = getenv("DTTS_TWO_STREAMS"); return !(v && v[0] == '0'); }();
     const bool piped = ready != nullptr && NS > J;
     const bool two = (env_two && opt_two_streams_) || piped;
@@ -1092,9 +1127,21 @@
         DTTS_CHECK_HIP(hipEventCreateWithFlags(&ev_fork_, hipEventDisableTiming));
         for (auto& e : ev_joinx_) DTTS_CHECK_HIP(hipEventCreateWithFlags(&e, hipEventDisableTiming));
     }
-    float* vin = ws().f32((size_t)Bv * ct);
-    for (int j = 0; j < J; ++j)
-        DTTS_CHECK_HIP(hipMemcpyAsync(vin + (size_t)j * Bi * ct, cbuf0, sizeof(float) * (size_t)Bi * ct, hipMemcpyDeviceToDevice, s));
+    float *vin = nullptr, *h1_0[2] = {nullptr, nullptr};
+    int h1_nb[2] = {0, 0};
+    const ResBlockW& rb0 = integ_[0].rb;
+    if (hoist) {
+        const int nb_full = NS >= J ? J * Bi : 0, nb_tail = (NS % J) * Bi;
+        auto split_of = [&](int nb) { return conv_x3_ksplit(rb0.c1.Cin, rb0.c1.CoutP, 1, T, nb); };
+        h1_nb[0] = nb_full ? nb_full : nb_tail;
+        h1_nb[1] = (nb_full && nb_tail && split_of(nb_tail) != split_of(nb_full)) ? nb_tail : 0;
+        for (int v = 0; v < 2; ++v)
+            if (h1_nb[v]) h1_0[v] = ws().f32((size_t)Bi * ct);
+    } else {
+        vin = ws().f32((size_t)Bv * ct);
+        for (int j = 0; j < J; ++j)
+            DTTS_CHECK_HIP(hipMemcpyAsync(vin + (size_t)j * Bi * ct, cbuf0, sizeof(float) * (size_t)Bi * ct, hipMemcpyDeviceToDevice, s));
+    }
     struct Lane { hipStream_t st; float *bufA, *bufB, *bufC, *qkv, *ab; void* xs; };
     Lane lanes[2];
     for (int q = 0; q < (two ? 2 : 1); ++q) {
@@ -1106,11 +1153,27 @@
         lanes[q].ab = ws().f32((size_t)2 * Bv * C);
         lanes[q].xs = x3 ? ws().raw(x3_bytes(Bv, C, T)) : nullptr;
     }
+    if (hoist) {
+        int groups = 32;
+        while (C % groups) groups /= 2;
+        const int* dli = upload_ints(lens_i_host, Bi, s);
+        register_cols(dli, lens_i_host, Bi, T, s);
+        launch_gn_split_planes(cbuf0, (long long)ct, T, dli, T, Bi, C, groups, rb0.gn1_g, rb0.gn1_b, 1e-5f, nullptr, 0, 0, ACT_SILU, lanes[0].xs, s);
+        for (int v = 0; v < 2; ++v) {
+            if (!h1_0[v]) continue;
+            ConvParams p = cp(cbuf0, C, h1_0[v], C, Bi, T, T, dli);
+            p.x3 = lanes[0].xs;
+            p.x3_tp = x3_tp(T);
+            p.plan_B = h1_nb[v];
+            run_conv(rb0.c1, p, s);
+        }
+        register_cols(dli, nullptr, 0, T, s);
+    }
     if (two) {
         DTTS_CHECK_HIP(hipEventRecord(ev_fork_, s));
         DTTS_CHECK_HIP(hipStreamWaitEvent(side, ev_fork_, 0));
     }
-    std::vector<int> lv(Bv), sv(Bv);
+    std::vector<int> lv(Bv), sv(Bv), lu;
     int ci = 0;
     const int prof_rot = prof_rot_++;
     for (int k0 = 0; k0 < NS; k0 += J, ++ci) {
@@ -1130,9 +1193,32 @@
             res_block_fwd(sc, l.rb, in, L.bufB, L.bufC, L.ab, dl, nb, T, T, 0, L.st, L.xs, ds);
             attention_block(l.at, L.bufC, o, L.qkv, L.bufB, L.ab, dl, nb, T, T, L.st, L.xs);
         };
-        dlayer(integ_[0], vin, L.bufA);
+        if (hoist) {
+            res_block_fwd(sc, rb0, cbuf0, L.bufB, L.bufC, L.ab, dl, nb, T, T, 0, L.st, L.xs, ds, nullptr, nullptr,
+                          (h1_0[1] && nb == h1_nb[1]) ? h1_0[1] : h1_0[0], Bi);
+            attention_block(integ_[0].at, L.bufC, L.bufA, L.qkv, L.bufB, L.ab, dl, nb, T, T, L.st, L.xs);
+        } else {
+            dlayer(integ_[0], vin, L.bufA);
+        }
         dlayer(integ_[1], L.bufA, L.bufA);
         dlayer(integ_[2], L.bufA, outp);
+        if (U) {
+            for (int u = 0; u < Nu; ++u)
+                for (int j0 = 0; j0 < jn; j0 += u_plan) {
+                    const int nj = std::min(u_plan, jn - j0);
+                    lu.assign((size_t)nj, lens_i_host[B + u]);
+                    const int* dlu = upload_ints(lu.data(), nj, L.st);
+                    const float* src = outp + ((size_t)j0 * Bi + B + u) * ct;
+                    launch_split_planes(src, (long long)Bi * ct, T, nullptr, ACT_NONE, dlu, T, nj, C, L.xs, L.st);
+                    ConvParams r = cp(src, C, U + ((size_t)(k0 + j0) * Nu + u) * ct, C, nj, T, T, dlu);
+                    r.x_bs = (long long)Bi * ct;
+                    r.y_bs = (long long)Nu * ct;
+                    r.x3 = L.xs;
+                    r.x3_tp = x3_tp(T);
+                    r.plan_B = u_plan;
+                    run_conv(integ2_, r, L.st);
+                }
+        }
         register_cols(dl, nullptr, 0, T, L.st);
         if (piped && ci) {
             DTTS_CHECK_HIP(hipEventRecord(ev_integ_[ci], si_));
@@ -1150,7 +1236,7 @@
 
 static size_t pair_ws_bytes(int B, int C, int T) {
     const size_t act = (size_t)B * C * T;
-    return sizeof(float) * (2 * act + 2 * (3 * act + qkv_floats(B, C, T) + (size_t)2 * B * C) + 2 * act + 2 * (2 * act + qkv_floats(B, C, T) + (size_t)2 * B * C)) +
+    return sizeof(float) * (3 * act + 2 * (3 * act + qkv_floats(B, C, T) + (size_t)2 * B * C) + 2 * act + 2 * (2 * act + qkv_floats(B, C, T) + (size_t)2 * B * C)) +
            9 * x3_bytes(B, C, T) + 64 * 256;
 }
 
@@ -1241,7 +1327,12 @@
     const bool env_pre = env_pre_on && (double)integ_table <= max_gb * 1073741824.0;
     const size_t integ_bytes = env_pre ? integ_table + integ_ws_bytes(integ_chunk(B + 1) * 2 * B, C, T) : 0;
     const size_t hist_floats = dpm ? (size_t)B * MC * T : 0;
-    ws().ensure(per_call + integ_bytes + sizeof(float) * ((size_t)2 * B * C * T + (size_t)2 * B * OC * T + hist_floats) + 8192);
+    const PairCut cut = pair_cut(B, T);
+    const bool want_u = env_pre && cut.from_u;
+    int nu = 1;
+    for (int b = 1; lens_host && b < B; ++b) nu += std::find(lens_host, lens_host + b, lens_host[b]) == lens_host + b ? 1 : 0;
+    const size_t u_bytes = want_u ? sizeof(float) * (size_t)n_steps * nu * C * T + 256 : 0;
+    ws().ensure(per_call + integ_bytes + u_bytes + sizeof(float) * ((size_t)2 * B * C * T + (size_t)2 * B * OC * T + hist_floats) + 8192);
     const PairPlan pl = plan_pair(lens_host, B, T, s);
     const int* lens2 = pl.lens2;
     const int* sids = upload_ints(sample_ids_host, B, s);
@@ -1269,7 +1360,7 @@
             }
         }
     }
-    float* integ_all = nullptr;
+    float *integ_all = nullptr, *u_all = nullptr;
     const int Bi = B + pl.Nu;
     static const int env_pipe = []() { const char* v = getenv("DTTS_INTEG_PIPELINE"); return v ? atoi(v) : -1; }();
     const int pipe_opt = env_pipe >= 0 ? env_pipe : opt_integ_pipeline_;
@@ -1281,7 +1372,8 @@
         for (int b = 0; b < B; ++b) li[b] = lens_host ? lens_host[b] : T;
         for (int u = 0; u < pl.Nu; ++u) li[B + u] = pl.ulen[u];
         integ_all = ws().f32((size_t)n_steps * Bi * C * T);
-        precompute_integrator(sc, cbuf0, li.data(), B, pl.Nu, T, steps, integ_all, s, pipe ? &ready : nullptr);
+        if (want_u) u_all = ws().f32((size_t)n_steps * pl.Nu * C * T);
+        precompute_integrator(sc, cbuf0, li.data(), B, pl.Nu, T, steps, integ_all, s, pipe ? &ready : nullptr, u_all, cut.n);
     }
     const size_t mark = ws().mark();
     size_t next_ready = 0;
@@ -1292,7 +1384,7 @@
         if (next_ready < ready.size() && ready[next_ready].first == k)
             DTTS_CHECK_HIP(hipStreamWaitEvent(s, ready[next_ready++].second, 0));
         diff_forward_pair(sc, x, cbuf0, lens2, pl.lens_i, pl.umap, B, pl.Nu, T, i, out2, s,
-                          integ_all ? integ_all + (size_t)k * Bi * C * T : nullptr);
+                          integ_all ? integ_all + (size_t)k * Bi * C * T : nullptr, u_all ? u_all + (size_t)k * pl.Nu * C * T : nullptr, pl.ug);
         const bool last = (k == n_steps - 1);
         const float* nz = step_noise ? step_noise + (size_t)k * B * MC * T : nullptr;
         if (dpm)
```

New measurement: 180.2 audio_s/s (median of 6 runs). No clear change (+0.7%).
